# MarinerQ/npf_GWwaveform

Measured on AMD Instinct MI355X. Metric: waveform target-points/sec (train step), higher is better.
Workload: dtype f32 (every contraction of the step: fp32 operands as three exact bf16 terms, six v_mfma_f32_16x16x32_bf16 per product group, f32 accumulation -- f32 results, DESIGN.md 3.1 / 3.2; the 1-4-wide first / last layers: f32 FMAs); 1 GPU; BASELINE config 2: AttnCNP scaledot, r=256, 4-layer xy-encoder/decoder, 256 context / 1024 target points, 256 tasks per GPU (256 global), fp32 train step (fwd+loss+bwd+allreduce+Adam); tasks_per_gpu=256, global_tasks=256, context_points=256, target_points=1024, r_dim=256, n_params=799588, parallelism=dp1, hip_graph=True

## Files before the change

include/npf_hip.h:

```cpp
#ifndef NPF_HIP_H
#define NPF_HIP_H

#include <stdint.h>

#ifdef __cplusplus
extern "C" {
#endif

#define NPF_OK 0
#define NPF_EINVAL (-1)
#define NPF_ELAUNCH (-2)

#define NPF_MAX_OPS 40
#define NPF_MAX_FEATURES 512

enum npf_opcode {
  NPF_OP_END = 0,
  NPF_OP_LOAD_PT = 1,
  NPF_OP_STORE_PT = 2,
  NPF_OP_LOAD_ROWS = 3,
  NPF_OP_STORE_ROWS = 4,
  NPF_OP_LINEAR = 5,
  NPF_OP_SOFTMAX = 6,
  NPF_OP_ADD_PT = 7,
  NPF_OP_MASK_POS = 8,
  NPF_OP_ADD_TASKVEC = 9,
  NPF_OP_ROWDOT_PT = 10,
  NPF_OP_SOFTMAX_BWD = 11,
  NPF_OP_RELU = 12,
  NPF_OP_SCALE = 13,
  NPF_OP_STORE_TR = 14,
  NPF_OP_LAYERNORM = 15,
  NPF_OP_STORE_WB = 18,
  NPF_OP_STORE_TRB = 19,
  NPF_OP_LOAD_RM = 17,
  NPF_OP_STORE_MASK = 20,
  NPF_OP_MASK_BITS = 21,
  NPF_OP_LAYERNORM_BWD = 16
};

enum npf_wmode {
  NPF_W_ROWMAJOR = 0,
  NPF_W_PT_ROWS = 1,
  NPF_W_PT_COLS = 2
};

#define NPF_F_RELU 1u
#define NPF_F_ADD_PT 2u
#define NPF_F_MASK_PT 4u
#define NPF_F_P16 16u
#define NPF_F_MASK_BITS 32u
#define NPF_F_ADD_RM 8u
#define NPF_F_STORE_IN 64u
#define NPF_F_STORE_BITS 256u
#define NPF_F_STORE_P16 128u

typedef struct npf_op {
  int32_t op;
  int32_t i0;
  int32_t i1;
  int32_t i2;
  int32_t i3;
  uint32_t flags;
  float f0;
  int32_t i4;
  const void *p0;
  const void *p1;
  const void *p2;
  int64_t s0;
  int64_t s1;
  void *p3;
} npf_op_t;

typedef struct npf_program {
  int32_t n_ops;
  int32_t n_tasks;
  int32_t pts_per_task;
  int32_t tiles_per_task;
  int32_t wg_per_task;
  int32_t reserved[3];
  npf_op_t ops[NPF_MAX_OPS];
} npf_program_t;

int npf_chain_run(const npf_program_t *prog, void *stream);

typedef struct npf_wgrad_job {
  const float *dZ;
  const float *A;
  float *dW;
  float *db;
  int64_t ldw;
  int32_t N, K;
  int32_t per_task;
  int32_t accumulate;
  int32_t ldz, lda, ldo;
  int32_t reserved;
} npf_wgrad_job_t;
#define NPF_WGRAD_ACCUMULATE 1
#define NPF_WGRAD_BF16 2
#define NPF_WGRAD_DZ16 4
#define NPF_WGRAD_A16 8
#define NPF_WGRAD_F32X6 16
#define NPF_WGRAD_NO_H16 32

#define NPF_MAX_WGRAD_JOBS 16
int npf_wgrad_run(const npf_wgrad_job_t *jobs, int32_t n_jobs, int32_t n_tasks, int32_t tiles_per_task,
                  float *partials, int64_t partials_bytes, void *stream);
int64_t npf_wgrad_partials_bytes(const npf_wgrad_job_t *jobs, int32_t n_jobs, int32_t n_tasks,
                                 int32_t tiles_per_task);

int npf_gauss_head_fwd(const float *suff, int32_t n_rows, int32_t pts, int32_t dy, int32_t homoskedastic,
                       const float *Y, int32_t n_y_rows, float *loc, float *scale, float *sum_logp,
                       void *stream);
int npf_gauss_head_bwd(const float *suff, const float *loc, const float *scale, int32_t n_rows, int32_t pts,
                       int32_t dy, int32_t homoskedastic, const float *Y, int32_t n_y_rows,
                       const float *d_loc, const float *d_scale, const float *d_sum_logp, float *d_suff,
                       void *stream);

int npf_masked_gauss_head_fwd(const float *suff, const int32_t *n_valid, int32_t n_tasks, int32_t n_rows, int32_t pts, int32_t dy,
                              int32_t homoskedastic, const float *Y, int32_t n_y_rows, float *loc, float *scale,
                              float *sum_logp, void *stream);
int npf_masked_gauss_head_bwd(const float *suff, const float *loc, const float *scale, const int32_t *n_valid, int32_t n_tasks,
                              int32_t n_rows, int32_t pts, int32_t dy, int32_t homoskedastic, const float *Y, int32_t n_y_rows,
                              const float *d_loc, const float *d_scale, const float *d_sum_logp, float *d_suff, void *stream);

int npf_mixture_summary(const float *suff, const int32_t *n_valid, int32_t n_z, int32_t n_tasks, int32_t pts, int32_t dy,
                        int32_t homoskedastic, const float *z_p, int32_t n_probs, const float *probs, float *mean, float *std,
                        float *quant, void *stream);

int npf_mixture_score(const float *suff, const float *Y, const int32_t *n_valid, int32_t n_z, int32_t n_tasks, int32_t pts,
                      int32_t dy, int32_t homoskedastic, float *log_density, float *pit, float *crps, void *stream);

int npf_mc_objective_fwd(const float *log_w, int32_t n_z, int32_t n_tasks, int32_t mode, const float *inv_weights,
                         int32_t m, float *out, void *stream);
int npf_mc_objective_bwd(const float *log_w, int32_t n_z, int32_t n_tasks, int32_t mode, const float *inv_weights,
                         int32_t m, const float *d_out, float *d_log_w, float *workspace, void *stream);

int npf_mean_agg_fwd(const float *R_pt, int32_t n_tasks, int32_t pts_per_task, int32_t F, float *out,
                     void *stream);
int npf_mean_agg_bwd(const float *d_out, int32_t n_tasks, int32_t pts_per_task, int32_t F, float *dR_pt,
                     int32_t accumulate, void *stream);

int npf_pack_pt(const float *rows, int32_t n_tasks, int32_t pts_per_task, int32_t F_valid, float *pt,
                void *stream);
int npf_unpack_pt(const float *pt, int32_t n_tasks, int32_t pts_per_task, int32_t F_valid, float *rows,
                  void *stream);
int npf_transpose(const float *src, int32_t rows, int32_t cols, float *dst, void *stream);
int npf_split_heads(const float *src, int32_t n_tasks, int32_t pts_per_task, int32_t F, int32_t n_heads, float *dst,
                    void *stream);
int npf_merge_heads(const float *src, int32_t n_tasks, int32_t pts_per_task, int32_t F, int32_t n_heads, float *dst,
                    void *stream);

int npf_mha_fwd(const float *q, const float *k, const float *v, int32_t n_tasks, int32_t n_heads, int32_t n_keys,
                int32_t n_queries, int32_t F, float *out, float *lse, void *stream);
int npf_mha_bwd(const float *q, const float *k, const float *v, const float *out, const float *d_out, const float *lse,
                int32_t n_tasks, int32_t n_heads, int32_t n_keys, int32_t n_queries, int32_t F, float *d_q, float *d_k, float *d_v,
                void *stream);

int npf_add_layernorm_fwd(const float *a, const float *b, const float *gamma, const float *beta, float eps, int32_t n_tasks,
                          int32_t pts_per_task, int32_t F, float *y, float *stats, void *stream);
int npf_add_layernorm_bwd(const float *a, const float *b, const float *gamma, const float *stats, const float *dy, int32_t n_tasks,
                          int32_t pts_per_task, int32_t F, float *dx, float *partials, void *stream);

int npf_gather_points(const float *x, const float *y, const int64_t *idx, int32_t n_tasks, int32_t n_points,
                      int32_t n_sel, int32_t x_dim, int32_t y_dim, float *out_x, float *out_y, void *stream);

int npf_cast_bf16_weights(const float *src, int32_t n_rows, int32_t n_cols, int32_t ld, int32_t transposed, void *dst,
                          void *stream);

typedef struct npf_wprep_job {
  const float *src;
  void *dst;
  int32_t n_rows, n_cols, ld, kind;
} npf_wprep_job_t;
#define NPF_MAX_WPREP_JOBS 32
int npf_prepare_weights(const npf_wprep_job_t *jobs, int32_t n_jobs, void *stream);

#define NPF_X6_MAX_LAYERS 8
typedef struct {
  const void *w_img;
  const float *bias;
  const float *mask;
  float *store_in;
  float *store_out;
  const float *addend;
  unsigned long long *store_bits;
  const unsigned long long *mask_bits;
  int32_t relu;
  int32_t reserved;
} npf_x6_layer_t;
int npf_mlp_x6_run(const npf_x6_layer_t *layers, int32_t n_layers, const float *x, float *y, int32_t n_tasks,
                   int32_t tiles_per_task, void *stream);
int npf_mlp_x6_run_rows(const npf_x6_layer_t *layers, int32_t n_layers, const float *x, const float *in_rows, const float *in_w,
                        float *y, const float *out_w, const float *out_b, float *out_rows, int32_t n_tasks,
                        int32_t tiles_per_task, void *stream);

#define NPF_X6_MAX_OPS 12
typedef struct npf_x6_op {
  const float *in_pt;
  const float *in_rows;
  const float *in_w;
  const float *in_b;
  const float *pre_add;
  const float *mask;
  const unsigned long long *mask_bits;
  const float *sbwd_p;
  float *store_in;
  unsigned long long *store_in_bits;
  const void *w_img;
  int64_t w_task_stride;
  const float *bias;
  int64_t bias_task_stride;
  const float *addend;
  float *store_out;
  unsigned long long *store_bits;
  int32_t in_n;
  int32_t in_relu;
  int32_t relu;
  int32_t softmax_n;
  float softmax_scale;
  float sbwd_scale;
  int32_t reserved[2];
} npf_x6_op_t;
#define NPF_X6_IN_RM 1
#define NPF_X6_ADD_RM 2
#define NPF_X6_STORE_IN_F32 4
#define NPF_X6_STORE_OUT_F32 8
#define NPF_X6_DEFAULT_VARIANT 3
int npf_x6_run_ex(const npf_x6_op_t *ops, int32_t n_ops, const float *out_w, const float *out_b, float *out_rows,
                  int32_t n_tasks, int32_t tiles_per_task, int32_t pts_per_task, int32_t per_task, int32_t width,
                  int32_t variant, void *stream);
int npf_x6_run(const npf_x6_op_t *ops, int32_t n_ops, const float *out_w, const float *out_b, float *out_rows,
               int32_t n_tasks, int32_t tiles_per_task, int32_t per_task, int32_t width, void *stream);
int npf_x6_task_images(const float *src, int32_t n_tasks, int32_t pts, int32_t width, void *row_img, void *tr_img, void *stream);

int npf_b16_run(const npf_x6_op_t *ops, int32_t n_ops, const float *out_w, const float *out_b, float *out_rows, int32_t n_tasks,
                int32_t tiles_per_task, int32_t per_task, int32_t width, int32_t variant, void *stream);
int npf_b16_task_images(const float *src, int32_t n_tasks, int32_t pts, int32_t width, void *row_img, void *tr_img, void *stream);

int npf_masked_attn_fwd(const float *q, const float *k, const float *v, const int32_t *n_valid, int32_t n_tasks, int32_t n_keys,
                        int32_t n_queries, int32_t d, float scale, float *out, float *lse, void *stream);
int npf_masked_attn_bwd(const float *q, const float *k, const float *v, const int32_t *n_valid, const float *out, const float *d_out,
                        const float *lse, int32_t n_tasks, int32_t n_keys, int32_t n_queries, int32_t d, float scale, float *d_q,
                        float *d_k, float *d_v, void *stream);
int npf_masked_attn_fwd_nq(const float *q, const float *k, const float *v, const int32_t *n_valid, const int32_t *n_q_valid,
                           int32_t n_tasks, int32_t n_keys, int32_t n_queries, int32_t d, float scale, float *out, float *lse,
                           void *stream);
int npf_masked_attn_bwd_nq(const float *q, const float *k, const float *v, const int32_t *n_valid, const int32_t *n_q_valid,
                           const float *out, const float *d_out, const float *lse, int32_t n_tasks, int32_t n_keys, int32_t n_queries,
                           int32_t d, float scale, float *d_q, float *d_k, float *d_v, void *stream);
int npf_masked_attn_fwd_prefix(const float *q, const float *k_pre, const float *v_pre, const int32_t *n_prefix, const float *k_tail,
                               const float *v_tail, const int32_t *n_tail, const int32_t *n_q_valid, int32_t n_tasks,
                               int32_t n_prefix_tasks, int32_t c_pad, int32_t m_tail, int32_t n_queries, int32_t d, float scale,
                               float *out, void *stream);
int npf_masked_attn_fwd_loo(const float *q, const float *k, const float *v, const int32_t *n_valid, const int32_t *n_q_valid,
                            int32_t n_tasks, int32_t n_keys, int32_t n_queries, int32_t d, float scale, float *out, void *stream);
int npf_masked_mean_fwd(const float *R_pt, const int32_t *n_valid, int32_t n_tasks, int32_t pts_per_task, int32_t F, float *out,
                        void *stream);
int npf_masked_mean_bwd(const float *d_out, const int32_t *n_valid, int32_t n_tasks, int32_t pts_per_task, int32_t F, float *dR_pt,
                        int32_t accumulate, void *stream);
int npf_loo_mean(const float *R_pt, const int32_t *n_valid, int32_t n_tasks, int32_t pts_per_task, int32_t F, float *out,
                 void *stream);
int npf_masked_attn_fwd_weighted(const float *q, const float *k, const float *v, const float *w, const int32_t *n_valid,
                                 const int32_t *n_q_valid, int32_t n_tasks, int32_t n_ctx_tasks, int32_t n_keys, int32_t n_queries,
                                 int32_t d, float scale, float *out, void *stream);
int npf_weighted_mean(const float *R_pt, const float *w, const int32_t *n_valid, int32_t n_tasks, int32_t n_ctx_tasks,
                      int32_t pts_per_task, int32_t F, float *out, void *stream);

int npf_masked_attn_fwd_weighted_ex(const float *q, const float *k, const float *v, const float *w, const int32_t *n_valid,
                                    const int32_t *n_q_valid, int32_t n_tasks, int32_t n_ctx_tasks, int32_t n_keys,
                                    int32_t n_queries, int32_t d, float scale, float *out, float *lse, void *stream);
int npf_masked_attn_bwd_weighted(const float *q, const float *k, const float *v, const float *w, const int32_t *n_valid,
                                 const int32_t *n_q_valid, const float *out, const float *d_out, const float *lse, int32_t n_tasks,
                                 int32_t n_keys, int32_t n_queries, int32_t d, float scale, float *d_q, float *d_k, float *d_v,
                                 float *d_w, void *stream);
int npf_weighted_mean_bwd(const float *R_pt, const float *w, const int32_t *n_valid, const float *out, const float *d_out,
                          int32_t n_tasks, int32_t pts_per_task, int32_t F, float *dR_pt, float *dw, void *stream);

#define NPF_APPEND_MAX_PAIRS 3
typedef struct npf_append_pair {
  const float *src;
  float *dst;
  int32_t F;
  int32_t reserved;
} npf_append_pair_t;
int npf_append_points(const npf_append_pair_t *pairs, int32_t n_pairs, int32_t *n_valid, const int32_t *n_new, int32_t n_tasks,
                      int32_t n_rows, int32_t capacity, void *stream);

#define NPF_WAVEFORM_JC 16
int64_t npf_waveform_match_workspace_bytes(int32_t n_rows, int32_t n_tau);
int npf_waveform_match(const float *h, int32_t h_ld, const float *g, const float *wgt, int32_t wgt_rows, const float *freq,
                       int32_t freq_rows, const int32_t *n_valid, int32_t n_rows, int32_t n_tasks, int32_t pts, double tau0,
                       double dtau, int32_t n_tau, float *hh, float *gg, float *overlap, float *match, float *mismatch,
                       int32_t *tau_index, float *phase, float *corr, void *workspace, void *stream);
int npf_waveform_match_ex(const float *h, int32_t h_ld, const float *g, const float *wgt, int32_t wgt_rows, const float *freq,
                          int32_t freq_rows, const int32_t *n_valid, int32_t n_rows, int32_t n_tasks, int32_t pts, double tau0,
                          double dtau, int32_t n_tau, float *hh, float *gg, float *overlap, float *match, float *mismatch,
                          int32_t *tau_index, float *phase, float *corr, void *workspace, double *saved, void *stream);
int npf_waveform_match_bwd(const float *h, int32_t h_ld, const float *g, const float *wgt, int32_t wgt_rows, const float *freq,
                           int32_t freq_rows, const int32_t *n_valid, int32_t n_rows, int32_t n_tasks, int32_t pts, double tau0,
                           double dtau, int32_t n_tau, const int32_t *tau_index, const double *saved, const float *d_match,
                           int32_t n_bcast, float *d_h, int32_t dh_ld, void *stream);

#define NPF_LOGLIKE_I0_SWITCH 24.0
int64_t npf_waveform_loglike_workspace_bytes(int32_t n_rows, int32_t n_tau);
int npf_waveform_loglike(const float *h, int32_t h_ld, const float *d, const float *wgt, int32_t wgt_rows, const float *freq,
                         int32_t freq_rows, const int32_t *n_valid, int32_t n_rows, int32_t n_tasks, int32_t pts, double tau0,
                         double dtau, int32_t n_tau, double *hh, double *dd, double *snr, double *lnl_max, double *lnl_marg,
                         int32_t *tau_index, double *phase, double *series, double *lnl_mix, double *lnl_max_mix, void *workspace,
                         void *stream);

#define NPF_NET_MAX_DET 8
int64_t npf_waveform_loglike_net_workspace_bytes(int32_t n_rows, int32_t n_det, int32_t n_tau);
int npf_waveform_loglike_net(const float *h, int32_t h_ld, const float *d, const float *wgt, int32_t wgt_rows, const float *freq,
                             int32_t freq_rows, const int32_t *n_valid, const double *delay, const double *resp, int32_t n_rows,
                             int32_t n_tasks, int32_t n_det, int32_t pts, double tau0, double dtau, int32_t n_tau, double *hh,
                             double *dd, double *snr, double *lnl_max, double *lnl_marg, int32_t *tau_index, double *phase,
                             double *series, double *lnl_mix, double *lnl_max_mix, double *hh_det, double *snr_det, double *dd_det,
                             void *workspace, void *stream);

int npf_version(void);

#ifdef __cplusplus
}
#endif
#endif
```

npf_gwwaveform_amd/_lib.py:

```python
from __future__ import annotations

import ctypes as C
import os
from typing import Optional

import torch

from . import _build

NPF_MAX_OPS = 40
NPF_MAX_FEATURES = 512
NPF_WGRAD_BLOCK = 256
NPF_MAX_FUSED_ROW = 256

OP_END, OP_LOAD_PT, OP_STORE_PT, OP_LOAD_ROWS, OP_STORE_ROWS, OP_LINEAR, OP_SOFTMAX, OP_ADD_PT, OP_MASK_POS, \
    OP_ADD_TASKVEC, OP_ROWDOT_PT, OP_SOFTMAX_BWD, OP_RELU, OP_SCALE, OP_STORE_TR, OP_LAYERNORM, OP_LAYERNORM_BWD, OP_LOAD_RM, OP_STORE_WB, OP_STORE_TRB, \
    OP_STORE_MASK, OP_MASK_BITS = range(22)
W_ROWMAJOR, W_PT_ROWS, W_PT_COLS = range(3)
F_RELU, F_ADD_PT, F_MASK_PT, F_ADD_RM, F_P16, F_MASK_BITS, F_STORE_IN, F_STORE_P16, F_STORE_BITS = 1, 2, 4, 8, 16, 32, 64, 128, 256


class NpfOp(C.Structure):
    _fields_ = [
        ("op", C.c_int32), ("i0", C.c_int32), ("i1", C.c_int32), ("i2", C.c_int32), ("i3", C.c_int32),
        ("flags", C.c_uint32), ("f0", C.c_float), ("i4", C.c_int32),
        ("p0", C.c_void_p), ("p1", C.c_void_p), ("p2", C.c_void_p),
        ("s0", C.c_int64), ("s1", C.c_int64), ("p3", C.c_void_p),
    ]


class NpfProgram(C.Structure):
    _fields_ = [
        ("n_ops", C.c_int32), ("n_tasks", C.c_int32), ("pts_per_task", C.c_int32), ("tiles_per_task", C.c_int32),
        ("wg_per_task", C.c_int32), ("reserved", C.c_int32 * 3),
        ("ops", NpfOp * NPF_MAX_OPS),
    ]


class NpfWgradJob(C.Structure):
    _fields_ = [
        ("dZ", C.c_void_p), ("A", C.c_void_p), ("dW", C.c_void_p), ("db", C.c_void_p), ("ldw", C.c_int64),
        ("N", C.c_int32), ("K", C.c_int32), ("per_task", C.c_int32), ("accumulate", C.c_int32),
        ("ldz", C.c_int32), ("lda", C.c_int32), ("ldo", C.c_int32), ("reserved", C.c_int32),
    ]


NPF_MAX_WGRAD_JOBS = 16
WGRAD_F32X6 = 16
WGRAD_NO_H16 = 32


class NpfWprepJob(C.Structure):
    _fields_ = [("src", C.c_void_p), ("dst", C.c_void_p), ("n_rows", C.c_int32), ("n_cols", C.c_int32), ("ld", C.c_int32),
                ("kind", C.c_int32)]


NPF_MAX_WPREP_JOBS = 32
NPF_X6_MAX_LAYERS = 8


class NpfX6Layer(C.Structure):
    _fields_ = [("w_img", C.c_void_p), ("bias", C.c_void_p), ("mask", C.c_void_p), ("store_in", C.c_void_p),
                ("store_out", C.c_void_p), ("addend", C.c_void_p), ("store_bits", C.c_void_p), ("mask_bits", C.c_void_p),
                ("relu", C.c_int32), ("reserved", C.c_int32)]


NPF_X6_MAX_OPS = 12
X6_IN_RM, X6_ADD_RM = 1, 2
X6_STORE_IN_F32, X6_STORE_OUT_F32 = 4, 8


class NpfX6Op(C.Structure):
    _fields_ = [("in_pt", C.c_void_p), ("in_rows", C.c_void_p), ("in_w", C.c_void_p), ("in_b", C.c_void_p),
                ("pre_add", C.c_void_p), ("mask", C.c_void_p), ("mask_bits", C.c_void_p), ("sbwd_p", C.c_void_p),
                ("store_in", C.c_void_p), ("store_in_bits", C.c_void_p), ("w_img", C.c_void_p), ("w_task_stride", C.c_int64),
                ("bias", C.c_void_p), ("bias_task_stride", C.c_int64), ("addend", C.c_void_p), ("store_out", C.c_void_p),
                ("store_bits", C.c_void_p), ("in_n", C.c_int32), ("in_relu", C.c_int32), ("relu", C.c_int32),
                ("softmax_n", C.c_int32), ("softmax_scale", C.c_float), ("sbwd_scale", C.c_float), ("reserved", C.c_int32 * 2)]


NPF_APPEND_MAX_PAIRS = 3


class NpfAppendPair(C.Structure):
    _fields_ = [("src", C.c_void_p), ("dst", C.c_void_p), ("F", C.c_int32), ("reserved", C.c_int32)]


assert C.sizeof(NpfAppendPair) == 24
assert C.sizeof(NpfX6Op) == 17 * 8 + 8 * 4
assert C.sizeof(NpfOp) == 80 and C.sizeof(NpfProgram) == 32 + 80 * NPF_MAX_OPS and C.sizeof(NpfWgradJob) == 72 and C.sizeof(NpfWprepJob) == 32

_i32, _i64, _p = C.c_int32, C.c_int64, C.c_void_p
SIGNATURES = {
    "npf_chain_run": (C.c_int, [C.POINTER(NpfProgram), _p]),
    "npf_wgrad_run": (C.c_int, [C.POINTER(NpfWgradJob), _i32, _i32, _i32, _p, _i64, _p]),
    "npf_wgrad_partials_bytes": (_i64, [C.POINTER(NpfWgradJob), _i32, _i32, _i32]),
    "npf_gauss_head_fwd": (C.c_int, [_p, _i32, _i32, _i32, _i32, _p, _i32, _p, _p, _p, _p]),
    "npf_gauss_head_bwd": (C.c_int, [_p, _p, _p, _i32, _i32, _i32, _i32, _p, _i32, _p, _p, _p, _p, _p]),
    "npf_mc_objective_fwd": (C.c_int, [_p, _i32, _i32, _i32, _p, _i32, _p, _p]),
    "npf_mc_objective_bwd": (C.c_int, [_p, _i32, _i32, _i32, _p, _i32, _p, _p, _p, _p]),
    "npf_mean_agg_fwd": (C.c_int, [_p, _i32, _i32, _i32, _p, _p]),
    "npf_mean_agg_bwd": (C.c_int, [_p, _i32, _i32, _i32, _p, _i32, _p]),
    "npf_pack_pt": (C.c_int, [_p, _i32, _i32, _i32, _p, _p]),
    "npf_unpack_pt": (C.c_int, [_p, _i32, _i32, _i32, _p, _p]),
    "npf_transpose": (C.c_int, [_p, _i32, _i32, _p, _p]),
    "npf_cast_bf16_weights": (C.c_int, [_p, _i32, _i32, _i32, _i32, _p, _p]),
    "npf_prepare_weights": (C.c_int, [C.POINTER(NpfWprepJob), _i32, _p]),
    "npf_gather_points": (C.c_int, [_p, _p, _p, _i32, _i32, _i32, _i32, _i32, _p, _p, _p]),
    "npf_split_heads": (C.c_int, [_p, _i32, _i32, _i32, _i32, _p, _p]),
    "npf_merge_heads": (C.c_int, [_p, _i32, _i32, _i32, _i32, _p, _p]),
    "npf_mlp_x6_run": (C.c_int, [C.POINTER(NpfX6Layer), _i32, _p, _p, _i32, _i32, _p]),
    "npf_mlp_x6_run_rows": (C.c_int, [C.POINTER(NpfX6Layer), _i32, _p, _p, _p, _p, _p, _p, _p, _i32, _i32, _p]),
    "npf_x6_run": (C.c_int, [C.POINTER(NpfX6Op), _i32, _p, _p, _p, _i32, _i32, _i32, _i32, _p]),
    "npf_x6_run_ex": (C.c_int, [C.POINTER(NpfX6Op), _i32, _p, _p, _p, _i32, _i32, _i32, _i32, _i32, _i32, _p]),
    "npf_x6_task_images": (C.c_int, [_p, _i32, _i32, _i32, _p, _p, _p]),
    "npf_b16_run": (C.c_int, [C.POINTER(NpfX6Op), _i32, _p, _p, _p, _i32, _i32, _i32, _i32, _i32, _p]),
    "npf_b16_task_images": (C.c_int, [_p, _i32, _i32, _i32, _p, _p, _p]),
    "npf_mha_fwd": (C.c_int, [_p, _p, _p, _i32, _i32, _i32, _i32, _i32, _p, _p, _p]),
    "npf_mha_bwd": (C.c_int, [_p, _p, _p, _p, _p, _p, _i32, _i32, _i32, _i32, _i32, _p, _p, _p, _p]),
    "npf_add_layernorm_fwd": (C.c_int, [_p, _p, _p, _p, C.c_float, _i32, _i32, _i32, _p, _p, _p]),
    "npf_add_layernorm_bwd": (C.c_int, [_p, _p, _p, _p, _p, _i32, _i32, _i32, _p, _p, _p]),
    "npf_masked_attn_fwd": (C.c_int, [_p, _p, _p, _p, _i32, _i32, _i32, _i32, C.c_float, _p, _p, _p]),
    "npf_masked_attn_bwd": (C.c_int, [_p, _p, _p, _p, _p, _p, _p, _i32, _i32, _i32, _i32, C.c_float, _p, _p, _p, _p]),
    "npf_masked_attn_fwd_nq": (C.c_int, [_p, _p, _p, _p, _p, _i32, _i32, _i32, _i32, C.c_float, _p, _p, _p]),
    "npf_masked_attn_bwd_nq": (C.c_int, [_p, _p, _p, _p, _p, _p, _p, _p, _i32, _i32, _i32, _i32, C.c_float, _p, _p, _p, _p]),
    "npf_masked_attn_fwd_prefix": (C.c_int, [_p, _p, _p, _p, _p, _p, _p, _p, _i32, _i32, _i32, _i32, _i32, _i32, C.c_float, _p, _p]),
    "npf_masked_attn_fwd_loo": (C.c_int, [_p, _p, _p, _p, _p, _i32, _i32, _i32, _i32, C.c_float, _p, _p]),
    "npf_loo_mean": (C.c_int, [_p, _p, _i32, _i32, _i32, _p, _p]),
    "npf_masked_attn_fwd_weighted": (C.c_int, [_p, _p, _p, _p, _p, _p, _i32, _i32, _i32, _i32, _i32, C.c_float, _p, _p]),
    "npf_weighted_mean": (C.c_int, [_p, _p, _p, _i32, _i32, _i32, _i32, _p, _p]),
    "npf_masked_attn_fwd_weighted_ex": (C.c_int, [_p, _p, _p, _p, _p, _p, _i32, _i32, _i32, _i32, _i32, C.c_float, _p, _p, _p]),
    "npf_masked_attn_bwd_weighted": (C.c_int, [_p, _p, _p, _p, _p, _p, _p, _p, _p, _i32, _i32, _i32, _i32, C.c_float,
                                               _p, _p, _p, _p, _p]),
    "npf_weighted_mean_bwd": (C.c_int, [_p, _p, _p, _p, _p, _i32, _i32, _i32, _p, _p, _p]),
    "npf_masked_gauss_head_fwd": (C.c_int, [_p, _p, _i32, _i32, _i32, _i32, _i32, _p, _i32, _p, _p, _p, _p]),
    "npf_masked_gauss_head_bwd": (C.c_int, [_p, _p, _p, _p, _i32, _i32, _i32, _i32, _i32, _p, _i32, _p, _p, _p, _p, _p]),
    "npf_mixture_summary": (C.c_int, [_p, _p, _i32, _i32, _i32, _i32, _i32, _p, _i32, _p, _p, _p, _p, _p]),
    "npf_mixture_score": (C.c_int, [_p, _p, _p, _i32, _i32, _i32, _i32, _i32, _p, _p, _p, _p]),
    "npf_masked_mean_fwd": (C.c_int, [_p, _p, _i32, _i32, _i32, _p, _p]),
    "npf_masked_mean_bwd": (C.c_int, [_p, _p, _i32, _i32, _i32, _p, _i32, _p]),
    "npf_append_points": (C.c_int, [C.POINTER(NpfAppendPair), _i32, _p, _p, _i32, _i32, _i32, _p]),
    "npf_waveform_match_workspace_bytes": (_i64, [_i32, _i32]),
    "npf_waveform_match": (C.c_int, [_p, _i32, _p, _p, _i32, _p, _i32, _p, _i32, _i32, _i32, C.c_double, C.c_double, _i32,
                                     _p, _p, _p, _p, _p, _p, _p, _p, _p, _p]),
    "npf_waveform_match_ex": (C.c_int, [_p, _i32, _p, _p, _i32, _p, _i32, _p, _i32, _i32, _i32, C.c_double, C.c_double, _i32,
                                        _p, _p, _p, _p, _p, _p, _p, _p, _p, _p, _p]),
    "npf_waveform_match_bwd": (C.c_int, [_p, _i32, _p, _p, _i32, _p, _i32, _p, _i32, _i32, _i32, C.c_double, C.c_double, _i32,
                                         _p, _p, _p, _i32, _p, _i32, _p]),
    "npf_waveform_loglike_workspace_bytes": (_i64, [_i32, _i32]),
    "npf_waveform_loglike": (C.c_int, [_p, _i32, _p, _p, _i32, _p, _i32, _p, _i32, _i32, _i32, C.c_double, C.c_double, _i32,
                                       _p, _p, _p, _p, _p, _p, _p, _p, _p, _p, _p, _p]),
    "npf_waveform_loglike_net_workspace_bytes": (_i64, [_i32, _i32, _i32]),
    "npf_waveform_loglike_net": (C.c_int, [_p, _i32, _p, _p, _i32, _p, _i32, _p, _p, _p, _i32, _i32, _i32, _i32, C.c_double, C.c_double,
                                           _i32, _p, _p, _p, _p, _p, _p, _p, _p, _p, _p, _p, _p, _p, _p, _p]),
    "npf_version": (C.c_int, []),
}

_lib: Optional[C.CDLL] = None


def lib_path() -> str:
    return os.environ.get("NPF_HIP_LIB") or _build.LIB_PATH


def load() -> C.CDLL:
    global _lib
    if _lib is not None:
        return _lib
    path = lib_path()
    if not os.path.exists(path):
        raise RuntimeError(
            f"HIP extension {path} is missing. Build it with `python -m npf_gwwaveform_amd._build` "
            "(needs hipcc); there is no CPU fallback for the neural-process path."
        )
    try:
        lib = C.CDLL(path)
    except OSError as e:
        raise RuntimeError(f"HIP extension {path} failed to load: {e}") from e
    for name, (res, args) in SIGNATURES.items():
        fn = getattr(lib, name)
        fn.restype = res
        fn.argtypes = args
    _lib = lib
    return lib


def check(rc: int, what: str) -> None:
    if rc != 0:
        raise RuntimeError(f"{what} failed with status {rc} "
                           f"({'invalid argument/unsupported size' if rc == -1 else 'kernel launch error'})")


def stream_ptr(device: Optional[torch.device] = None) -> int:
    return torch.cuda.current_stream(device).cuda_stream


def ptr(t: Optional[torch.Tensor], strided: bool = False) -> Optional[int]:
    if t is None:
        return None
    if not t.is_cuda:
        raise RuntimeError("the HIP path takes device tensors only (got a CPU tensor); there is no CPU fallback")
    if t.dtype != torch.float32:
        raise RuntimeError(f"the HIP path computes in fp32 (got {t.dtype})")
    if not strided and not t.is_contiguous():
        raise RuntimeError("tensor handed to the HIP path must be contiguous")
    return t.data_ptr()
```

npf_gwwaveform_amd/csrc/layout_kernels.hip:

```cpp
#include "npf_common.hpp"

namespace npf {

__global__ void pack_pt_kernel(const float* __restrict__ rows, int n_tasks, int pts, int Fv, int Fp, float* __restrict__ pt) {
  const int tiles = (pts + 31) / 32;
  const size_t total = (size_t)n_tasks * tiles * (Fp / 4) * 32;
  for (size_t idx = blockIdx.x * (size_t)blockDim.x + threadIdx.x; idx < total; idx += (size_t)gridDim.x * blockDim.x) {
    const int p = idx & 31;
    const size_t r = idx >> 5;
    const int f4 = r % (Fp / 4);
    const size_t tt = r / (Fp / 4);
    const int tile = tt % tiles;
    const size_t task = tt / tiles;
    const int point = tile * 32 + p;
    f32x4 v = {0.f, 0.f, 0.f, 0.f};
    if (point < pts) {
      const float* src = rows + (task * pts + point) * (size_t)Fv + 4 * f4;
#pragma unroll
      for (int j = 0; j < 4; ++j)
        if (4 * f4 + j < Fv) v[j] = src[j];
    }
    *(f32x4*)(pt + idx * 4) = v;
  }
}

__global__ void unpack_pt_kernel(const float* __restrict__ pt, int n_tasks, int pts, int Fv, int Fp, float* __restrict__ rows) {
  const int tiles = (pts + 31) / 32;
  const size_t total = (size_t)n_tasks * tiles * (Fp / 4) * 32;
  for (size_t idx = blockIdx.x * (size_t)blockDim.x + threadIdx.x; idx < total; idx += (size_t)gridDim.x * blockDim.x) {
    const int p = idx & 31;
    const size_t r = idx >> 5;
    const int f4 = r % (Fp / 4);
    const size_t tt = r / (Fp / 4);
    const int tile = tt % tiles;
    const size_t task = tt / tiles;
    const int point = tile * 32 + p;
    if (point < pts) {
      const f32x4 v = *(const f32x4*)(pt + idx * 4);
      float* dst = rows + (task * pts + point) * (size_t)Fv + 4 * f4;
#pragma unroll
      for (int j = 0; j < 4; ++j)
        if (4 * f4 + j < Fv) dst[j] = v[j];
    }
  }
}

template <bool SPLIT>
__global__ void heads_kernel(const float* __restrict__ src, int n_tasks, int pts, int Fp, int hsz, int n_heads,
                             float* __restrict__ dst) {
  const int tiles = (pts + 31) / 32;
  const int hq = ((hsz + 31) / 32) * 8;
  const int fq = Fp / 4;
  if (SPLIT) {
    const size_t total = (size_t)n_heads * n_tasks * tiles * hq * 32;
    for (size_t idx = blockIdx.x * (size_t)blockDim.x + threadIdx.x; idx < total; idx += (size_t)gridDim.x * blockDim.x) {
      const int p = idx & 31;
      const size_t r = idx >> 5;
      const int q = r % hq;
      const size_t tt = r / hq;
      const int tile = tt % tiles;
      const size_t ht = tt / tiles;
      const int h = ht / n_tasks, b = ht - (size_t)h * n_tasks;
      f32x4 v = {0.f, 0.f, 0.f, 0.f};
      if (4 * q < hsz) v = *(const f32x4*)(src + ((((size_t)b * tiles + tile) * fq + (h * hsz) / 4 + q) * 32 + p) * 4);
      *(f32x4*)(dst + idx * 4) = v;
    }
  } else {
    const size_t total = (size_t)n_tasks * tiles * fq * 32;
    for (size_t idx = blockIdx.x * (size_t)blockDim.x + threadIdx.x; idx < total; idx += (size_t)gridDim.x * blockDim.x) {
      const int p = idx & 31;
      const size_t r = idx >> 5;
      const int q = r % fq;
      const size_t tt = r / fq;
      const int tile = tt % tiles;
      const size_t b = tt / tiles;
      const int h = (4 * q) / hsz, qh = q - (h * hsz) / 4;
      f32x4 v = {0.f, 0.f, 0.f, 0.f};
      if (h < n_heads) v = *(const f32x4*)(src + (((((size_t)h * n_tasks + b) * tiles + tile) * hq + qh) * 32 + p) * 4);
      *(f32x4*)(dst + idx * 4) = v;
    }
  }
}

__global__ void gather_points_kernel(const float* __restrict__ x, const float* __restrict__ y,
                                     const long long* __restrict__ idx, int n_tasks, int n_points, int n_sel, int x_dim,
                                     int y_dim, float* __restrict__ out_x, float* __restrict__ out_y) {
  const size_t total = (size_t)n_tasks * n_sel;
  for (size_t t = blockIdx.x * (size_t)blockDim.x + threadIdx.x; t < total; t += (size_t)gridDim.x * blockDim.x) {
    const size_t b = t / n_sel;
    long long j = idx[t];
    j = j < 0 ? 0 : (j >= n_points ? n_points - 1 : j);
    const float* xs = x + (b * n_points + (size_t)j) * x_dim;
    for (int d = 0; d < x_dim; ++d) out_x[t * x_dim + d] = xs[d];
    if (y) {
      const float* ys = y + (b * n_points + (size_t)j) * y_dim;
      for (int d = 0; d < y_dim; ++d) out_y[t * y_dim + d] = ys[d];
    }
  }
}

__global__ void cast_bf16_weights_kernel(const float* __restrict__ src, int n_rows, int n_cols, int ld, int transposed,
                                         unsigned short* __restrict__ dst) {
  const int rows = transposed ? n_cols : n_rows, cols = transposed ? n_rows : n_cols;
  const int Kp = ((cols + 31) >> 5) * 32;
  const size_t total = (size_t)rows * Kp;
  for (size_t idx = blockIdx.x * (size_t)blockDim.x + threadIdx.x; idx < total; idx += (size_t)gridDim.x * blockDim.x) {
    const int r = idx / Kp, q = idx - (size_t)r * Kp;
    const int sgrp = q >> 5, g = (q & 31) >> 3, i = q & 7;
    const int c = 32 * sgrp + (i < 4 ? 4 * g + i : 16 + 4 * g + (i - 4));
    float v = 0.f;
    if (c < cols) v = transposed ? src[(size_t)c * ld + r] : src[(size_t)r * ld + c];
    const __bf16 b = (__bf16)v;
    dst[idx] = __builtin_bit_cast(unsigned short, b);
  }
}

__global__ void transpose_kernel(const float* __restrict__ src, int rows, int cols, float* __restrict__ dst) {
  __shared__ float tile[32][33];
  const int c0 = blockIdx.x * 32, r0 = blockIdx.y * 32;
  const int tx = threadIdx.x & 31, ty = threadIdx.x >> 5;
  for (int i = ty; i < 32; i += 8)
    if (r0 + i < rows && c0 + tx < cols) tile[i][tx] = src[(size_t)(r0 + i) * cols + c0 + tx];
  __syncthreads();
  for (int i = ty; i < 32; i += 8)
    if (c0 + i < cols && r0 + tx < rows) dst[(size_t)(c0 + i) * rows + r0 + tx] = tile[tx][i];
}

struct WprepJobs {
  npf_wprep_job_t job[NPF_MAX_WPREP_JOBS];
};
__global__ void prepare_weights_kernel(const WprepJobs J) {
  __shared__ float tile[32][33];
  const npf_wprep_job_t& jb = J.job[blockIdx.y];
  const float* __restrict__ src = jb.src;
  if (jb.kind == 0) {
    float* __restrict__ dst = (float*)jb.dst;
    const int rows = jb.n_rows, cols = jb.n_cols, ld = jb.ld;
    const int tc = (cols + 31) / 32, tr = (rows + 31) / 32;
    const int tx = threadIdx.x & 31, ty = threadIdx.x >> 5;
    for (int tl = blockIdx.x; tl < tc * tr; tl += gridDim.x) {
      const int c0 = (tl % tc) * 32, r0 = (tl / tc) * 32;
      for (int i = ty; i < 32; i += 8)
        if (r0 + i < rows && c0 + tx < cols) tile[i][tx] = src[(size_t)(r0 + i) * ld + c0 + tx];
      __syncthreads();
      for (int i = ty; i < 32; i += 8)
        if (c0 + i < cols && r0 + tx < rows) dst[(size_t)(c0 + i) * rows + r0 + tx] = tile[tx][i];
      __syncthreads();
    }
  } else {
    unsigned short* __restrict__ dst = (unsigned short*)jb.dst;
    const bool transposed = (jb.kind & 3) == 2;
    const int term = (jb.kind >> 4) & 3;
    const int rows = transposed ? jb.n_cols : jb.n_rows, cols = transposed ? jb.n_rows : jb.n_cols, ld = jb.ld;
    const int Kp = (jb.kind & 4) ? 256 : ((cols + 31) >> 5) * 32;
    const size_t total = (size_t)rows * Kp;
    for (size_t idx = blockIdx.x * (size_t)blockDim.x + threadIdx.x; idx < total; idx += (size_t)gridDim.x * blockDim.x) {
      const int r = idx / Kp, q = idx - (size_t)r * Kp;
      const int sgrp = q >> 5, g = (q & 31) >> 3, i = q & 7;
      const int c = 32 * sgrp + (i < 4 ? 4 * g + i : 16 + 4 * g + (i - 4));
      float v = 0.f;
      if (c < cols) v = transposed ? src[(size_t)c * ld + r] : src[(size_t)r * ld + c];
      for (int t = 1; t < term; ++t) v -= (float)(__bf16)v;
      const __bf16 b = (__bf16)v;
      dst[idx] = __builtin_bit_cast(unsigned short, b);
    }
  }
}

template <bool MASKED>
__global__ void mean_fwd_kernel(const float* __restrict__ R, const int32_t* __restrict__ n_valid, int pts, int F,
                                float* __restrict__ out) {
  const int tiles = (pts + 31) / 32;
  const int p = threadIdx.x & 31, f4 = blockIdx.x * 8 + (threadIdx.x >> 5);
  const size_t task = blockIdx.y;
  const int n = MASKED ? clamp_count(n_valid, task, pts) : pts;
  const bool in_F = MASKED || f4 < F / 4;
  f32x4 s = {0.f, 0.f, 0.f, 0.f};
  if (in_F) {
    const float* base = R + task * tiles * (size_t)(F * 32) + pt_off(f4, p);
    for (int t = 0; t * 32 < n; ++t)
      if (t * 32 + p < n) s += *(const f32x4*)(base + (size_t)t * F * 32);
  }
#pragma unroll
  for (int off = 16; off >= 1; off >>= 1)
#pragma unroll
    for (int j = 0; j < 4; ++j) s[j] += __shfl_xor(s[j], off);
  if (p == 0 && in_F) *(f32x4*)(out + task * F + 4 * f4) = (!MASKED || n > 0) ? s * (1.f / (float)n) : f32x4{0.f, 0.f, 0.f, 0.f};
}

__global__ void loo_mean_kernel(const float* __restrict__ R, const int32_t* __restrict__ n_valid, int pts, int F,
                                float* __restrict__ out) {
  const int tiles = (pts + 31) / 32;
  const int p = threadIdx.x & 31, f4 = blockIdx.x * 8 + (threadIdx.x >> 5);
  const size_t task = blockIdx.y;
  const int n = clamp_count(n_valid, task, pts);
  const size_t at = task * tiles * (size_t)(F * 32) + pt_off(f4, p);
  double s[4] = {0.0, 0.0, 0.0, 0.0};
  for (int t = 0; t * 32 < n; ++t)
    if (t * 32 + p < n) {
      const f32x4 r = *(const f32x4*)(R + at + (size_t)t * F * 32);
#pragma unroll
      for (int j = 0; j < 4; ++j) s[j] += (double)r[j];
    }
#pragma unroll
  for (int off = 16; off >= 1; off >>= 1)
#pragma unroll
    for (int j = 0; j < 4; ++j) s[j] += __shfl_xor(s[j], off);
  const double others = (double)(n - 1);
  for (int t = 0; t < tiles; ++t) {
    f32x4 v = {0.f, 0.f, 0.f, 0.f};
    if (n > 1 && t * 32 + p < n) {
      const f32x4 r = *(const f32x4*)(R + at + (size_t)t * F * 32);
#pragma unroll
      for (int j = 0; j < 4; ++j) v[j] = (float)((s[j] - (double)r[j]) / others);
    }
    *(f32x4*)(out + at + (size_t)t * F * 32) = v;
  }
}

__global__ void weighted_mean_kernel(const float* __restrict__ R, const float* __restrict__ W, const int32_t* __restrict__ n_valid,
                                     int n_ctx_tasks, int pts, int F, float* __restrict__ out) {
  const int tiles = (pts + 31) / 32, fblocks = F / 32;
  const int p = threadIdx.x & 31, f4 = (blockIdx.x % fblocks) * 8 + (threadIdx.x >> 5);
  const size_t task = blockIdx.x / fblocks, bc = task % n_ctx_tasks;
  const int n = clamp_count(n_valid, bc, pts);
  const float* base = R + bc * tiles * (size_t)(F * 32) + pt_off(f4, p);
  const float* wrow = W + task * pts;
  double s[4] = {0.0, 0.0, 0.0, 0.0}, ws = 0.0;
  for (int t = 0; t * 32 < n; ++t)
    if (t * 32 + p < n) {
      const float w = wrow[t * 32 + p];
      if (w > 0.f && w < INFINITY) {
        const f32x4 r = *(const f32x4*)(base + (size_t)t * F * 32);
#pragma unroll
        for (int j = 0; j < 4; ++j) s[j] += (double)w * (double)r[j];
        ws += (double)w;
      }
    }
#pragma unroll
  for (int off = 16; off >= 1; off >>= 1) {
#pragma unroll
    for (int j = 0; j < 4; ++j) s[j] += __shfl_xor(s[j], off);
    ws += __shfl_xor(ws, off);
  }
  if (p == 0) {
    f32x4 v = {0.f, 0.f, 0.f, 0.f};
    if (ws > 0.0) {
#pragma unroll
      for (int j = 0; j < 4; ++j) v[j] = (float)(s[j] / ws);
    }
    *(f32x4*)(out + task * F + 4 * f4) = v;
  }
}

__global__ void weighted_mean_bwd_kernel(const float* __restrict__ R, const float* __restrict__ W, const int32_t* __restrict__ n_valid,
                                         const float* __restrict__ , const float* __restrict__ d_out, int pts, int F,
                                         float* __restrict__ dR, float* __restrict__ dW) {
  __shared__ double part[8 * 32];
  const int tiles = (pts + 31) / 32;
  const int p = threadIdx.x & 31, fg = threadIdx.x >> 5;
  const size_t task = blockIdx.x / tiles;
  const int t = blockIdx.x % tiles;
  const int n = clamp_count(n_valid, task, pts);
  const float* wrow = W + task * pts;
  double ws = 0.0;
  for (int tt = 0; tt * 32 < n; ++tt)
    if (tt * 32 + p < n) {
      const float w = wrow[tt * 32 + p];
      if (w > 0.f && w < INFINITY) ws += (double)w;
    }
#pragma unroll
  for (int off = 16; off >= 1; off >>= 1) ws += __shfl_xor(ws, off);
  const int pt = t * 32 + p;
  const float w = pt < n ? wrow[pt] : 0.f;
  const bool ok = ws > 0.0 && w > 0.f && w < INFINITY;
  const double cw = ok ? (double)w / ws : 0.0;
  const size_t base = (task * tiles + t) * (size_t)(F * 32);
  const bool any = ws > 0.0 && t * 32 < n;
  double dot = 0.0;
  for (int f4 = fg; f4 < F / 4; f4 += 8) {
    double o[4] = {0.0, 0.0, 0.0, 0.0};
    if (any) {
      for (int tt = 0; tt * 32 < n; ++tt)
        if (tt * 32 + p < n) {
          const float wk = wrow[tt * 32 + p];
          if (wk > 0.f && wk < INFINITY) {
            const f32x4 r = *(const f32x4*)(R + (task * tiles + tt) * (size_t)(F * 32) + pt_off(f4, p));
#pragma unroll
            for (int j = 0; j < 4; ++j) o[j] += (double)wk * (double)r[j];
          }
        }
#pragma unroll
      for (int off = 16; off >= 1; off >>= 1) {
#pragma unroll
        for (int j = 0; j < 4; ++j) o[j] += __shfl_xor(o[j], off);
      }
#pragma unroll
      for (int j = 0; j < 4; ++j) o[j] /= ws;
    }
    f32x4 v = {0.f, 0.f, 0.f, 0.f};
    if (ok) {
      const f32x4 r = *(const f32x4*)(R + base + pt_off(f4, p));
      const f32x4 gq = *(const f32x4*)(d_out + task * F + 4 * f4);
#pragma unroll
      for (int j = 0; j < 4; ++j) {
        v[j] = (float)(cw * (double)gq[j]);
        dot += (double)gq[j] * ((double)r[j] - o[j]);
      }
    }
    *(f32x4*)(dR + base + pt_off(f4, p)) = v;
  }
  part[fg * 32 + p] = dot;
  __syncthreads();
  if (fg == 0 && pt < pts) {
    double s = 0.0;
#pragma unroll
    for (int k = 0; k < 8; ++k) s += part[k * 32 + p];
    dW[task * pts + pt] = ok ? (float)(s / ws) : 0.f;
  }
}

template <bool MASKED>
__global__ void mean_bwd_kernel(const float* __restrict__ d_out, const int32_t* __restrict__ n_valid, int n_tasks, int pts, int F,
                                float* __restrict__ dR, int accumulate) {
  const int tiles = (pts + 31) / 32;
  const size_t total = (size_t)n_tasks * tiles * (F / 4) * 32;
  for (size_t idx = blockIdx.x * (size_t)blockDim.x + threadIdx.x; idx < total; idx += (size_t)gridDim.x * blockDim.x) {
    const int p = idx & 31;
    const size_t r = idx >> 5;
    const int f4 = r % (F / 4);
    const size_t tt = r / (F / 4);
    const int tile = tt % tiles;
    const size_t task = tt / tiles;
    const int n = MASKED ? clamp_count(n_valid, task, pts) : pts;
    f32x4 v = {0.f, 0.f, 0.f, 0.f};
    if (tile * 32 + p < n) v = *(const f32x4*)(d_out + task * F + 4 * f4) * (1.f / (float)n);
    if (accumulate) v += *(const f32x4*)(dR + idx * 4);
    *(f32x4*)(dR + idx * 4) = v;
  }
}

static unsigned grid_for(size_t total, int block) {
  size_t g = (total + block - 1) / block;
  if (g > 256u * 8u) g = 256u * 8u;
  if (g == 0) g = 1;
  return (unsigned)g;
}

}

extern "C" int npf_pack_pt(const float* rows, int32_t n_tasks, int32_t pts, int32_t Fv, float* pt, void* stream) {
  if (!rows || !pt || n_tasks <= 0 || pts <= 0 || Fv <= 0) return NPF_EINVAL;
  const int Fp = npf::round_up(Fv, 32);
  const size_t total = (size_t)n_tasks * ((pts + 31) / 32) * (Fp / 4) * 32;
  hipLaunchKernelGGL(npf::pack_pt_kernel, dim3(npf::grid_for(total, 256)), dim3(256), 0, (hipStream_t)stream, rows, n_tasks,
                     pts, Fv, Fp, pt);
  NPF_CHECK_LAUNCH();
  return NPF_OK;
}

extern "C" int npf_unpack_pt(const float* pt, int32_t n_tasks, int32_t pts, int32_t Fv, float* rows, void* stream) {
  if (!rows || !pt || n_tasks <= 0 || pts <= 0 || Fv <= 0) return NPF_EINVAL;
  const int Fp = npf::round_up(Fv, 32);
  const size_t total = (size_t)n_tasks * ((pts + 31) / 32) * (Fp / 4) * 32;
  hipLaunchKernelGGL(npf::unpack_pt_kernel, dim3(npf::grid_for(total, 256)), dim3(256), 0, (hipStream_t)stream, pt,
                     n_tasks, pts, Fv, Fp, rows);
  NPF_CHECK_LAUNCH();
  return NPF_OK;
}

extern "C" int npf_transpose(const float* src, int32_t rows, int32_t cols, float* dst, void* stream) {
  if (!src || !dst || rows <= 0 || cols <= 0) return NPF_EINVAL;
  hipLaunchKernelGGL(npf::transpose_kernel, dim3((cols + 31) / 32, (rows + 31) / 32), dim3(256), 0, (hipStream_t)stream,
                     src, rows, cols, dst);
  NPF_CHECK_LAUNCH();
  return NPF_OK;
}

static int heads_launch(bool split, const float* src, int32_t n_tasks, int32_t pts, int32_t F, int32_t n_heads, float* dst,
                        void* stream) {
  if (!src || !dst || n_tasks <= 0 || pts <= 0 || F <= 0 || n_heads <= 0 || F % n_heads) return NPF_EINVAL;
  const int hsz = F / n_heads;
  if (hsz & 3) return NPF_EINVAL;
  const int Fp = npf::round_up(F, 32), tiles = (pts + 31) / 32;
  if (split) {
    const size_t total = (size_t)n_heads * n_tasks * tiles * (npf::round_up(hsz, 32) / 4) * 32;
    hipLaunchKernelGGL(npf::heads_kernel<true>, dim3(npf::grid_for(total, 256)), dim3(256), 0, (hipStream_t)stream, src,
                       n_tasks, pts, Fp, hsz, n_heads, dst);
  } else {
    const size_t total = (size_t)n_tasks * tiles * (Fp / 4) * 32;
    hipLaunchKernelGGL(npf::heads_kernel<false>, dim3(npf::grid_for(total, 256)), dim3(256), 0, (hipStream_t)stream, src,
                       n_tasks, pts, Fp, hsz, n_heads, dst);
  }
  NPF_CHECK_LAUNCH();
  return NPF_OK;
}

extern "C" int npf_gather_points(const float* x, const float* y, const int64_t* idx, int32_t n_tasks, int32_t n_points,
                                 int32_t n_sel, int32_t x_dim, int32_t y_dim, float* out_x, float* out_y, void* stream) {
  if (!x || !idx || !out_x || n_tasks <= 0 || n_points <= 0 || n_sel < 0 || x_dim <= 0) return NPF_EINVAL;
  if (y && (!out_y || y_dim <= 0)) return NPF_EINVAL;
  if (n_sel == 0) return NPF_OK;
  const size_t total = (size_t)n_tasks * n_sel;
  hipLaunchKernelGGL(npf::gather_points_kernel, dim3(npf::grid_for(total, 256)), dim3(256), 0, (hipStream_t)stream, x, y,
                     (const long long*)idx, n_tasks, n_points, n_sel, x_dim, y_dim, out_x, out_y);
  NPF_CHECK_LAUNCH();
  return NPF_OK;
}

extern "C" int npf_cast_bf16_weights(const float* src, int32_t n_rows, int32_t n_cols, int32_t ld, int32_t transposed,
                                     void* dst, void* stream) {
  if (!src || !dst || n_rows <= 0 || n_cols <= 0 || ld < n_cols || (((uintptr_t)dst) & 15)) return NPF_EINVAL;
  const int rows = transposed ? n_cols : n_rows, cols = transposed ? n_rows : n_cols;
  const size_t total = (size_t)rows * npf::round_up(cols, 32);
  hipLaunchKernelGGL(npf::cast_bf16_weights_kernel, dim3(npf::grid_for(total, 256)), dim3(256), 0, (hipStream_t)stream, src,
                     n_rows, n_cols, ld, transposed, (unsigned short*)dst);
  NPF_CHECK_LAUNCH();
  return NPF_OK;
}

extern "C" int npf_prepare_weights(const npf_wprep_job_t* jobs, int32_t n_jobs, void* stream) {
  if (!jobs || n_jobs <= 0 || n_jobs > NPF_MAX_WPREP_JOBS) return NPF_EINVAL;
  npf::WprepJobs J;
  size_t most = 0;
  for (int j = 0; j < n_jobs; ++j) {
    const npf_wprep_job_t& b = jobs[j];
    const int base = b.kind & 15, term = b.kind >> 4;
    const bool kind_ok = b.kind >= 0 && ((term == 0 && (base <= 2 || base == 5 || base == 6)) || (term >= 1 && term <= 3 && (base == 1 || base == 2)));
    if (!b.src || !b.dst || b.n_rows <= 0 || b.n_cols <= 0 || b.ld < b.n_cols || !kind_ok) return NPF_EINVAL;
    if (b.kind != 0 && (((uintptr_t)b.dst) & 15)) return NPF_EINVAL;
    if ((b.kind == 5 && b.n_cols > 256) || (b.kind == 6 && b.n_rows > 256)) return NPF_EINVAL;
    J.job[j] = b;
    const size_t img_rows = (b.kind & 3) == 2 ? b.n_cols : b.n_rows;
    const size_t blocks = b.kind == 0   ? (size_t)((b.n_rows + 31) / 32) * ((b.n_cols + 31) / 32)
                          : (b.kind & 4) ? (img_rows * 256 + 255) / 256
                                         : ((size_t)b.n_rows * b.n_cols + 255) / 256;
    most = blocks > most ? blocks : most;
  }
  for (int j = n_jobs; j < NPF_MAX_WPREP_JOBS; ++j) J.job[j] = jobs[0];
  const unsigned gx = (unsigned)(most < 64 ? most : 64);
  hipLaunchKernelGGL(npf::prepare_weights_kernel, dim3(gx ? gx : 1, n_jobs), dim3(256), 0, (hipStream_t)stream, J);
  NPF_CHECK_LAUNCH();
  return NPF_OK;
}

extern "C" int npf_split_heads(const float* src, int32_t n_tasks, int32_t pts, int32_t F, int32_t n_heads, float* dst,
                               void* stream) {
  return heads_launch(true, src, n_tasks, pts, F, n_heads, dst, stream);
}

extern "C" int npf_merge_heads(const float* src, int32_t n_tasks, int32_t pts, int32_t F, int32_t n_heads, float* dst,
                               void* stream) {
  return heads_launch(false, src, n_tasks, pts, F, n_heads, dst, stream);
}

extern "C" int npf_mean_agg_fwd(const float* R_pt, int32_t n_tasks, int32_t pts, int32_t F, float* out, void* stream) {
  if (!R_pt || !out || n_tasks <= 0 || pts <= 0 || F <= 0 || (F & 31)) return NPF_EINVAL;
  hipLaunchKernelGGL(npf::mean_fwd_kernel<false>, dim3(F / 32, n_tasks), dim3(256), 0, (hipStream_t)stream, R_pt, nullptr, pts, F,
                     out);
  NPF_CHECK_LAUNCH();
  return NPF_OK;
}

extern "C" int npf_mean_agg_bwd(const float* d_out, int32_t n_tasks, int32_t pts, int32_t F, float* dR_pt,
                                int32_t accumulate, void* stream) {
  if (!d_out || !dR_pt || n_tasks <= 0 || pts <= 0 || F <= 0 || (F & 31)) return NPF_EINVAL;
  const size_t total = (size_t)n_tasks * ((pts + 31) / 32) * (F / 4) * 32;
  hipLaunchKernelGGL(npf::mean_bwd_kernel<false>, dim3(npf::grid_for(total, 256)), dim3(256), 0, (hipStream_t)stream, d_out,
                     nullptr, n_tasks, pts, F, dR_pt, accumulate);
  NPF_CHECK_LAUNCH();
  return NPF_OK;
}

extern "C" int npf_masked_mean_fwd(const float* R_pt, const int32_t* n_valid, int32_t n_tasks, int32_t pts, int32_t F, float* out,
                                   void* stream) {
  if (!R_pt || !n_valid || !out || n_tasks < 0 || pts <= 0 || F <= 0 || (F & 31)) return NPF_EINVAL;
  if ((((uintptr_t)R_pt) | ((uintptr_t)out)) & 15) return NPF_EINVAL;
  if (n_tasks == 0) return NPF_OK;
  hipLaunchKernelGGL(npf::mean_fwd_kernel<true>, dim3(F / 32, n_tasks), dim3(256), 0, (hipStream_t)stream, R_pt, n_valid, pts, F, out);
  NPF_CHECK_LAUNCH();
  return NPF_OK;
}

extern "C" int npf_masked_mean_bwd(const float* d_out, const int32_t* n_valid, int32_t n_tasks, int32_t pts, int32_t F, float* dR_pt,
                                   int32_t accumulate, void* stream) {
  if (!d_out || !n_valid || !dR_pt || n_tasks < 0 || pts <= 0 || F <= 0 || (F & 31)) return NPF_EINVAL;
  if ((((uintptr_t)d_out) | ((uintptr_t)dR_pt)) & 15) return NPF_EINVAL;
  if (n_tasks == 0) return NPF_OK;
  const size_t total = (size_t)n_tasks * ((pts + 31) / 32) * (F / 4) * 32;
  hipLaunchKernelGGL(npf::mean_bwd_kernel<true>, dim3(npf::grid_for(total, 256)), dim3(256), 0, (hipStream_t)stream, d_out, n_valid,
                     n_tasks, pts, F, dR_pt, accumulate);
  NPF_CHECK_LAUNCH();
  return NPF_OK;
}

extern "C" int npf_loo_mean(const float* R_pt, const int32_t* n_valid, int32_t n_tasks, int32_t pts, int32_t F, float* out,
                            void* stream) {
  if (!R_pt || !n_valid || !out || n_tasks < 0 || pts <= 0 || F <= 0 || (F & 31)) return NPF_EINVAL;
  if ((((uintptr_t)R_pt) | ((uintptr_t)out)) & 15) return NPF_EINVAL;
  if (n_tasks == 0) return NPF_OK;
  if (n_tasks > 65535) return NPF_EINVAL;
  hipLaunchKernelGGL(npf::loo_mean_kernel, dim3(F / 32, n_tasks), dim3(256), 0, (hipStream_t)stream, R_pt, n_valid, pts, F, out);
  NPF_CHECK_LAUNCH();
  return NPF_OK;
}

extern "C" int npf_weighted_mean(const float* R_pt, const float* w, const int32_t* n_valid, int32_t n_tasks, int32_t n_ctx_tasks,
                                 int32_t pts, int32_t F, float* out, void* stream) {
  if (!R_pt || !w || !n_valid || !out || n_tasks < 0 || n_ctx_tasks <= 0 || n_tasks % n_ctx_tasks != 0) return NPF_EINVAL;
  if (pts <= 0 || F <= 0 || (F & 31)) return NPF_EINVAL;
  if (((((uintptr_t)R_pt) | ((uintptr_t)out)) & 15) || (((uintptr_t)w) & 3)) return NPF_EINVAL;
  if (n_tasks == 0) return NPF_OK;
  if ((size_t)n_tasks * (F / 32) > 0x7fffffffu) return NPF_EINVAL;
  hipLaunchKernelGGL(npf::weighted_mean_kernel, dim3((unsigned)n_tasks * (F / 32)), dim3(256), 0, (hipStream_t)stream, R_pt, w, n_valid,
                     n_ctx_tasks, pts, F, out);
  NPF_CHECK_LAUNCH();
  return NPF_OK;
}

extern "C" int npf_weighted_mean_bwd(const float* R_pt, const float* w, const int32_t* n_valid, const float* out, const float* d_out,
                                     int32_t n_tasks, int32_t pts, int32_t F, float* dR_pt, float* dw, void* stream) {
  if (!R_pt || !w || !n_valid || !out || !d_out || !dR_pt || !dw || n_tasks < 0) return NPF_EINVAL;
  if (pts <= 0 || F <= 0 || (F & 31)) return NPF_EINVAL;
  if ((((uintptr_t)R_pt) | ((uintptr_t)out) | ((uintptr_t)d_out) | ((uintptr_t)dR_pt)) & 15) return NPF_EINVAL;
  if ((((uintptr_t)w) | ((uintptr_t)dw)) & 3) return NPF_EINVAL;
  if (n_tasks == 0) return NPF_OK;
  const size_t blocks = (size_t)n_tasks * ((pts + 31) / 32);
  if (blocks > 0x7fffffffu) return NPF_EINVAL;
  hipLaunchKernelGGL(npf::weighted_mean_bwd_kernel, dim3((unsigned)blocks), dim3(256), 0, (hipStream_t)stream, R_pt, w, n_valid, out,
                     d_out, pts, F, dR_pt, dw);
  NPF_CHECK_LAUNCH();
  return NPF_OK;
}

extern "C" int npf_version(void) { return 2; }
```

npf_gwwaveform_amd/csrc/npf_common.hpp:

```cpp
#pragma once
#include <hip/hip_runtime.h>
#include <stdint.h>

#include "npf_hip.h"

typedef float f32x16 __attribute__((ext_vector_type(16)));
typedef float f32x4 __attribute__((ext_vector_type(4)));

namespace npf {

constexpr int kTilePts = 32;

__host__ __device__ inline int pt_off(int f4, int p) { return (f4 * 32 + p) * 4; }

inline int round_up(int v, int m) { return (v + m - 1) / m * m; }

__device__ __forceinline__ int clamp_count(const int32_t* __restrict__ n, size_t i, int hi) {
  const int v = n[i];
  return v < 0 ? 0 : (v > hi ? hi : v);
}

#define NPF_CHECK_LAUNCH()                     \
  do {                                         \
    hipError_t e__ = hipGetLastError();        \
    if (e__ != hipSuccess) return NPF_ELAUNCH; \
  } while (0)

__device__ __forceinline__ float block_sum(float v, float* red) {
#pragma unroll
  for (int off = 32; off >= 1; off >>= 1) v += __shfl_xor(v, off);
  const int wave = threadIdx.x >> 6;
  __syncthreads();
  if ((threadIdx.x & 63) == 0) red[wave] = v;
  __syncthreads();
  float s = 0.f;
  for (int i = 0; i < (int)(blockDim.x >> 6); ++i) s += red[i];
  return s;
}

__device__ __forceinline__ float softplus_t(float x) { return x > 20.f ? x : log1pf(expf(x)); }

}
```

npf_gwwaveform_amd/functional.py:

```python
from __future__ import annotations

import math
import os
from typing import NamedTuple, Optional

import torch

from . import _lib as L
from . import chain as CH
from .chain import pad32, pt_empty, pt_shape, tiles_of


def _pack(rows: torch.Tensor) -> torch.Tensor:
    n_tasks, pts, F = rows.shape
    out = pt_empty(n_tasks, pts, F, rows.device)
    L.check(L.load().npf_pack_pt(L.ptr(rows.contiguous()), n_tasks, pts, F, L.ptr(out), L.stream_ptr()), "npf_pack_pt")
    return out


def _unpack(pt: torch.Tensor, pts: int, F: int) -> torch.Tensor:
    n_tasks = pt.shape[0]
    out = torch.empty((n_tasks, pts, F), dtype=torch.float32, device=pt.device)
    L.check(L.load().npf_unpack_pt(L.ptr(pt.contiguous()), n_tasks, pts, F, L.ptr(out), L.stream_ptr()), "npf_unpack_pt")
    return out


class _PackFn(torch.autograd.Function):
    @staticmethod
    def forward(ctx, rows):
        ctx.pts, ctx.F = rows.shape[1], rows.shape[2]
        return _pack(rows)

    @staticmethod
    def backward(ctx, g):
        return _unpack(g.contiguous(), ctx.pts, ctx.F)


class _UnpackFn(torch.autograd.Function):
    @staticmethod
    def forward(ctx, pt, pts, F):
        return _unpack(pt, pts, F)

    @staticmethod
    def backward(ctx, g):
        return _pack(g.contiguous()), None, None


def pack_pt(rows: torch.Tensor) -> torch.Tensor:
    return _PackFn.apply(rows)


def unpack_pt(pt: torch.Tensor, pts: int, F: int) -> torch.Tensor:
    return _UnpackFn.apply(pt, pts, F)


def sum_points_pt(pt: torch.Tensor, pts: int, F: int) -> torch.Tensor:
    n_tasks = pt.shape[0]
    Fp = pad32(F)
    out = torch.empty((n_tasks, Fp), dtype=torch.float32, device=pt.device)
    L.check(L.load().npf_mean_agg_fwd(L.ptr(pt), n_tasks, pts, Fp, L.ptr(out), L.stream_ptr()), "npf_mean_agg_fwd")
    return out * float(pts)


class _MeanFn(torch.autograd.Function):

    @staticmethod
    def forward(ctx, pt, n_valid, n_tasks, pts, F):
        Fp = pad32(F)
        ctx.geo = (n_tasks, pts, Fp)
        if n_valid is not None:
            ctx.save_for_backward(n_valid)
        out = torch.empty((n_tasks, Fp), dtype=torch.float32, device=pt.device)
        name, counts = ("npf_mean_agg_fwd", ()) if n_valid is None else ("npf_masked_mean_fwd", (_iptr(n_valid),))
        L.check(getattr(L.load(), name)(L.ptr(pt.contiguous()), *counts, n_tasks, pts, Fp, L.ptr(out), L.stream_ptr()), name)
        return out

    @staticmethod
    def backward(ctx, g):
        n_tasks, pts, Fp = ctx.geo
        d = pt_empty(n_tasks, pts, Fp, g.device)
        name, counts = ("npf_masked_mean_bwd", (_iptr(ctx.saved_tensors[0]),)) if ctx.saved_tensors else ("npf_mean_agg_bwd", ())
        L.check(getattr(L.load(), name)(L.ptr(g.contiguous()), *counts, n_tasks, pts, Fp, L.ptr(d), 0, L.stream_ptr()), name)
        return d, None, None, None, None


def mean_agg(pt: torch.Tensor, pts: int, F: int) -> torch.Tensor:
    return _MeanFn.apply(pt, None, pt.shape[0], pts, F)


class _GaussHeadFn(torch.autograd.Function):

    @staticmethod
    def forward(ctx, suff, Y, n_valid, dy, homosk, want_dist):
        n_rows, pts, two_dy = suff.shape
        n_tasks = 1 if n_valid is None else n_valid.shape[0]
        assert two_dy == 2 * dy and n_rows % n_tasks == 0
        suff = suff.contiguous()
        loc = scale = None
        if want_dist:
            loc = torch.empty((n_rows, pts, dy), dtype=torch.float32, device=suff.device)
            scale = torch.empty_like(loc)
        slp = None
        n_y = 0
        if Y is not None:
            Y = Y.contiguous()
            n_y = Y.shape[0]
            assert Y.shape[1:] == (pts, dy) and n_rows % n_y == 0 and n_y % n_tasks == 0
            slp = torch.empty((n_rows,), dtype=torch.float32, device=suff.device)
        elif not want_dist:
            raise ValueError("a loss-only head launch needs the targets")
        name, counts = ("npf_gauss_head_fwd", ()) if n_valid is None else ("npf_masked_gauss_head_fwd", (_iptr(n_valid), n_tasks))
        L.check(getattr(L.load(), name)(L.ptr(suff), *counts, n_rows, pts, dy, int(homosk), L.ptr(Y), n_y, L.ptr(loc), L.ptr(scale),
                                        L.ptr(slp), L.stream_ptr()), name)
        ctx.save_for_backward(suff, loc, scale, Y, *(() if n_valid is None else (n_valid,)))
        ctx.cfg = (dy, homosk)
        empty = suff.new_zeros((0,))
        outs = [loc if want_dist else empty, scale if want_dist else empty, slp if slp is not None else suff.new_zeros((n_rows,))]
        nd = ([] if want_dist else [outs[0], outs[1]]) + ([] if slp is not None else [outs[2]])
        if nd:
            ctx.mark_non_differentiable(*nd)
        return tuple(outs)

    @staticmethod
    def backward(ctx, d_loc, d_scale, d_slp):
        suff, loc, scale, Y, *n_valid = ctx.saved_tensors
        dy, homosk = ctx.cfg
        n_rows, pts, _ = suff.shape
        d_suff = torch.empty_like(suff)
        c = lambda t: t.contiguous() if t is not None else None
        if loc is None:
            d_loc = d_scale = None
        name, counts = ("npf_masked_gauss_head_bwd", (_iptr(n_valid[0]), n_valid[0].shape[0])) if n_valid else ("npf_gauss_head_bwd", ())
        L.check(getattr(L.load(), name)(L.ptr(suff), L.ptr(loc), L.ptr(scale), *counts, n_rows, pts, dy, int(homosk), L.ptr(Y),
                                        Y.shape[0] if Y is not None else 0, L.ptr(c(d_loc)), L.ptr(c(d_scale)),
                                        L.ptr(c(d_slp)) if Y is not None else None, L.ptr(d_suff), L.stream_ptr()), name)
        return d_suff, None, None, None, None, None


def gauss_head(suff: torch.Tensor, Y: Optional[torch.Tensor], dy: int, homoskedastic: bool, want_dist: bool = True,
               n_valid: Optional[torch.Tensor] = None):
    if n_valid is not None:
        n_tasks = n_valid.shape[0] if isinstance(n_valid, torch.Tensor) and n_valid.dim() == 1 else suff.shape[0]
        if suff.shape[0] % max(n_tasks, 1) != 0 or n_tasks == 0:
            raise ValueError(f"n_valid has {n_tasks} counts, the head {suff.shape[0]} rows (not a multiple)")
        n_valid = counts_i32(n_valid, n_tasks)
    return _GaussHeadFn.apply(suff, Y, n_valid, dy, homoskedastic, want_dist)


MIXTURE_MAX_NZ = 128
_Z_P_CACHE = {}


def check_probs(probs) -> tuple:
    if isinstance(probs, torch.Tensor) or not isinstance(probs, (tuple, list)):
        raise ValueError(f"probs must be a host sequence (tuple / list) of probabilities, got {type(probs).__name__}")
    out = []
    for p in probs:
        if isinstance(p, torch.Tensor) or isinstance(p, bool) or not isinstance(p, (int, float)):
            raise ValueError(f"probs must hold host floats, got {type(p).__name__}")
        if not (0.0 < float(p) < 1.0):
            raise ValueError(f"probs must lie strictly inside (0, 1), got {p}")
        out.append(float(p))
    return tuple(out)


def normal_quantiles(probs) -> tuple:
    probs = check_probs(probs)
    if not probs:
        return ()
    return tuple(torch.special.ndtri(torch.tensor(probs, dtype=torch.float64)).tolist())


def _z_p_device(probs: tuple, device: torch.device):
    key = (probs, device.type, device.index if device.index is not None else torch.cuda.current_device())
    hit = _Z_P_CACHE.get(key)
    if hit is None:
        hit = (torch.tensor(normal_quantiles(probs), dtype=torch.float64).to(torch.float32).to(device),
               torch.tensor(probs, dtype=torch.float64).to(torch.float32).to(device))
        _Z_P_CACHE[key] = hit
    return hit


def mixture_summary(suff: torch.Tensor, n_z: int, dy: int, homoskedastic: bool, probs=(), n_valid: Optional[torch.Tensor] = None):
    probs = check_probs(probs)
    if not suff.is_cuda or suff.dtype != torch.float32:
        raise RuntimeError("the HIP path takes fp32 device tensors only; there is no CPU fallback")
    n_rows, pts, two_dy = suff.shape
    if two_dy != 2 * dy or n_z < 1 or n_rows % n_z != 0:
        raise ValueError(f"suff of shape {tuple(suff.shape)} does not hold n_z={n_z} samples of a {dy}-dimensional head")
    if n_z > MIXTURE_MAX_NZ:
        raise NotImplementedError(f"mixture_summary covers up to {MIXTURE_MAX_NZ} latent samples (got {n_z})")
    B = n_rows // n_z
    suff = suff.detach().contiguous()
    nv = counts_i32(n_valid, B) if n_valid is not None else None
    mean = torch.empty((B, pts, dy), dtype=torch.float32, device=suff.device)
    std = torch.empty_like(mean)
    quant = torch.empty((len(probs), B, pts, dy), dtype=torch.float32, device=suff.device)
    z_p, p_dev = _z_p_device(probs, suff.device) if probs else (None, None)
    L.check(L.load().npf_mixture_summary(L.ptr(suff), _iptr(nv) if nv is not None else None, n_z, B, pts, dy, int(homoskedastic),
                                         L.ptr(z_p), len(probs), L.ptr(p_dev), L.ptr(mean), L.ptr(std),
                                         L.ptr(quant) if probs else None, L.stream_ptr()), "npf_mixture_summary")
    return mean, std, quant


SCORE_NAMES = ("log_density", "pit", "crps")


def check_want(want) -> tuple:
    if isinstance(want, str) or not isinstance(want, (tuple, list)):
        raise ValueError(f"want must be a tuple / list of names out of {SCORE_NAMES}, got {want!r}")
    for w in want:
        if w not in SCORE_NAMES:
            raise ValueError(f"want: unknown score {w!r} (known: {SCORE_NAMES})")
    if not want:
        raise ValueError(f"want must name at least one of {SCORE_NAMES}")
    return tuple(want)


def mixture_score(suff: torch.Tensor, Y: torch.Tensor, n_z: int, dy: int, homoskedastic: bool, n_valid: Optional[torch.Tensor] = None,
                  want=SCORE_NAMES):
    want = check_want(want)
    if not suff.is_cuda or suff.dtype != torch.float32 or not Y.is_cuda or Y.dtype != torch.float32:
        raise RuntimeError("the HIP path takes fp32 device tensors only; there is no CPU fallback")
    n_rows, pts, two_dy = suff.shape
    if two_dy != 2 * dy or n_z < 1 or n_rows % n_z != 0:
        raise ValueError(f"suff of shape {tuple(suff.shape)} does not hold n_z={n_z} samples of a {dy}-dimensional head")
    if n_z > MIXTURE_MAX_NZ:
        raise NotImplementedError(f"mixture_score covers up to {MIXTURE_MAX_NZ} latent samples (got {n_z})")
    B = n_rows // n_z
    if tuple(Y.shape) != (B, pts, dy):
        raise ValueError(f"Y must have shape [B={B}, pts={pts}, dy={dy}], got {tuple(Y.shape)}")
    suff, Y = suff.detach().contiguous(), Y.detach().contiguous()
    nv = counts_i32(n_valid, B) if n_valid is not None else None
    out = [torch.empty((B, pts, dy), dtype=torch.float32, device=suff.device) if name in want else None for name in SCORE_NAMES]
    L.check(L.load().npf_mixture_score(L.ptr(suff), L.ptr(Y), _iptr(nv) if nv is not None else None, n_z, B, pts, dy,
                                       int(homoskedastic), L.ptr(out[0]), L.ptr(out[1]), L.ptr(out[2]), L.stream_ptr()),
            "npf_mixture_score")
    return tuple(out)


MATCH_NAMES = ("hh", "gg", "overlap", "match", "mismatch", "tau_index", "phase")
MATCH_JC = 16
MATCH_MAX_TAU = 65536
_MATCH_WS = {}


class WaveformMatch(NamedTuple):
    hh: Optional[torch.Tensor]
    gg: Optional[torch.Tensor]
    overlap: Optional[torch.Tensor]
    match: Optional[torch.Tensor]
    mismatch: Optional[torch.Tensor]
    tau_index: Optional[torch.Tensor]
    phase: Optional[torch.Tensor]
    corr: Optional[torch.Tensor]


def check_match_want(want) -> tuple:
    if isinstance(want, str) or not isinstance(want, (tuple, list)):
        raise ValueError(f"want must be a tuple / list of names out of {MATCH_NAMES}, got {want!r}")
    for w in want:
        if w not in MATCH_NAMES:
            raise ValueError(f"want: unknown entry {w!r} (known: {MATCH_NAMES})")
    return tuple(want)


def check_taus(taus, have_freqs: bool):
    if taus is None:
        return None
    if isinstance(taus, torch.Tensor) or not isinstance(taus, (tuple, list)) or len(taus) != 3:
        raise ValueError(f"taus must be None or a host triple (tau0, dtau, n_tau), got {taus!r}")
    if not have_freqs:
        raise ValueError("taus (a time-shift grid) needs freqs, the physical frequency of every point")
    t0, dt, n = taus
    if any(isinstance(v, (torch.Tensor, bool)) or not isinstance(v, (int, float)) for v in (t0, dt)) \
            or isinstance(n, bool) or not isinstance(n, int):
        raise ValueError(f"taus = (tau0, dtau, n_tau) takes two host floats and a host int, got {taus!r}")
    if n < 1 or n > MATCH_MAX_TAU:
        raise ValueError(f"taus: n_tau must lie in [1, {MATCH_MAX_TAU}], got {n} (no time maximisation: taus=None)")
    tau0, dtau = float(t0), float(dt)
    if not (math.isfinite(tau0) and math.isfinite(dtau)):
        raise ValueError(f"taus: tau0 and dtau must be finite, got {tau0}, {dtau}")
    return tau0, dtau, n


def check_match_args(h_shape, g, weights=None, freqs=None, taus=None, what="g (the reference waveforms)"):
    h_shape = tuple(h_shape)
    if len(h_shape) != 3 or h_shape[2] < 2 or h_shape[0] < 1 or h_shape[1] < 1:
        raise ValueError(f"h must have shape [R, T, >= 2] (amplitude, phase first), got {list(h_shape)}")
    R, T, ld = h_shape
    if not isinstance(g, torch.Tensor) or g.dim() != 3 or g.shape[0] < 1 or tuple(g.shape[1:]) != (T, 2):
        raise ValueError(f"{what} must have shape [B, T={T}, 2], got "
                         f"{list(g.shape) if isinstance(g, torch.Tensor) else type(g).__name__}")
    B = g.shape[0]
    if R % B != 0:
        raise ValueError(f"h holds {R} rows, g {B} tasks: R % B != 0 (row k * B + b is latent sample k of task b)")

    def rows_of(t, what):
        if t is None:
            return 1
        if not isinstance(t, torch.Tensor) or tuple(t.shape) not in ((T,), (B, T)):
            raise ValueError(f"{what} must be None or a tensor of shape [T={T}] or [B={B}, T={T}], got "
                             f"{list(t.shape) if isinstance(t, torch.Tensor) else type(t).__name__}")
        return 1 if t.dim() == 1 else B

    wgt_rows, freq_rows = rows_of(weights, "weights"), rows_of(freqs, "freqs")
    taus = check_taus(taus, freqs is not None)
    tau0, dtau, n_tau = taus if taus is not None else (0.0, 0.0, 0)
    return R, T, ld, B, wgt_rows, freq_rows, tau0, dtau, n_tau


def _match_workspace(device: torch.device, n_bytes: int) -> torch.Tensor:
    idx = device.index if device.index is not None else torch.cuda.current_device()
    held = _MATCH_WS.setdefault(idx, [])
    need = (n_bytes + 7) // 8
    if not held or held[-1].numel() < need:
        if torch.cuda.is_current_stream_capturing():
            raise RuntimeError("waveform_match: the workspace has to grow, which cannot happen during graph capture; call once at "
                               "these sizes before capturing")
        held.append(torch.empty((max(need, 2 * held[-1].numel() if held else 0),), dtype=torch.float64, device=device))
    return held[-1]


def waveform_match(h: torch.Tensor, g: torch.Tensor, weights: Optional[torch.Tensor] = None, freqs: Optional[torch.Tensor] = None,
                   taus=None, n_valid: Optional[torch.Tensor] = None, want=MATCH_NAMES, corr: bool = False) -> WaveformMatch:
    want = check_match_want(want)
    R, T, ld, B, wgt_rows, freq_rows, tau0, dtau, n_tau = check_match_args(getattr(h, "shape", ()), g, weights, freqs, taus)
    if not want and not corr:
        raise ValueError(f"want must name at least one of {MATCH_NAMES} (or corr=True)")
    for t in (h, g, weights, freqs):
        if t is not None and (not t.is_cuda or t.dtype != torch.float32):
            raise RuntimeError("the HIP path takes fp32 device tensors only; there is no CPU fallback")
    h, g = h.detach().contiguous(), g.detach().contiguous()
    weights = weights.detach().contiguous() if weights is not None else None
    freqs = freqs.detach().contiguous() if freqs is not None and n_tau > 0 else None
    nv = counts_i32(n_valid, B) if n_valid is not None else None
    return _match_launch(h, g, weights, freqs, nv, (R, T, ld, B, wgt_rows, freq_rows, tau0, dtau, n_tau), want, corr, None)


def _match_launch(h, g, weights, freqs, nv, geo, want, corr, saved) -> WaveformMatch:
    R, T, ld, B, wgt_rows, freq_rows, tau0, dtau, n_tau = geo
    lib = L.load()
    ws = _match_workspace(h.device, int(lib.npf_waveform_match_workspace_bytes(R, n_tau)))
    new = lambda n, dtype=torch.float32: torch.empty((n,), dtype=dtype, device=h.device)
    out = {name: (new(B if name == "gg" else R, torch.int32 if name == "tau_index" else torch.float32) if name in want else None)
           for name in MATCH_NAMES}
    c = torch.empty((R, max(n_tau, 1), 2), dtype=torch.float32, device=h.device) if corr else None
    args = (L.ptr(h), ld, L.ptr(g), L.ptr(weights), wgt_rows, L.ptr(freqs), freq_rows, _iptr(nv) if nv is not None else None, R, B, T,
            tau0, dtau, n_tau, *(out[name].data_ptr() if out[name] is not None else None for name in MATCH_NAMES), L.ptr(c),
            ws.data_ptr())
    if saved is None:
        L.check(lib.npf_waveform_match(*args, L.stream_ptr()), "npf_waveform_match")
    else:
        L.check(lib.npf_waveform_match_ex(*args, saved.data_ptr(), L.stream_ptr()), "npf_waveform_match_ex")
    return WaveformMatch(*(out[name] for name in MATCH_NAMES), c)

# ... 646 lines not shown
```

npf_gwwaveform_amd/neuralproc.py:

```python
from __future__ import annotations

import abc
import math
from functools import partial
from typing import NamedTuple, Optional, Tuple

import torch
import torch.nn as nn
from torch.distributions import Independent, Normal

from . import functional as FN
from .architectures import (MLP, DotAttender, KeyWeights, LeaveOneOut, MergeFlatInputs, MultiheadAttender, PrefixTail, SelfAttention,
                            TrainKeyWeights, as_key_rule, get_attender, merge_flat_input)
from .chain import Chain, PTensor, pad32, pt_shape

__all__ = ["NeuralProcessFamily", "LatentNeuralProcessFamily", "CNP", "LNP", "AttnCNP", "AttnLNP",
           "MultivariateNormalDiag", "HeadDistribution", "Conditioned", "Prediction", "Score", "Match", "LogLike", "NetworkLogLike", "Reweighted", "bootstrap_weights",
           "kfold_weights"]


def MultivariateNormalDiag(loc, scale_diag):
    if loc.dim() < 1:
        raise ValueError("loc must be at least one-dimensional.")
    return Independent(Normal(loc, scale_diag, validate_args=False), 1)
# ... 339 lines not shown
    def kfold(self, folds, k) -> HeadDistribution:
        m = self._model
        m._refuse_kfold()
        rows = self._rows()
        k = _check_folds(folds, k, self.B, rows)
        Xc_pt, R_pts, n = self._row_tensors("kfold")
        if folds.device != R_pts.t.device:
            raise ValueError(f"folds lives on {folds.device}, the conditioned state on {R_pts.t.device}")
        with torch.no_grad():
            if n is None:
                n = torch.full((self.B,), rows, dtype=torch.int32, device=folds.device)
            return m._kfold_from(Xc_pt, R_pts, n, folds, k, self.B, rows)

    def _function_sampler(self, X_trgt, n_samples, eps, chunk):
        m = self._model
        m._refuse_unimplemented("sample_functions")
        if self.z_samples is not None and self.z_samples.shape[0] != 1:
            raise ValueError(f"sample_functions draws one trajectory per sample: condition with n_z_samples=1 (got {self.z_samples.shape[0]})")
        if X_trgt.dim() != 3 or X_trgt.shape[0] != self.B or X_trgt.shape[2] != m.x_dim:
            raise ValueError(f"X_trgt must be [B={self.B}, T, x_dim={m.x_dim}], got {list(X_trgt.shape)}")
        T = X_trgt.shape[1]
        if T == 0:
            raise ValueError("X_trgt holds no target points")
        S = int(n_samples)
        if S < 1:
            raise ValueError(f"n_samples must be at least 1, got {n_samples}")
        if eps is not None and tuple(eps.shape) != (S, self.B, T, m.y_dim):
            raise ValueError(f"eps must be [S={S}, B={self.B}, T={T}, y_dim={m.y_dim}], got {list(eps.shape)}")
        chunk = int(chunk)
        if chunk < 1:
            raise ValueError(f"chunk must be at least 1, got {chunk}")
        padded_kind = self.capacity is not None or (self.n_cntxt is not None and self.C > 0)
        if self._fused_t and not padded_kind:
            raise ValueError("sample_functions: this context was stored for the fused target side (images of keys / values only); "
                             "condition with counts (n_cntxt=...) or a capacity (condition_with_capacity)")
        m._check_tensors(X_trgt, eps)
        if eps is None:
            eps = torch.randn(S, self.B, T, m.y_dim, device=X_trgt.device)
        with torch.no_grad():
            return _FunctionSampler(self, S, T, X_trgt.device), eps, chunk

    def sample_functions(self, X_trgt, n_samples, eps=None, chunk=1) -> torch.Tensor:
        sampler, eps, chunk = self._function_sampler(X_trgt, n_samples, eps, chunk)
        S, B, T = sampler.S, self.B, X_trgt.shape[1]
        m = self._model
        Y = torch.empty(S, B, T, m.y_dim, device=X_trgt.device)
        with torch.no_grad():
            for t0 in range(0, T, chunk):
                x = X_trgt[:, t0:t0 + chunk]
                n = x.shape[1]
                x = x.unsqueeze(0).expand(S, B, n, m.x_dim).reshape(S * B, n, m.x_dim)
                y = sampler.step(x, eps[:, :, t0:t0 + chunk].reshape(S * B, n, m.y_dim))
                Y[:, :, t0:t0 + chunk] = y.view(S, B, n, m.y_dim)
        return Y


def tail_capacity(T: int) -> int:
    return pad32(T)


def pooled_mean_of_two(mean_p, n_p, mean_t, n_t):
    n_p, n_t = n_p.to(mean_p.dtype).unsqueeze(-1), n_t.to(mean_t.dtype).unsqueeze(-1)
    return (n_p * mean_p + n_t * mean_t) / (n_p + n_t).clamp(min=1)


class _FunctionSampler:

    def __init__(self, post: "Conditioned", S: int, T: int, device):
        m = post._model
        self.post, self.m, self.S, self.B, self.SB = post, m, S, post.B, S * post.B
        B, r = post.B, m.r_dim
        self.c_pad = post.C if post.capacity is None else post.capacity
        self.m_tail = tail_capacity(T)
        if post.n_cntxt is not None:
            self.n_pre = post.n_cntxt
        else:
            self.n_pre = torch.full((B,), self.c_pad, dtype=torch.int32, device=device)
        self.n_tail = torch.zeros(self.SB, dtype=torch.int32, device=device)
        zeros = lambda n, pts, F: torch.zeros(pt_shape(n, pts, F), device=device)
        att = getattr(m, "attender", None)
        latent = post.z_samples is not None
        self.keep_R = not m._attentive or isinstance(att, DotAttender) or latent
        self.R_tail = zeros(self.SB, self.m_tail, r) if self.keep_R else None
        self.tails = [(self.R_tail, r)] if self.keep_R else []
        if m._attentive:
            Xc = post._Xc_pt.t if post._Xc_pt is not None else zeros(B, 0, m.x_transf_dim)
            R = post._R.t if post._R is not None else zeros(B, 0, r)
            if isinstance(att, DotAttender):
                self.K_tail = zeros(self.SB, self.m_tail, m.x_transf_dim)
                self.tails.append((self.K_tail, m.x_transf_dim))
                self.walk = PrefixTail(Xc, R, self.n_pre, self.K_tail, self.R_tail, self.n_tail, B, self.c_pad, self.m_tail)
            else:
                H, d = att.n_heads, att.kq_size
                if self.c_pad > 0:
                    Kh = FN.split_heads(att._project(Xc, B, self.c_pad, att.key_transform), B, self.c_pad, d, H)
                    Vh = FN.split_heads(att._project(R, B, self.c_pad, att.value_transform), B, self.c_pad, att.value_size, H)
                else:
                    Kh, Vh = zeros(H * B, 0, d // H), zeros(H * B, 0, att.value_size // H)
                self.K_tail, self.V_tail = zeros(self.SB, self.m_tail, d), zeros(self.SB, self.m_tail, att.value_size)
                self.tails += [(self.K_tail, d), (self.V_tail, att.value_size)]
                self.walk = PrefixTail(Kh, Vh, self.n_pre, self.K_tail, self.V_tail, self.n_tail, H * B, self.c_pad, self.m_tail,
                                       heads_of_prefix=H)
            self.mean_pre = FN.masked_mean(R, self.n_pre, B, self.c_pad, r)[:, :r] if (latent and self.c_pad > 0) \
                else torch.zeros(B, r, device=device)
        else:
            self.walk = None
            self.mean_pre = post._R.reshape(B, r)
        self.eps_z = None
        if latent:
            if post.eps is not None:
                eps = post.eps
            else:
                q = post.q_zCc.base_dist
                eps = (post.z_samples - q.loc) / q.scale
            self.eps_z = eps[0].repeat(S, 1, 1)

    def _pooled(self):
        m, r = self.m, self.m.r_dim
        mean_t = FN.masked_mean(self.R_tail, self.n_tail, self.SB, self.m_tail, r)[:, :r]
        n_p = self.n_pre.clamp(0, self.c_pad).repeat(self.S)
        return pooled_mean_of_two(self.mean_pre.repeat(self.S, 1), n_p, mean_t, self.n_tail).reshape(self.SB, 1, r)

    def step(self, x, eps):
        m, SB = self.m, self.SB
        n = x.shape[1]
        Xt_pt = m._xenc_pt(x)
        z = None
        R = None
        if self.eps_z is not None or not m._attentive:
            R = self._pooled()
        if self.eps_z is not None:
            q = m._latent_dist_from(R).base_dist
            z = (q.loc + q.scale * self.eps_z).unsqueeze(0)
        C = self.c_pad + self.m_tail
        if m._attentive:
            suff = m._target_suffstat(None, z, None, Xt_pt, SB, C, n, n_valid=self.walk)
        else:
            suff = m._target_suffstat(None, z, R, Xt_pt, SB, C, n)
        p = m._head(suff, None, SB, n).base_dist
        y = p.loc[0] + p.scale[0] * eps
        Xn_pt, Rn_pts = m._encode_points(x, y)
        src = [Rn_pts.t] if self.keep_R else []
        if m._attentive:
            att = m.attender
            if isinstance(att, DotAttender):
                src.append(Xn_pt.t)
            else:
                src += [att._project(Xn_pt.t, SB, n, att.key_transform), att._project(Rn_pts.t, SB, n, att.value_transform)]
        FN.append_points([(s, dst, F) for s, (dst, F) in zip(src, self.tails)], self.n_tail, None, SB, n, self.m_tail)
        return y


class Reweighted:

    def __init__(self, post: "Conditioned", W, Xc_pt, R_pts, n, rows):
        self.post, self.W, self.S, self.B, self.rows = post, W, W.shape[0], post.B, rows
        self._Xc_pt, self._R_pts, self.n_cntxt = Xc_pt, R_pts, n

    def _eps(self):
        post = self.post
        if post.eps is not None:
            eps = post.eps
        else:
            q = post.q_zCc.base_dist
            eps = (post.z_samples - q.loc) / q.scale
        return eps.repeat(1, self.S, 1, 1)

    def query(self, X_trgt, n_trgt=None) -> HeadDistribution:
        post, m, S, B, rows = self.post, self.post._model, self.S, self.B, self.rows
        SB, r = S * B, m.r_dim
        with torch.no_grad():
            if n_trgt is not None:
                n_trgt = m._check_counts(n_trgt, X_trgt, "n_trgt").repeat(S)
            m._check_tensors(X_trgt)
            if X_trgt.dim() != 3 or X_trgt.shape[0] != B:
                raise ValueError(f"X_trgt must be [B={B}, T, x_dim] (the batch the model was conditioned on), got {list(X_trgt.shape)}")
            T = X_trgt.shape[1]
            if T == 0:
                raise ValueError("no target points")
            Xt_pt = m._xenc_pt(X_trgt)
            z = Rw = None
            if post.z_samples is not None or not m._attentive:
                Rw = FN.weighted_mean(self._R_pts.t, self.W, self.n_cntxt, SB, B, rows, r)[:, :r].reshape(SB, 1, r)
            if post.z_samples is not None:
                q = m._latent_dist_from(Rw).base_dist
                z = q.loc.unsqueeze(0) + q.scale.unsqueeze(0) * self._eps()
            if m._attentive:
                Xt_rep = PTensor(Xt_pt.t.repeat(S, 1, 1, 1, 1), T, m.x_transf_dim) if S > 1 else Xt_pt
                suff = m._target_suffstat(self._Xc_pt, z, self._R_pts, Xt_rep, SB, rows, T,
                                          n_valid=KeyWeights(self.W, self.n_cntxt, S), n_q_valid=n_trgt)
            else:
                vec = Rw.reshape(SB, r) if z is None else m._rep_rows(z, Rw, SB)
                suff = m._decode_taskvec(Xt_pt, vec.contiguous(), B, T, vec.shape[0])
            return m._head(suff, None, SB, T, n_trgt=n_trgt)


def bootstrap_weights(n_cntxt_or_C, S, rows, generator=None, device=None, n_tasks=1) -> torch.Tensor:
    S, rows = int(S), int(rows)
    if S < 1 or rows < 1:
        raise ValueError(f"bootstrap_weights needs S >= 1 and rows >= 1, got {S} and {rows}")
    if isinstance(n_cntxt_or_C, torch.Tensor):
        n = n_cntxt_or_C
        if n.dim() != 1 or n.is_floating_point() or n.dtype == torch.bool:
            raise ValueError(f"the counts must be an integer tensor [B], got {n.dtype} {list(n.shape)}")
        device = n.device if device is None else torch.device(device)
        n = n.to(device)
    else:
        n = torch.full((int(n_tasks),), int(n_cntxt_or_C), dtype=torch.int32, device=device)
        device = n.device
    B = n.shape[0]
    n = n.clamp(0, rows).view(1, B, 1)
    u = torch.rand(S, B, rows, generator=generator, device=device)
    idx = (u * n).long().minimum((n - 1).clamp(min=0).long())
    drawn = (torch.arange(rows, device=device).view(1, 1, rows) < n).to(torch.float32).expand(S, B, rows)
    return torch.zeros(S, B, rows, dtype=torch.float32, device=device).scatter_add_(2, idx, drawn.contiguous())


def _check_folds(folds, k, B, rows) -> int:
    k = int(k)
    if k < 2:
        raise ValueError(f"k must be at least 2 folds, got {k}")
    if not isinstance(folds, torch.Tensor) or folds.is_floating_point() or folds.dtype == torch.bool:
        raise ValueError(f"folds must be an integer tensor [B={B}, rows={rows}] of fold ids in [0, k), got "
                         f"{folds.dtype if isinstance(folds, torch.Tensor) else type(folds).__name__}")
    if tuple(folds.shape) != (B, rows):
        raise ValueError(f"folds must be [B={B}, rows={rows}] (one fold id per stored context row), got {list(folds.shape)}")
    return k


def kfold_weights(folds, k) -> torch.Tensor:
    return (folds.unsqueeze(0) != torch.arange(int(k), device=folds.device, dtype=folds.dtype).view(-1, 1, 1)).to(torch.float32)


def _mean_rows(R_pt, pts, B, r, n_valid=None):
    if isinstance(n_valid, TrainKeyWeights):
        m = FN.key_weighted_mean(R_pt, n_valid.w, n_valid.n_valid, B, pts, r)
    else:
        m = FN.mean_agg(R_pt, pts, r) if n_valid is None else FN.masked_mean(R_pt, n_valid, B, pts, r)
    return m[:, :r].reshape(B, 1, r)


def _q_z_scale(z_scale):
    return 0.1 + 0.9 * torch.sigmoid(z_scale)


class NeuralProcessFamily(nn.Module, abc.ABC):

    _valid_paths = ["deterministic", "latent", "both"]

    def __init__(self, x_dim, y_dim, encoded_path, r_dim=128, x_transf_dim=-1, is_heteroskedastic=True, XEncoder=None,
                 Decoder=None, PredictiveDistribution=MultivariateNormalDiag, p_y_loc_transformer=None,
                 p_y_scale_transformer=None):
        super().__init__()
        self.x_dim, self.y_dim, self.r_dim = x_dim, y_dim, r_dim
        self.is_heteroskedastic = is_heteroskedastic
        if x_transf_dim is None:
            self.x_transf_dim = self.x_dim
        elif x_transf_dim == -1:
            self.x_transf_dim = self.r_dim
        else:
            self.x_transf_dim = x_transf_dim
        self.encoded_path = encoded_path.lower()
        if self.encoded_path not in self._valid_paths:
            raise ValueError(f"Unknown encoded_path={self.encoded_path}.")
        if PredictiveDistribution is not MultivariateNormalDiag or p_y_loc_transformer is not None \
                or p_y_scale_transformer is not None:
            raise NotImplementedError("the HIP Gaussian head implements the reference defaults only: diagonal "
                                      "Gaussian, identity loc, scale = 0.01 + 0.99 softplus (base.py:114-116)")
        if XEncoder is None:
            XEncoder = self.dflt_Modules["XEncoder"]
        if Decoder is None:
            Decoder = self.dflt_Modules["Decoder"]
        self.x_encoder = XEncoder(self.x_dim, self.x_transf_dim)
        self.decoder = Decoder(self.x_transf_dim, self.r_dim, self.y_dim * 2)
        if not isinstance(self.x_encoder, MLP) or not isinstance(self.decoder, MergeFlatInputs):
            raise NotImplementedError("the HIP path needs the stock MLP XEncoder and merge_flat_input(MLP) Decoder")
        if max(self.x_dim, 2 * self.y_dim) > 32:
            raise NotImplementedError("x_dim and 2*y_dim are limited to 32 on the hot path")
        self.PredictiveDistribution = PredictiveDistribution
        self.p_y_loc_transformer = nn.Identity()
        self.validate_inputs = True

    def reset_parameters(self):
        pass

    @property
    def dflt_Modules(self):
        d = dict()
        d["XEncoder"] = partial(MLP, n_hidden_layers=1, hidden_size=self.r_dim)
        d["SubDecoder"] = partial(MLP, n_hidden_layers=4, hidden_size=self.r_dim)
        d["Decoder"] = merge_flat_input(d["SubDecoder"], is_sum_merge=True)
        return d

    def forward(self, X_cntxt, Y_cntxt, X_trgt, Y_trgt=None, n_cntxt=None, n_trgt=None):
        return self._forward_weighted(X_cntxt, Y_cntxt, X_trgt, Y_trgt, n_cntxt=n_cntxt, n_trgt=n_trgt)

    def _forward_weighted(self, X_cntxt, Y_cntxt, X_trgt, Y_trgt=None, n_cntxt=None, n_trgt=None, w_cntxt=None):
        if n_cntxt is not None:
            n_cntxt = self._check_counts(n_cntxt, X_cntxt, "n_cntxt")
        if n_trgt is not None:
            n_trgt = self._check_counts(n_trgt, X_trgt, "n_trgt")
        if w_cntxt is not None:
            w_cntxt = self._check_weights(w_cntxt, X_cntxt)
        self._validate_inputs(X_cntxt, Y_cntxt, X_trgt, Y_trgt)
        B, C, _ = X_cntxt.shape
        T = X_trgt.shape[1]
        if T == 0:
            raise ValueError("no target points")
        if w_cntxt is not None and C > 0:
            full = n_cntxt if n_cntxt is not None else torch.full((B,), C, dtype=torch.int32, device=X_cntxt.device)
            n_cntxt = TrainKeyWeights(w_cntxt, full)
        fused_t = self._fused_target_side(C, T)
        Xc_pt, R = self._context_stage(X_cntxt, Y_cntxt, n_cntxt, fused_t)
        return self._target_stage(Xc_pt, R, X_trgt, Y_trgt, B, C, n_cntxt, n_trgt, fused_t)

    def influence(self, X_cntxt, Y_cntxt, X_trgt, Y_trgt, n_cntxt=None, n_trgt=None) -> torch.Tensor:
        self._refuse_weights()
        B, C, _ = X_cntxt.shape
        w = torch.ones((B, C), dtype=torch.float32, device=X_cntxt.device, requires_grad=True)
        if C == 0:
            return w.detach()
        was = self.training
        self.eval()
        try:
            with torch.enable_grad():
                p_yCc = self(X_cntxt, Y_cntxt, X_trgt, Y_trgt, n_cntxt=n_cntxt, n_trgt=n_trgt, w_cntxt=w)[0]
                ll = p_yCc.sum_log_prob(Y_trgt)
                (g,) = torch.autograd.grad(ll.sum(), w)
        finally:
            self.train(was)
        return g

    def _context_stage(self, X_cntxt, Y_cntxt, n_cntxt, fused_t):
        from . import chain as _chain

        B, C, _ = X_cntxt.shape
        if n_cntxt is not None and C > 0:
            if self._fused_context_side(C):
                from . import x6

                Xc_pt, R_pts = x6.context_side(self, X_cntxt, Y_cntxt)
                return Xc_pt, self._pool_pt(R_pts, B, n_valid=n_cntxt)
            Xc_pt = self._xenc_pt(X_cntxt)
            return Xc_pt, self._encode_globally_pt(Xc_pt, Y_cntxt, B, C, n_valid=n_cntxt)
        fused_c = self._fused_context_side(C)
        if fused_c and self._attentive and not fused_t and _chain.COMPUTE_DTYPE == "bf16":
            fused_c = False
        if fused_c:
            from . import x6

            Xc_pt, R_pts = x6.context_side(self, X_cntxt, Y_cntxt)
            return Xc_pt, self._pool_pt(R_pts, B)
        Xc_pt = self._xenc_pt(X_cntxt, with_tr=self._attentive and not fused_t) if C > 0 else None
        return Xc_pt, self._encode_globally_pt(Xc_pt, Y_cntxt, B, C)

    def _target_stage(self, Xc_pt, R, X_trgt, Y_trgt, B, C, n_cntxt, n_trgt, fused_t, latent=None):
        T = X_trgt.shape[1]
        padded = n_cntxt is not None and C > 0
        n_valid = n_cntxt if padded else None
        X_raw = None
        if padded:
            Xt_pt = self._xenc_pt(X_trgt)
        elif fused_t:
            Xt_pt, X_raw = None, X_trgt
        elif self._xenc_with_query_projection(C, T):
            from . import x6

            Xt_pt, q_proj = x6.xenc_proj(self, X_trgt, self.attender.query_transform)
            Xt_pt.proj = q_proj
        else:
            Xt_pt = self._xenc_pt(X_trgt)
        self._X_trgt_raw = X_raw
        try:
            if latent is not None:
                z_samples, q_zCc, q_zCct = latent[0], latent[1], None
            elif self.encoded_path in ["latent", "both"]:
                z_samples, q_zCc, q_zCct = self._latent_path_pt(R, C, Xt_pt, Y_trgt, B, T, n_valid=n_valid, n_trgt=n_trgt)
            else:
                z_samples, q_zCc, q_zCct = None, None, None
            if self.encoded_path == "latent":
                R = None
            suff = self._target_suffstat(Xc_pt, z_samples, R, Xt_pt, B, C, T, n_valid=n_valid,
                                         n_q_valid=n_trgt if padded else None)
        finally:
            self._X_trgt_raw = None
        return self._head(suff, Y_trgt, B, T, n_trgt=n_trgt), z_samples, q_zCc, q_zCct

    def _n_z_for(self, n_z_samples=None) -> Optional[int]:
        return None

    def condition(self, X_cntxt, Y_cntxt, n_cntxt=None, n_z_samples=None) -> "Conditioned":
        with torch.no_grad():
            n_z = self._n_z_for(n_z_samples)
            if n_cntxt is not None:
                n_cntxt = self._check_counts(n_cntxt, X_cntxt, "n_cntxt")
            self._check_tensors(X_cntxt, Y_cntxt)
            B, C, _ = X_cntxt.shape
            if n_z is not None:
                self.n_z_samples = n_z
            fused_t = self._fused_target_side(C, 1)
            R_pts = None
            if not self._attentive and C > 0 and not getattr(self, "is_self_attn", False):
                Xc_pt, R_pts = self._encode_points(X_cntxt, Y_cntxt)
                R = self._pool_pt(R_pts, B, n_valid=n_cntxt)
            else:
                Xc_pt, R = self._context_stage(X_cntxt, Y_cntxt, n_cntxt, fused_t)
            z_samples = q_zCc = None
            if n_z is not None:
                q_zCc = self._infer_q_zCc(R, B, n_cntxt if C > 0 else None)
                z_samples = q_zCc.rsample([n_z])
        return Conditioned(self, Xc_pt, R, z_samples, q_zCc, n_cntxt, B, C, fused_t, R_pts=R_pts)

    def condition_with_capacity(self, X_cntxt, Y_cntxt, capacity, n_cntxt=None, n_z_samples=None) -> "Conditioned":
        self._refuse_unimplemented("capacity")
        with torch.no_grad():
            n_z = self._n_z_for(n_z_samples)
            if X_cntxt.dim() != 3 or Y_cntxt.dim() != 3 or X_cntxt.shape[:2] != Y_cntxt.shape[:2]:
                raise ValueError(f"X_cntxt / Y_cntxt must be [B, C, x_dim] / [B, C, y_dim], got {list(X_cntxt.shape)} / {list(Y_cntxt.shape)}")
            B, C, _ = X_cntxt.shape
            capacity = int(capacity)
            if capacity < max(C, 1):
                raise ValueError(f"capacity={capacity} must be at least the context size C={C} (and at least 1)")
            self._check_tensors(X_cntxt, Y_cntxt)
            if n_cntxt is not None:
                n_cntxt = self._check_counts(n_cntxt, X_cntxt, "n_cntxt")
            if n_z is not None:
                self.n_z_samples = n_z
            dev = X_cntxt.device
            R_pts = PTensor(torch.zeros(pt_shape(B, capacity, self.r_dim), device=dev), capacity, self.r_dim)
            Xc_pt = PTensor(torch.zeros(pt_shape(B, capacity, self.x_transf_dim), device=dev), capacity, self.x_transf_dim)
            counts = torch.zeros(B, dtype=torch.int32, device=dev)
            post = Conditioned(self, Xc_pt, R_pts if self._attentive else torch.zeros(B, 1, self.r_dim, device=dev), None, None, counts,
                               B, C, False, capacity=capacity, R_pts=R_pts)
            if C > 0:
                Xn_pt, Rn_pts = self._encode_points(X_cntxt, Y_cntxt)
                pairs = [(Rn_pts.t, R_pts.t, self.r_dim), (Xn_pt.t, Xc_pt.t, self.x_transf_dim)]
                FN.append_points(pairs, counts, n_cntxt, B, C, capacity)
            post._refresh()
            if n_z is not None:
                post.q_zCc = q = self._infer_q_zCc(post._R, B, counts)
                post.eps = torch.randn(n_z, B, 1, self.z_dim, device=dev)
                post.z_samples = q.base_dist.loc + q.base_dist.scale * post.eps
        return post

    def loo(self, X_cntxt, Y_cntxt, n_cntxt=None) -> HeadDistribution:
        self._refuse_loo()
        if X_cntxt.dim() != 3 or Y_cntxt.dim() != 3 or X_cntxt.shape[:2] != Y_cntxt.shape[:2]:
            raise ValueError(f"X_cntxt / Y_cntxt must be [B, C, x_dim] / [B, C, y_dim], got {list(X_cntxt.shape)} / {list(Y_cntxt.shape)}")
        B, C, _ = X_cntxt.shape
        if C == 0:
            raise ValueError("loo: no context points")
        with torch.no_grad():
            if n_cntxt is not None:
                n_cntxt = self._check_counts(n_cntxt, X_cntxt, "n_cntxt")
            self._check_tensors(X_cntxt, Y_cntxt)
            if n_cntxt is None:
                n_cntxt = torch.full((B,), C, dtype=torch.int32, device=X_cntxt.device)
            Xc_pt, R_pts = self._encode_points(X_cntxt, Y_cntxt)
            return self._loo_from(Xc_pt, R_pts, n_cntxt, B, C)

    def _refuse_loo(self):
        if self.encoded_path != "deterministic":
            raise NotImplementedError("loo is not implemented for latent models (LNP / AttnLNP): q(z | C without i) differs per "
                                      "left-out point and the decoder takes one z per task")
        self._refuse_unimplemented("loo")

    def _loo_from(self, Xc_pt, R_pts, n, B, rows) -> HeadDistribution:
        return self._head(self._loo_suffstat(Xc_pt, R_pts, n, B, rows), None, B, rows, n_trgt=n)

    def kfold(self, X_cntxt, Y_cntxt, folds, k, n_cntxt=None) -> HeadDistribution:
        self._refuse_kfold()
        if X_cntxt.dim() != 3 or Y_cntxt.dim() != 3 or X_cntxt.shape[:2] != Y_cntxt.shape[:2]:
            raise ValueError(f"X_cntxt / Y_cntxt must be [B, C, x_dim] / [B, C, y_dim], got {list(X_cntxt.shape)} / {list(Y_cntxt.shape)}")
        B, C, _ = X_cntxt.shape
        if C == 0:
            raise ValueError("kfold: no context points")
        k = _check_folds(folds, k, B, C)
        with torch.no_grad():
            if n_cntxt is not None:
                n_cntxt = self._check_counts(n_cntxt, X_cntxt, "n_cntxt")
            self._check_tensors(X_cntxt, Y_cntxt)
            if folds.device != X_cntxt.device:
                raise ValueError(f"folds lives on {folds.device}, the batch on {X_cntxt.device}")
            if n_cntxt is None:
                n_cntxt = torch.full((B,), C, dtype=torch.int32, device=X_cntxt.device)
            Xc_pt, R_pts = self._encode_points(X_cntxt, Y_cntxt)
            return self._kfold_from(Xc_pt, R_pts, n_cntxt, folds, k, B, C)

    def _refuse_kfold(self):
        if self.encoded_path != "deterministic":
            raise NotImplementedError("kfold is not implemented for latent models (LNP / AttnLNP): q(z | C without the fold) differs "
                                      "per fold and the decoder takes one z per task; use Conditioned.reweighted with the fold masks")
        self._refuse_unimplemented("kfold")

    def _kfold_from(self, Xc_pt, R_pts, n, folds, k, B, rows) -> HeadDistribution:
        own = folds.long().clamp(0, k - 1)
        R_g = self._kfold_rep(Xc_pt, R_pts, n, kfold_weights(own, k), own, k, B, rows)
        return self._head(self._decode_pointwise(R_g, Xc_pt.t, B, rows), None, B, rows, n_trgt=n)

    def _decode_pointwise(self, R_t, X1_pt, B, T):
        from . import x6

        if x6.decoder_side_usable(self, T):
            return x6.decoder_side(self, R_t, X1_pt, T)
        ch = Chain(B, T, X1_pt.device, wg_per_task=True)
        ch.input_pt(R_t, self.r_dim)
        return self.decoder.finish_rows(ch, x1_pt=X1_pt)

    def _encode_points(self, X, Y):
        if self._fused_context_side(X.shape[1]):
            from . import x6

            return x6.context_side(self, X, Y)
        X_pt = self._xenc_pt(X)
        return X_pt, self._xyenc_pt(X_pt, Y, with_tr=False)

    def predict(self, X_cntxt, Y_cntxt, X_trgt, n_cntxt=None, n_trgt=None, n_z_samples=None, probs=(0.025, 0.5, 0.975)) -> Prediction:
        probs = FN.check_probs(probs)
        return self.condition(X_cntxt, Y_cntxt, n_cntxt=n_cntxt, n_z_samples=n_z_samples).query(X_trgt, n_trgt=n_trgt).summary(probs)

    def _refuse_unimplemented(self, what):
        from . import chain as _chain

        if getattr(self, "is_self_attn", False):
            raise NotImplementedError(f"{what} is not implemented for self-attention context encoders (is_self_attn=True)")
        if _chain.COMPUTE_DTYPE != "fp32":
            raise NotImplementedError(f"{what} is not implemented in the bf16 compute mode (set_compute_dtype('bf16'))")

    def _refuse_weights(self):
        self._refuse_unimplemented("w_cntxt")
        if isinstance(self, LatentNeuralProcessFamily):
            raise NotImplementedError("w_cntxt is not implemented for the latent models (LNP / AttnLNP): q(z | C, T) would need a rule "
                                      "for the weights of the targets")

    def _check_weights(self, w, X):
        self._refuse_weights()
        B, C = X.shape[0], X.shape[1]
        if not isinstance(w, torch.Tensor) or not w.is_floating_point():
            raise ValueError(f"w_cntxt must be a float device tensor of shape [{B}, {C}], got "
                             f"{w.dtype if isinstance(w, torch.Tensor) else type(w).__name__}")
        if tuple(w.shape) != (B, C):
            raise ValueError(f"w_cntxt must have shape [{B}, {C}] (one weight per context point), got {list(w.shape)}")
        if w.device != X.device:
            raise ValueError(f"w_cntxt lives on {w.device}, the batch on {X.device}")
        return w.to(torch.float32).contiguous()

    def _check_counts(self, n, X, what):
        self._refuse_unimplemented(what)
        n = FN.counts_i32(n, X.shape[0], what)
        if n.device != X.device:
            raise ValueError(f"{what} lives on {n.device}, the batch on {X.device}")
        return n

    def _validate_inputs(self, X_cntxt, Y_cntxt, X_trgt, Y_trgt):
        self._check_tensors(X_cntxt, Y_cntxt, X_trgt, Y_trgt)
        if self.training and self.validate_inputs:
            m = X_trgt.abs().amax() if X_trgt.numel() else X_trgt.new_zeros(())
            if X_cntxt.numel():
                m = torch.maximum(m, X_cntxt.abs().amax())
            if self.validate_inputs == "deferred":
                if getattr(self, "_range_seen", None) is None or self._range_seen.device != m.device:
                    self._range_seen = torch.zeros((), device=m.device)
                self._range_seen.copy_(torch.maximum(self._range_seen, m))
                return
            if not (m.item() <= 1.0):
                lo = min(X_cntxt.min().item() if X_cntxt.numel() else 0.0, X_trgt.min().item())
                hi = max(X_cntxt.max().item() if X_cntxt.numel() else 0.0, X_trgt.max().item())
                raise ValueError(f"Features during training should be in [-1,1]. Got [{lo}, {hi}].")

    @staticmethod
    def _check_tensors(*tensors):
        for t in tensors:
            if t is not None and (not t.is_cuda or t.dtype != torch.float32):
                raise RuntimeError("the HIP path takes fp32 device tensors only; there is no CPU fallback")

    def check_deferred_inputs(self):
        seen = getattr(self, "_range_seen", None)
        if seen is None:
            return
        worst = seen.item()
        seen.zero_()
        if not (worst <= 1.0):
            raise ValueError(f"Features during training should be in [-1,1]. Got max |x| = {worst}.")

    _attentive = False

    def _fused_target_side(self, C, T) -> bool:
        return False

    def _xenc_with_query_projection(self, C, T) -> bool:
        from . import x6

        att = getattr(self, "attender", None)
        if not (self._attentive and isinstance(att, MultiheadAttender) and C > 0):
            return False
        return FN.mha_usable(att.kq_head_size, att.value_head_size, C) and x6.xenc_proj_usable(self, att.query_transform, T)

    def _fused_context_side(self, C) -> bool:
        from . import x6

        return hasattr(self, "xy_encoder") and hasattr(self, "_pool_pt") and x6.context_side_usable(self, C)

    def _xenc_pt(self, X, with_tr=False) -> PTensor:
        B, P, dx = X.shape
        ch = Chain(B, P, X.device)
        ch.input_rows(X.contiguous(), dx)
        return self.x_encoder.append_to(ch).run_pt(as_weights=with_tr)

    def _xyenc_pt(self, X_enc: PTensor, Y, with_tr: Optional[bool] = None) -> PTensor:
        ch = Chain(X_enc.n_tasks, X_enc.pts, Y.device)
        ch.input_rows(Y.contiguous(), self.y_dim)
        return self.xy_encoder.run_pt(ch, X_enc.t, X_enc.n_tasks, X_enc.pts,
                                      with_tr=self._attentive if with_tr is None else with_tr)

    def _head(self, suff, Y_trgt, B, T, n_trgt=None):
        return HeadDistribution(suff, self.y_dim, not self.is_heteroskedastic, suff.shape[0] // B, B, T, n_trgt=n_trgt)

    def _decode_taskvec(self, Xt_pt, vec, B, T, n_rows):
        ch = Chain(n_rows, T, Xt_pt.t.device)
        ch.input_pt(Xt_pt.t, self.x_transf_dim, modulus=(B if n_rows != B else 0))
        return self.decoder.finish_rows(ch, taskvec=vec)

    @abc.abstractmethod
    def encode_globally(self, X_cntxt, Y_cntxt):
        pass

    @abc.abstractmethod
    def trgt_dependent_representation(self, X_cntxt, z_samples, R, X_trgt):
        pass

    def latent_path(self, X_cntxt, R, X_trgt, Y_trgt):
        raise NotImplementedError(
            f"`latent_path` not implemented. Cannot use encoded_path={self.encoded_path} in such case.")

    def decode(self, X_trgt, R_trgt):
        n_z, B, T, _ = R_trgt.shape
        suff = self.decoder(X_trgt, R_trgt).reshape(n_z * B, T, 2 * self.y_dim)
        return self._head(suff, None, B, T)

    def set_extrapolation(self, min_max):
        pass


class LatentNeuralProcessFamily(NeuralProcessFamily):

    _valid_paths = ["latent", "both"]

    def __init__(self, *args, is_q_zCct=False, n_z_samples_train=32, n_z_samples_test=32, LatentEncoder=None,
                 LatentDistribution=MultivariateNormalDiag, q_z_loc_transformer=None, q_z_scale_transformer=None,
                 z_dim=None, **kwargs):
        super().__init__(*args, **kwargs)
        self.is_q_zCct = is_q_zCct
        self.n_z_samples_train, self.n_z_samples_test = n_z_samples_train, n_z_samples_test
        self.z_dim = self.r_dim if z_dim is None else z_dim
        if LatentEncoder is None:
            LatentEncoder = self.dflt_Modules["LatentEncoder"]
        self.latent_encoder = LatentEncoder(self.r_dim, self.z_dim * 2)
        if self.encoded_path == "both":
            self.r_z_merger = nn.Linear(self.r_dim + self.z_dim, self.r_dim)
        self.LatentDistribution = LatentDistribution
        self.q_z_loc_transformer = nn.Identity() if q_z_loc_transformer is None else q_z_loc_transformer
        self.q_z_scale_transformer = _q_z_scale if q_z_scale_transformer is None else q_z_scale_transformer
        if self.z_dim != self.r_dim and self.encoded_path == "latent":
            self.reshaper_z = nn.Linear(self.z_dim, self.r_dim)

    @property
    def dflt_Modules(self):
        d = NeuralProcessFamily.dflt_Modules.__get__(self)
        d["LatentEncoder"] = partial(MLP, n_hidden_layers=1, hidden_size=self.r_dim)
        return d

    def forward(self, *args, **kwargs):
        self.n_z_samples = self._n_z_for()
        return super().forward(*args, **kwargs)

    def _n_z_for(self, n_z_samples=None) -> int:
        if n_z_samples is not None:
            if int(n_z_samples) < 1:
                raise ValueError(f"n_z_samples must be at least 1, got {n_z_samples}")
            return int(n_z_samples)
        try:
            return self.n_z_samples_train.rvs() if self.training else self.n_z_samples_test.rvs()
        except AttributeError:
            return self.n_z_samples_train if self.training else self.n_z_samples_test

    def infer_latent_dist(self, X, R):
        R_lat_inp = self.rep_to_lat_input(R)
        return self._latent_dist_from(R_lat_inp)

    def _latent_dist_from(self, R_lat_inp):
        suff = self.latent_encoder(R_lat_inp)
        q_z_loc, q_z_scale = suff.split(self.z_dim, dim=-1)
        return self.LatentDistribution(self.q_z_loc_transformer(q_z_loc), self.q_z_scale_transformer(q_z_scale))

    def rep_to_lat_input(self, R):
        return R

    def latent_path(self, X_cntxt, R, X_trgt, Y_trgt):
        q_zCc = self.infer_latent_dist(X_cntxt, R)
        if self.is_q_zCct and Y_trgt is not None:
            R_from_trgt = self.encode_globally(X_trgt, Y_trgt)
            q_zCct = self.infer_latent_dist(X_trgt, R_from_trgt)
            sampling_dist = q_zCct
        else:
            q_zCct, sampling_dist = None, q_zCc
        return sampling_dist.rsample([self.n_z_samples]), q_zCc, q_zCct

    def _infer_q_zCc(self, R, B, n_valid=None):
        return self._latent_dist_from(self._lat_input(R, B, n_valid=n_valid))

    def _latent_path_pt(self, R, C, Xt_pt, Y_trgt, B, T, n_valid=None, n_trgt=None):
        q_zCc = self._infer_q_zCc(R, B, n_valid)
        if self.is_q_zCct and Y_trgt is not None:
            if Xt_pt is None:
                if self._fused_context_side(T):
                    from . import x6

                    R_t = self._pool_pt(x6.context_side(self, self._X_trgt_raw, Y_trgt)[1], B, n_valid=n_trgt)
                else:
                    R_t = self._encode_globally_pt(self._xenc_pt(self._X_trgt_raw), Y_trgt, B, T, n_valid=n_trgt)
            else:
                R_t = self._encode_globally_pt(Xt_pt, Y_trgt, B, T, n_valid=n_trgt)
            q_zCct = self._latent_dist_from(self._lat_input(R_t, B, n_valid=n_trgt))
            sampling_dist = q_zCct
        else:
            q_zCct, sampling_dist = None, q_zCc
        return sampling_dist.rsample([self.n_z_samples]), q_zCc, q_zCct

    def merge_r_z(self, R, z_samples):
        if R.shape != z_samples.shape:
            R = R.unsqueeze(0).expand(*z_samples.shape[:-1], self.r_dim)
        lead = z_samples.shape[:-1]
        rows = int(math.prod(lead))
        out = self._merge_rows(R.reshape(rows, self.r_dim), z_samples.reshape(rows, self.z_dim))
        return out.reshape(*lead, self.r_dim)

    def _merge_rows(self, R_rows, z_rows):
        rows = R_rows.shape[0]
        W, b, r = self.r_z_merger.weight, self.r_z_merger.bias, self.r_dim
        ch = Chain(1, rows, R_rows.device)
        ch.input_pt(FN.pack_pt(z_rows.reshape(1, rows, self.z_dim)), self.z_dim).linear(W[:, r:], b).output_pt()
        (zb,) = ch.run()
        ch = Chain(1, rows, R_rows.device)
        ch.input_pt(FN.pack_pt(R_rows.reshape(1, rows, r)), r).linear(W[:, :r], None, relu=True, addend=zb).output_pt()
        return FN.unpack_pt(ch.run()[0], rows, r).reshape(rows, r)


class CNP(NeuralProcessFamily):

    _valid_paths = ["deterministic"]

    def __init__(self, x_dim, y_dim, XYEncoder=None, **kwargs):
        kwargs["encoded_path"] = kwargs.get("encoded_path", "deterministic")
        super().__init__(x_dim, y_dim, **kwargs)
        if XYEncoder is None:
            XYEncoder = self.dflt_Modules["XYEncoder"]
        self.xy_encoder = XYEncoder(self.x_transf_dim, self.y_dim, self.r_dim)
        if not isinstance(self.xy_encoder, MergeFlatInputs):
            raise NotImplementedError("the HIP path needs the stock merge_flat_input(MLP) XYEncoder")

    @property
    def dflt_Modules(self):
        d = NeuralProcessFamily.dflt_Modules.__get__(self)
        sub = partial(MLP, n_hidden_layers=2, is_force_hid_smaller=True, hidden_size=self.r_dim)
        d["XYEncoder"] = merge_flat_input(sub, is_sum_merge=True)
        return d

    forward = NeuralProcessFamily._forward_weighted

    def encode_globally(self, X_cntxt, Y_cntxt):
        B, C, _ = X_cntxt.shape
        if C == 0:
            return torch.zeros(B, 1, self.r_dim, device=X_cntxt.device)
        return self._encode_globally_pt(PTensor(FN.pack_pt(X_cntxt), C, self.x_transf_dim), Y_cntxt, B, C)

    def trgt_dependent_representation(self, _, __, R, X_trgt):
        B, T, _ = X_trgt.shape
        return R.expand(B, T, self.r_dim).unsqueeze(0)

    def _encode_globally_pt(self, X_enc, Y, B, P, n_valid=None):
        if P == 0:
            return torch.zeros(B, 1, self.r_dim, device=Y.device)
        return self._pool_pt(self._xyenc_pt(X_enc, Y), B, n_valid=n_valid)

    def _pool_pt(self, R_pts: PTensor, B, n_valid=None):
        return _mean_rows(R_pts.t, R_pts.pts, B, self.r_dim, n_valid)

    def _target_suffstat(self, Xc_pt, z_samples, R, Xt_pt, B, C, T, n_valid=None, n_q_valid=None):
        return self._decode_taskvec(Xt_pt, R.reshape(B, self.r_dim), B, T, B)

    def _loo_suffstat(self, Xc_pt, R_pts, n, B, rows):
        return self._decode_pointwise(FN.loo_mean(R_pts.t, n, B, rows, self.r_dim), Xc_pt.t, B, rows)

    def _kfold_rep(self, Xc_pt, R_pts, n, W, own, k, B, rows):
        r = self.r_dim
        means = FN.weighted_mean(R_pts.t, W, n, k * B, B, rows, r)[:, :r].view(k, B, r)
        return FN.pack_pt(means[own, torch.arange(B, device=own.device).view(B, 1)])


class LNP(LatentNeuralProcessFamily, CNP):

    _valid_paths = ["latent", "both"]

    def __init__(self, x_dim, y_dim, encoded_path="latent", **kwargs):
        super().__init__(x_dim, y_dim, encoded_path=encoded_path, **kwargs)

    def _lat_input(self, R, B, n_valid=None):
        return R

    def _rep_rows(self, z_samples, R, B):
        n_z = z_samples.size(0)
        if self.encoded_path == "both":
            R_trgt = self.merge_r_z(R, z_samples)
        else:
            R_trgt = z_samples
            if self.z_dim != self.r_dim:
                R_trgt = _rows_mlp_linear(self.reshaper_z, R_trgt)
        return R_trgt.reshape(n_z * B, self.r_dim)

    def trgt_dependent_representation(self, _, z_samples, R, X_trgt):
        B, T, _ = X_trgt.shape
        n_z = z_samples.size(0)
        return self._rep_rows(z_samples, R, B).reshape(n_z, B, 1, self.r_dim).expand(n_z, B, T, self.r_dim)

    def _target_suffstat(self, Xc_pt, z_samples, R, Xt_pt, B, C, T, n_valid=None, n_q_valid=None):
        n_z = z_samples.size(0)
        return self._decode_taskvec(Xt_pt, self._rep_rows(z_samples, R, B), B, T, n_z * B)


def _rows_mlp_linear(lin: nn.Linear, x: torch.Tensor) -> torch.Tensor:
    lead = x.shape[:-1]
    rows = int(math.prod(lead))
    ch = Chain(1, rows, x.device)
    ch.input_pt(FN.pack_pt(x.reshape(1, rows, x.shape[-1])), x.shape[-1]).linear(lin.weight, lin.bias).output_pt()
    return FN.unpack_pt(ch.run()[0], rows, lin.out_features).reshape(*lead, lin.out_features)


class AttnCNP(NeuralProcessFamily):

    _valid_paths = ["deterministic"]
    _attentive = True

    def __init__(self, x_dim, y_dim, XYEncoder=None, attention="scaledot", attention_kwargs={},
                 self_attention_kwargs={}, is_self_attn=False, **kwargs):
        kwargs["encoded_path"] = kwargs.get("encoded_path", "deterministic")
        super().__init__(x_dim, y_dim, **kwargs)
        self.is_self_attn = is_self_attn
        if is_self_attn:
            XYEncoder = merge_flat_input(SelfAttention, is_sum_merge=True, **self_attention_kwargs)
        elif XYEncoder is None:
            XYEncoder = self.dflt_Modules["XYEncoder"]
        self.xy_encoder = XYEncoder(self.x_transf_dim, self.y_dim, self.r_dim)
        if not isinstance(self.xy_encoder, MergeFlatInputs):
            raise NotImplementedError("the HIP path needs the stock merge_flat_input(MLP) XYEncoder")
        self.attender = get_attender(attention, self.x_transf_dim, self.r_dim, self.r_dim, **attention_kwargs)
        if not isinstance(self.attender, (DotAttender, MultiheadAttender)):
            raise NotImplementedError("the HIP path implements attention = 'scaledot', 'multihead', 'transformer'")

    dflt_Modules = CNP.dflt_Modules
    forward = NeuralProcessFamily._forward_weighted

    def _fused_target_side(self, C, T) -> bool:
        from . import x6

        return type(self) is AttnCNP and self.encoded_path == "deterministic" and x6.target_side_usable(self, C, T)

    def encode_globally(self, X_cntxt, Y_cntxt):
        B, C, _ = X_cntxt.shape
        if C == 0:
            return torch.zeros(B, 0, self.r_dim, device=X_cntxt.device)
        return self.xy_encoder(X_cntxt, Y_cntxt)
# ... 166 lines not shown
```

npf_gwwaveform_amd/x6.py:

```python
from __future__ import annotations

import ctypes as C
import math
import os
from typing import List, Optional, Sequence

import torch

from . import _lib as L
from . import chain as CH
from . import functional as FN

ENABLED = os.environ.get("NPF_NO_X6_FUSED", "0") != "1"
WIDTH = 256
VARIANT = int(os.environ.get("NPF_X6_VARIANT", "0"))
B16_ENABLED = os.environ.get("NPF_NO_B16_FUSED", "0") != "1"
B16_VARIANT = int(os.environ.get("NPF_B16_VARIANT", "0"))


class Program:

    def __init__(self, n_tasks: int, tiles: int, per_task: bool, width: int = WIDTH, pts: Optional[int] = None,
                 bf16: bool = False):
        self.n_tasks, self.tiles, self.per_task, self.width = n_tasks, tiles, per_task, width
        self.bf16 = bf16
        self.pts = tiles * 32 if pts is None else pts
        self.ops: List[dict] = []
        self.tail = None
        self.tag = ""

    def op(self, **kw) -> "Program":
        self.ops.append(kw)
        return self

    @staticmethod
    def _ptr(t, what):
        if t is None:
            return None
        if not t.is_cuda or not t.is_contiguous():
            raise RuntimeError(f"x6 program operand {what} must be a contiguous device tensor")
        return t.data_ptr()

    def _pt_ok(self, t, what, p16=False):
        want = (self.n_tasks, self.tiles, self.width // 8, 32, 8) if p16 else (self.n_tasks, self.tiles, self.width // 4, 32, 4)
        dt = torch.bfloat16 if p16 else torch.float32
        if t is not None and (tuple(t.shape) != want or t.dtype != dt):
            raise ValueError(f"x6 program operand {what}: {'PT16' if p16 else 'PT32'} tensor {tuple(t.shape)} {t.dtype}, "
                             f"expected {want} {dt}")

    def launch(self) -> None:
        if len(self.ops) > L.NPF_X6_MAX_OPS:
            raise RuntimeError(f"x6 program longer than NPF_X6_MAX_OPS={L.NPF_X6_MAX_OPS}")
        arr = (L.NpfX6Op * len(self.ops))()
        F, pts = self.width, self.n_tasks * self.tiles * 32
        flops = 0
        nbytes = 0
        for j, o in enumerate(self.ops):
            flags = 0
            for k in ("in_pt", "pre_add", "mask", "sbwd_p", "store_in", "addend", "store_out"):
                t = o.get(k)
                if t is not None and o.get(k + "_rm"):
                    if k not in ("in_pt", "addend") or tuple(t.shape) != (self.n_tasks, self.pts, F) or t.dtype != torch.float32:
                        raise ValueError(f"x6 program operand {k}: row-major tensor {tuple(t.shape)} {t.dtype}")
                    if self.bf16:
                        raise ValueError("b16 programs take no row-major operands")
                    flags |= L.X6_IN_RM if k == "in_pt" else L.X6_ADD_RM
                else:
                    p16 = self.bf16 and (k == "sbwd_p" or (k in ("store_in", "store_out") and not o.get(k + "_f32")))
                    if self.bf16 and k in ("store_in", "store_out") and o.get(k + "_f32") and t is not None:
                        flags |= L.X6_STORE_IN_F32 if k == "store_in" else L.X6_STORE_OUT_F32
                    if self.bf16 and k == "mask" and t is not None:
                        raise ValueError("b16 programs take ReLU masks as bits")
                    self._pt_ok(t, k, p16)
                setattr(arr[j], k, self._ptr(t, k))
                nbytes += pts * F * (t.element_size() if t is not None else 0)
            arr[j].reserved[0] = flags
            for k in ("mask_bits", "store_in_bits", "store_bits"):
                t = o.get(k)
                if t is not None and (tuple(t.shape) != (self.n_tasks, self.tiles, 2, 64) or t.dtype != torch.int64):
                    raise ValueError(f"x6 program operand {k}: bits tensor {tuple(t.shape)} {t.dtype}")
                setattr(arr[j], k, self._ptr(t, k))
                nbytes += pts * F // 8 if t is not None else 0
            if o.get("in_rows") is not None:
                rows, w, b = o["in_rows"], o["in_w"], o.get("in_b")
                n = w.shape[1]
                if tuple(rows.shape) != (self.n_tasks, self.tiles * 32, 4) or w.shape[0] != 4 or n % 16 or n > F:
                    raise ValueError(f"x6 rows prologue: rows {tuple(rows.shape)}, matrix {tuple(w.shape)}")
                if b is not None and tuple(b.shape) != (n,):
                    raise ValueError("x6 rows prologue: bias shape")
                arr[j].in_rows, arr[j].in_w, arr[j].in_b = L.ptr(rows), L.ptr(w), L.ptr(b)
                arr[j].in_n, arr[j].in_relu = n, int(bool(o.get("in_relu", False)))
                flops += 2 * 4 * n * pts
                nbytes += pts * 16
            img = o.get("img")
            if img is not None:
                per_task = bool(o.get("img_per_task", False))
                terms = (1,) if self.bf16 else (3,)
                want = ((self.n_tasks,) if per_task else ()) + (() if self.bf16 else (3,)) + (F, F)
                if tuple(img.shape) != want or img.dtype != torch.bfloat16 or not img.is_contiguous():
                    raise ValueError(f"x6 program weight image {tuple(img.shape)} {img.dtype}, expected {want} bfloat16")
                arr[j].w_img = img.data_ptr()
                arr[j].w_task_stride = terms[0] * F * F * 2 if per_task else 0
                bias = o.get("bias")
                if bias is not None:
                    bpt = bool(o.get("bias_per_task", False))
                    if tuple(bias.shape) != ((self.n_tasks, F) if bpt else (F,)):
                        raise ValueError(f"x6 program bias {tuple(bias.shape)}")
                    arr[j].bias = L.ptr(bias)
                    arr[j].bias_task_stride = F if bpt else 0
                arr[j].relu = int(bool(o.get("relu", False)))
                arr[j].softmax_n = int(o.get("softmax_n", 0))
                arr[j].softmax_scale = float(o.get("softmax_scale", 1.0))
                flops += 2 * o.get("true_k", F) * o.get("true_n", F) * pts
                nbytes += terms[0] * 2 * F * F * (self.n_tasks if per_task else 1)
            elif any(o.get(k) is not None for k in ("bias", "addend", "store_out", "store_bits")) or o.get("relu") or o.get("softmax_n"):
                raise ValueError("x6 program: an op without a multiply has no output side")
            arr[j].sbwd_scale = float(o.get("sbwd_scale", 1.0))
        tail = self.tail
        if tail is not None:
            flops += 2 * 4 * F * pts
            nbytes += pts * 16
        if CH.PROFILE is not None:
            ev0, ev1 = torch.cuda.Event(enable_timing=True), torch.cuda.Event(enable_timing=True)
            ev0.record()
        tw, tb, tr = (L.ptr(tail[0]) if tail else None, L.ptr(tail[1]) if (tail and tail[1] is not None) else None,
                      L.ptr(tail[2]) if tail else None)
        if self.bf16:
            if self.pts != self.tiles * 32:
                raise ValueError("b16 programs run on whole tiles")
            L.check(L.load().npf_b16_run(arr, len(self.ops), tw, tb, tr, self.n_tasks, self.tiles, int(self.per_task), F,
                                         B16_VARIANT, L.stream_ptr()), "npf_b16_run")
        else:
            L.check(L.load().npf_x6_run_ex(arr, len(self.ops), tw, tb, tr, self.n_tasks, self.tiles, self.pts, int(self.per_task), F,
                                           VARIANT if F in (256, 512) else 0, L.stream_ptr()), "npf_x6_run_ex")
        if CH.PROFILE is not None:
            ev1.record()
            CH.PROFILE.append(("b16_program_kernel" if self.bf16 else "x6_program_kernel", flops, ev0, ev1, nbytes, self.tag))
        if CH.TRACE is not None:
            CH.TRACE.append(("prog", self))


def task_images(pt: torch.Tensor, pts: int, row: bool = True, tr: bool = True, width: int = WIDTH, bf16: bool = False):
    n_tasks = pt.shape[0]
    if tuple(pt.shape) != (n_tasks, CH.tiles_of(pts), width // 4, 32, 4) or pts > width:
        raise ValueError(f"task_images: PT32 tensor {tuple(pt.shape)} for {pts} points x {width} features")
    shape = (n_tasks, width, width) if bf16 else (n_tasks, 3, width, width)
    mk = lambda: torch.empty(shape, dtype=torch.bfloat16, device=pt.device)
    ri, ti = (mk() if row else None), (mk() if tr else None)
    if CH.PROFILE is not None:
        ev0, ev1 = torch.cuda.Event(enable_timing=True), torch.cuda.Event(enable_timing=True)
        ev0.record()
    fn = L.load().npf_b16_task_images if bf16 else L.load().npf_x6_task_images
    L.check(fn(L.ptr(pt.detach().contiguous()), n_tasks, pts, width, ri.data_ptr() if row else None,
               ti.data_ptr() if tr else None, L.stream_ptr()), "npf_x6_task_images")
    if CH.PROFILE is not None:
        ev1.record()
        CH.PROFILE.append(("x6_task_images_kernel", 0, ev0, ev1,
                           pt.numel() * 4 + (int(row) + int(tr)) * n_tasks * (1 if bf16 else 3) * width * width * 2))
    return ri, ti


def _weight_images(Ws: Sequence[torch.Tensor], kinds: Sequence[int], width: int = WIDTH, bf16: bool = False) -> List[List[torch.Tensor]]:
    if bf16:
        n = len(Ws)
        buf = torch.empty((len(kinds), n, width, width), dtype=torch.bfloat16, device=Ws[0].device)
        CH.prepare_weights([(Ws[i].detach(), kind) for kind in kinds for i in range(n)],
                           dsts=[buf[k, i] for k in range(len(kinds)) for i in range(n)])
        return [[buf[k, i] for i in range(n)] for k in range(len(kinds))]
    from .mlp_x6 import _three_term_images

    return _three_term_images(Ws, kinds, width)


def _r16(t: Optional[torch.Tensor]) -> Optional[torch.Tensor]:
    return None if t is None else t.to(torch.bfloat16).to(torch.float32)


def _bits(n_tasks, tiles, dev):
    return torch.empty((n_tasks, tiles, 2, 64), dtype=torch.int64, device=dev)


_ZEROS = {}


def _zeros(shape, device) -> torch.Tensor:
    key = (tuple(shape), str(device))
    z = _ZEROS.get(key)
    if z is None:
        z = torch.zeros(shape, dtype=torch.float32, device=device)
        if not (z.is_cuda and torch.cuda.is_current_stream_capturing()):
            _ZEROS[key] = z
    return z


def _pad_rows4(X: torch.Tensor) -> torch.Tensor:
    d = X.shape[-1]
    if d == 4:
        return X.contiguous()
    return torch.cat((X, _zeros((*X.shape[:-1], 4 - d), X.device)), dim=-1)


def _first_layer_matrix(W: torch.Tensor, n_out: int) -> torch.Tensor:
    n, d = W.shape
    Wt = W.detach().t()
    if n < n_out:
        Wt = torch.cat((Wt, _zeros((d, n_out - n), W.device)), dim=1)
    if d < 4:
        Wt = torch.cat((Wt, _zeros((4 - d, n_out), W.device)), dim=0)
    return Wt.contiguous()


def decode_rows_usable(mod, x1: torch.Tensor, x2: torch.Tensor) -> bool:
    from .architectures import MLP

    if not (ENABLED and CH.COMPUTE_DTYPE == "fp32" and mod.is_sum_merge and isinstance(mod.flat_module, MLP)):
        return False
    F = x1.shape[-1]
    fm, rs = mod.flat_module, mod.resizer
    if F not in (128, 256, 512) or x2.shape[-1] != F or x1.shape[:-1] != x2.shape[:-1] or fm.is_res or rs.is_res:
        return False
    if any(m.dropout_p > 0 and m.training for m in (fm, rs)):
        return False
    if not (_square(rs.layers(), F) and _square([fm.to_hidden, *fm.linears], F) and fm.out.in_features == F
            and fm.out.out_features <= 4):
        return False
    return len(rs.layers()) + len(fm.linears) + 1 <= L.NPF_X6_MAX_OPS and x1.shape[-2] > 0


def decode_rows(mod, x1: torch.Tensor, x2: torch.Tensor) -> torch.Tensor:
    n, T, F = x1.shape
    fm, rs = mod.flat_module, mod.resizer
    lins = [*rs.layers(), fm.to_hidden, *fm.linears]
    imgs = _weight_images([l.weight for l in lins], (1,), F)[0]
    tiles = CH.tiles_of(T)
    prog = Program(n, tiles, per_task=False, width=F, pts=T)
    n_res = len(rs.layers())
    for i, lin in enumerate(lins):
        o = dict(img=imgs[i], bias=lin.bias.detach() if lin.bias is not None else None, relu=True)
        if i == 0:
            o.update(in_pt=x2.detach().contiguous(), in_pt_rm=True)
        if i == n_res - 1:
            o.update(addend=x1.detach().contiguous(), addend_rm=True)
        prog.op(**o)
    rows = torch.empty((n, tiles * 32, 4), dtype=torch.float32, device=x1.device)
    Wo, bo = _pad_out(fm.out.weight, fm.out.bias)
    prog.tail = (Wo, bo, rows)
    prog.tag = f"decode (merge + {F}-wide decoder + output layer) from row-major inputs"
    prog.launch()
    return rows[:, :T, :fm.out.out_features]


def _pad_out(W: torch.Tensor, b: Optional[torch.Tensor]):
    n = W.shape[0]
    if n == 4:
        return W.detach().contiguous(), (b.detach().contiguous() if b is not None else None)
    Wp = torch.zeros((4, W.shape[1]), dtype=torch.float32, device=W.device)
    Wp[:n] = W.detach()
    bp = None
    if b is not None:
        bp = torch.zeros((4,), dtype=torch.float32, device=W.device)
        bp[:n] = b.detach()
    return Wp, bp


class _TargetSideFn(torch.autograd.Function):

    @staticmethod
    def forward(ctx, X, K_pt, V_pt, C, scale, spec, zb, *params):
        n_x, n_mrz, n_res, n_flat = spec
        B, T, dx = X.shape
        dev = X.device
        tiles = T // 32
        Ws, bs = list(params[0::2]), list(params[1::2])
        W1, b1 = Ws[0], bs[0]
        W_out, b_out = Ws[-1], bs[-1]
        n_out = W_out.shape[0]
        mid_W, mid_b = Ws[1:-1], bs[1:-1]
        F = mid_W[0].shape[0]
        if n_mrz:
            mid_b[n_x] = zb
        train = any(ctx.needs_input_grad)
        bf16 = CH.COMPUTE_DTYPE == "bf16"
        imgs = _weight_images(mid_W, (1, 2) if train else (1,), F, bf16)
        fw = imgs[0]
        K_row, K_tr = task_images(K_pt, C, row=True, tr=train, width=F, bf16=bf16)
        V_row, V_tr = task_images(V_pt, C, row=train, tr=True, width=F, bf16=bf16)
        X4 = _pad_rows4(X.detach())
        W1p = _first_layer_matrix(W1, F)
        if bf16:
            X4, W1p = _r16(X4), _r16(W1p)
        pt = lambda: CH.pt_empty(B, T, F, dev)
        pb = (lambda: CH.pt16_empty(B, T, F, dev)) if bf16 else pt
        prog = Program(B, tiles, per_task=True, width=F, bf16=bf16)
        saved_acts, saved_bits = [], []
        h1 = pb() if train else None
        bits_h1 = _bits(B, tiles, dev) if train else None
        Xt_enc = pt()
        for i in range(n_x):
            last = i == n_x - 1
            o = dict(img=fw[i], w_ref=("shared", mid_W[i]), bias=mid_b[i].detach() if mid_b[i] is not None else None, relu=not last)
            if i == 0:
                o.update(in_rows=X4, in_w=W1p, in_b=b1.detach() if b1 is not None else None, in_relu=True, store_in=h1,
                         store_in_bits=bits_h1)
            if last:
                o["store_out"], o["store_out_f32"] = Xt_enc, True
            elif train:
                o["store_out"], o["store_bits"] = pb(), _bits(B, tiles, dev)
                saved_acts.append(o["store_out"])
                saved_bits.append(o["store_bits"])
            prog.op(**o)
        P = pb() if train else None
        prog.op(img=K_row, w_ref=("task_row", K_pt, C), img_per_task=True, softmax_n=C, softmax_scale=scale, store_out=P, true_n=C)
        R_trgt = pb() if train else None
        prog.op(img=V_tr, w_ref=("task_tr", V_pt, C), img_per_task=True, store_out=R_trgt, true_k=C)
        for i in range(n_mrz + n_res + n_flat):
            j = n_x + i
            o = dict(img=fw[j], w_ref=("shared", mid_W[j]), bias=mid_b[j].detach().contiguous() if mid_b[j] is not None else None,
                     relu=True, bias_per_task=bool(n_mrz and i == 0))
            if i == n_mrz + n_res - 1:
                o["addend"] = Xt_enc
            if train:
                o["store_out"], o["store_bits"] = pb(), _bits(B, tiles, dev)
                saved_acts.append(o["store_out"])
                saved_bits.append(o["store_bits"])
            prog.op(**o)
        rows = torch.empty((B, T, 4), dtype=torch.float32, device=dev)
        Wo, bo = _pad_out(W_out, b_out)
        if bf16:
            Wo = _r16(Wo)
        prog.tail = (Wo, bo, rows)
        prog.tag = "target side forward (x-encoder, attention, decoder, output layer)"
        prog.launch()
        ctx.geom = (B, T, tiles, dx, C, float(scale), n_out, F)
        ctx.spec, ctx.bf16 = spec, bf16
        ctx.trace_ref = ([W.detach() for W in mid_W], K_pt, V_pt) if CH.TRACE is not None else None
        ctx.has_b = [b is not None for b in bs]
        ctx.set_materialize_grads(False)
        if train:
            ctx.n_acts, ctx.n_bits = len(saved_acts), len(saved_bits)
            ctx.save_for_backward(X4, h1, bits_h1, Xt_enc, P, R_trgt, *saved_acts, *saved_bits, *imgs[1], V_row, K_tr, Wo)
        return rows[..., :n_out] if n_out != 4 else rows

    @staticmethod
    def backward(ctx, g):
        n_x, n_mrz, n_res, n_flat = ctx.spec
        n_dec = n_mrz + n_res + n_flat
        n_mid = n_x + n_dec
        n_par = 2 * (n_mid + 2)
        if g is None:
            return (None,) * (7 + n_par)
        B, T, tiles, dx, C, scale, n_out, F = ctx.geom
        sv = list(ctx.saved_tensors)
        X4, h1, bits_h1, Xt_enc, P, R_trgt = sv[:6]
        acts = sv[6:6 + ctx.n_acts]
        bits = sv[6 + ctx.n_acts:6 + ctx.n_acts + ctx.n_bits]
        rest = sv[6 + ctx.n_acts + ctx.n_bits:]
        bw, (V_row, K_tr, Wo) = rest[:n_mid], rest[n_mid:]
        dev = g.device
        bf16 = ctx.bf16
        g4 = g.contiguous() if n_out == 4 else torch.nn.functional.pad(g, (0, 4 - n_out)).contiguous()
        if bf16:
            g4 = _r16(g4)
        pt = lambda: CH.pt_empty(B, T, F, dev)
        pb = (lambda: CH.pt16_empty(B, T, F, dev)) if bf16 else pt
        x_acts, x_bits = acts[:n_x - 1], bits[:n_x - 1]
        d_acts, d_bits = acts[n_x - 1:], bits[n_x - 1:]
        prog = Program(B, tiles, per_task=True, width=F, bf16=bf16)
        tr = ctx.trace_ref
        wref = lambda j: ("shared", tr[0][j].t()) if tr is not None else None
        dz = [None] * n_mid
        for i in range(n_dec - 1, -1, -1):
            j = n_x + i
            is_merge = i == n_mrz + n_res - 1 or (n_mrz and i == 0)
            dz[j] = pt() if is_merge else pb()
            o = dict(mask_bits=d_bits[i], store_in=dz[j], store_in_f32=is_merge, img=bw[j], w_ref=wref(j))
            if i == n_dec - 1:
                o.update(in_rows=g4, in_w=Wo)
            prog.op(**o)
        dO, dS = pb(), pb()
        prog.op(store_in=dO, img=V_row, w_ref=("task_row", tr[2], C) if tr is not None else None, img_per_task=True, true_n=C)
        prog.op(sbwd_p=P, sbwd_scale=scale, store_in=dS, img=K_tr, w_ref=("task_tr", tr[1], C) if tr is not None else None,
                img_per_task=True, addend=dz[n_x + n_mrz + n_res - 1], true_k=C)
        for i in range(n_x - 1, -1, -1):
            dz[i] = pb()
            o = dict(store_in=dz[i], img=bw[i], w_ref=wref(i))
            if i < n_x - 1:
                o["mask_bits"] = x_bits[i]
            prog.op(**o)
        dz1 = pb()
        prog.op(mask_bits=bits_h1, store_in=dz1)
        prog.tag = "target side dgrad (decoder, attention backward, x-encoder)"
        prog.launch()
        jobs, grads = [], []
        dW1p = torch.empty((F, 4), dtype=torch.float32, device=dev)
        db1 = torch.empty((F,), dtype=torch.float32, device=dev) if ctx.has_b[0] else None
        jobs.append(dict(dZ=dz1, A=FN._pack(X4), N=F, K=4, dW=dW1p, db=db1))
        grads += [None, db1]
        ins = [h1, *x_acts, R_trgt, *d_acts[:-1]]
        for j in range(n_mid):
            dW = torch.empty((F, F), dtype=torch.float32, device=dev)
            db = torch.empty((F,), dtype=torch.float32, device=dev) if (ctx.has_b[1 + j] and not (n_mrz and j == n_x)) else None
            jobs.append(dict(dZ=dz[j], A=ins[j], N=F, K=F, dW=dW, db=db))
            grads += [dW, db]
        dz_out = torch.zeros(CH.pt_shape(B, T, 4), dtype=torch.float32, device=dev)
        dz_out[:, :, 0] = g4.view(B, tiles, 32, 4)
        dWo = torch.empty((n_out, F), dtype=torch.float32, device=dev)
        dbo = torch.empty((n_out,), dtype=torch.float32, device=dev) if ctx.has_b[-1] else None
        jobs.append(dict(dZ=dz_out, A=d_acts[-1], N=n_out, K=F, dW=dWo, db=dbo))
        grads += [dWo, dbo]
        mk = torch.zeros if C % 32 else torch.empty
        dK = mk(CH.pt_shape(B, C, F), dtype=torch.float32, device=dev) if ctx.needs_input_grad[1] else None
        dV = mk(CH.pt_shape(B, C, F), dtype=torch.float32, device=dev) if ctx.needs_input_grad[2] else None
        if dV is not None:
            jobs.append(dict(dZ=P, A=dO, N=C, K=F, dW=dV, per_task=True, ldz=F))
        if dK is not None:
            jobs.append(dict(dZ=dS, A=Xt_enc, N=C, K=F, dW=dK, per_task=True, ldz=F))
        CH.run_wgrad(jobs, B, T, dev, tag="target side weight / key / value gradients")
        if CH.TRACE is not None:
            CH.TRACE.append(("wgrad", jobs, B, T, bf16))
        grads[0] = dW1p[:, :dx].contiguous() if dx != 4 else dW1p
        d_zb = FN.sum_points_pt(dz[n_x], T, F)[:, :F].contiguous() if (n_mrz and ctx.needs_input_grad[6]) else None
        return (None, dK, dV, None, None, None, d_zb, *grads)


class _DecoderSideFn(torch.autograd.Function):

    @staticmethod
    def forward(ctx, R_pt, X1_pt, T, spec, zb, *params):
        n_mrz, n_res, n_flat = spec
        B, tiles = R_pt.shape[0], R_pt.shape[1]
        dev = R_pt.device
        Ws, bs = list(params[0::2]), list(params[1::2])
        W_out, b_out = Ws[-1], bs[-1]
        n_out = W_out.shape[0]
        mid_W, mid_b = Ws[:-1], bs[:-1]
        F = mid_W[0].shape[0]
        n_mid = n_mrz + n_res + n_flat
        if n_mrz:
            mid_b[0] = zb
        train = any(ctx.needs_input_grad)
        imgs = _weight_images(mid_W, (1, 2) if train else (1,), F)
        fw = imgs[0]
        R_pt, X1_pt = R_pt.contiguous(), X1_pt.contiguous()
        pt = lambda: CH.pt_empty(B, tiles * 32, F, dev)
        prog = Program(B, tiles, per_task=bool(n_mrz), width=F)
        acts, bits = [], []
        for i in range(n_mid):
            o = dict(img=fw[i], w_ref=("shared", mid_W[i]), bias=mid_b[i].detach().contiguous() if mid_b[i] is not None else None,
                     relu=True, bias_per_task=bool(n_mrz and i == 0))
            if i == 0:
                o["in_pt"] = R_pt.detach()
            if i == n_mrz + n_res - 1:
                o["addend"] = X1_pt.detach()
            if train:
                o["store_out"], o["store_bits"] = pt(), _bits(B, tiles, dev)
                acts.append(o["store_out"])
                bits.append(o["store_bits"])
            prog.op(**o)
        rows = torch.empty((B, tiles * 32, 4), dtype=torch.float32, device=dev)
        Wo, bo = _pad_out(W_out, b_out)
        prog.tail = (Wo, bo, rows)
        prog.tag = "decoder forward (resizer, merge, flat MLP, output layer)"
        prog.launch()
        ctx.geom = (B, T, tiles, n_out, F)
        ctx.spec = spec
        ctx.has_b = [b is not None for b in bs]
        ctx.set_materialize_grads(False)
        ctx.trace_ref = [W.detach() for W in mid_W] if CH.TRACE is not None else None
        if train:
            ctx.save_for_backward(R_pt.detach(), *acts, *bits, *imgs[1], Wo)
        return rows[:, :T, :n_out]

    @staticmethod
    def backward(ctx, g):
        n_mrz, n_res, n_flat = ctx.spec
        n_mid = n_mrz + n_res + n_flat
        if g is None:
            return (None,) * (5 + 2 * (n_mid + 1))
        B, T, tiles, n_out, F = ctx.geom
        sv = list(ctx.saved_tensors)
        R_pt, acts, bits, bw, Wo = sv[0], sv[1:1 + n_mid], sv[1 + n_mid:1 + 2 * n_mid], sv[1 + 2 * n_mid:1 + 3 * n_mid], sv[-1]
        dev = g.device
        if T == tiles * 32 and n_out == 4:
            g4 = g.contiguous()
        else:
            g4 = torch.zeros((B, tiles * 32, 4), dtype=torch.float32, device=dev)
            g4[:, :T, :n_out] = g
        pt = lambda: CH.pt_empty(B, tiles * 32, F, dev)
        tr = ctx.trace_ref
        prog = Program(B, tiles, per_task=bool(n_mrz), width=F)
        dz = [None] * n_mid
        dR = pt() if ctx.needs_input_grad[0] else None
        for i in range(n_mid - 1, -1, -1):
            dz[i] = pt()
            o = dict(mask_bits=bits[i], store_in=dz[i], img=bw[i], w_ref=("shared", tr[i].t()) if tr is not None else None)
            if i == n_mid - 1:
                o.update(in_rows=g4, in_w=Wo)
            if i == 0 and dR is not None:
                o["store_out"] = dR
            prog.op(**o)
        prog.tag = "decoder dgrad"
        prog.launch()
        jobs, grads = [], []
        ins = [R_pt, *acts[:-1]]
        for j in range(n_mid):
            dW = torch.empty((F, F), dtype=torch.float32, device=dev)
            db = torch.empty((F,), dtype=torch.float32, device=dev) if (ctx.has_b[j] and not (n_mrz and j == 0)) else None
            jobs.append(dict(dZ=dz[j], A=ins[j], N=F, K=F, dW=dW, db=db))
            grads += [dW, db]
        dz_out = torch.zeros(CH.pt_shape(B, tiles * 32, 4), dtype=torch.float32, device=dev)
        dz_out[:, :, 0] = g4.view(B, tiles, 32, 4)
        dWo = torch.empty((n_out, F), dtype=torch.float32, device=dev)
        dbo = torch.empty((n_out,), dtype=torch.float32, device=dev) if ctx.has_b[-1] else None
        jobs.append(dict(dZ=dz_out, A=acts[-1], N=n_out, K=F, dW=dWo, db=dbo))
        grads += [dWo, dbo]
        CH.run_wgrad(jobs, B, tiles * 32, dev, tag="decoder weight gradients")
        if CH.TRACE is not None:
            CH.TRACE.append(("wgrad", jobs, B, tiles * 32, False))
        dX1 = dz[n_mrz + n_res - 1] if ctx.needs_input_grad[1] else None
        d_zb = FN.sum_points_pt(dz[0], tiles * 32, F)[:, :F].contiguous() if (n_mrz and ctx.needs_input_grad[4]) else None
        return (dR, dX1, None, None, d_zb, *grads)


def decoder_side_usable(model, T: int) -> bool:
    from .architectures import MLP, MergeFlatInputs

    if not (ENABLED and CH.COMPUTE_DTYPE == "fp32") or T <= 0:
        return False
    dec = getattr(model, "decoder", None)
    F = getattr(model, "r_dim", 0)
    if F != 128 or getattr(model, "x_transf_dim", F) != F or not isinstance(dec, MergeFlatInputs):
        return False
    if not (dec.is_sum_merge and isinstance(dec.flat_module, MLP)):
        return False
    fm, rs = dec.flat_module, dec.resizer
    for m in (fm, rs):
        if m.is_res or (m.dropout_p > 0 and m.training):
            return False
    if not (_square(rs.layers(), F) and _square([fm.to_hidden, *fm.linears], F) and fm.out.in_features == F
            and fm.out.out_features <= 4):
        return False
    return len(rs.layers()) + len(fm.linears) + 2 <= L.NPF_X6_MAX_OPS


def decoder_side(model, R_pt: torch.Tensor, X1_pt: torch.Tensor, T: int, zb: Optional[torch.Tensor] = None) -> torch.Tensor:
    dec = model.decoder
    fm, rs = dec.flat_module, dec.resizer
    lins = [*rs.layers(), fm.to_hidden, *fm.linears, fm.out]
    params = []
    for lin in lins:
        params += [lin.weight, lin.bias]
    if zb is not None:
        params[0:0] = [model.r_z_merger.weight[:, :model.r_dim], None]
    return _DecoderSideFn.apply(R_pt, X1_pt, T, (int(zb is not None), len(rs.layers()), len(fm.linears) + 1), zb, *params)


class _PairLinearFn(torch.autograd.Function):

    @staticmethod
    def forward(ctx, a_pt, b_pt, pts, Wa, Wb):
        B, tiles = a_pt.shape[0], a_pt.shape[1]
        F = Wa.shape[0]
        dev = a_pt.device
        train = any(ctx.needs_input_grad)
        imgs = _weight_images([Wa, Wb], (1, 2) if train else (1,), F)
        a_pt, b_pt = a_pt.contiguous(), b_pt.contiguous()
        oa, ob = CH.pt_empty(B, tiles * 32, F, dev), CH.pt_empty(B, tiles * 32, F, dev)
        prog = Program(B, tiles, per_task=False, width=F)
        prog.op(in_pt=a_pt.detach(), img=imgs[0][0], w_ref=("shared", Wa), store_out=oa)
        prog.op(in_pt=b_pt.detach(), img=imgs[0][1], w_ref=("shared", Wb), store_out=ob)
        prog.tag = "key / value projections"
        prog.launch()
        ctx.geom = (B, tiles, F, pts)
        ctx.set_materialize_grads(False)
        if train:
            ctx.save_for_backward(a_pt.detach(), b_pt.detach(), *imgs[1])
        return oa, ob

    @staticmethod
    def backward(ctx, ga, gb):
        if ga is None and gb is None:
            return (None,) * 5
        B, tiles, F, pts = ctx.geom
        a_pt, b_pt, ia, ib = ctx.saved_tensors
        dev = a_pt.device
        zeros = lambda: torch.zeros(CH.pt_shape(B, tiles * 32, F), dtype=torch.float32, device=dev)
        ga = ga.contiguous() if ga is not None else zeros()
        gb = gb.contiguous() if gb is not None else zeros()
        da, db = CH.pt_empty(B, tiles * 32, F, dev), CH.pt_empty(B, tiles * 32, F, dev)
        prog = Program(B, tiles, per_task=False, width=F)
        prog.op(in_pt=ga, img=ia, store_out=da)
        prog.op(in_pt=gb, img=ib, store_out=db)
        prog.tag = "key / value projections dgrad"
        prog.launch()
        dWa, dWb = (torch.empty((F, F), dtype=torch.float32, device=dev) for _ in range(2))
        CH.run_wgrad([dict(dZ=ga, A=a_pt, N=F, K=F, dW=dWa, db=None), dict(dZ=gb, A=b_pt, N=F, K=F, dW=dWb, db=None)], B, pts, dev,
                     tag="key / value projection weight gradients")
        return da, db, None, dWa, dWb


def pair_linear_usable(lin_a, lin_b) -> bool:
    F = lin_a.in_features
    return (ENABLED and CH.COMPUTE_DTYPE == "fp32" and F in (128, 256) and lin_a.bias is None and lin_b.bias is None
            and _square([lin_a, lin_b], F))


def pair_linear(a_pt: torch.Tensor, b_pt: torch.Tensor, pts: int, lin_a, lin_b):
    return _PairLinearFn.apply(a_pt, b_pt, pts, lin_a.weight, lin_b.weight)


class _XEncProjFn(torch.autograd.Function):

    @staticmethod
    def forward(ctx, X, n_x, *params):
        B, P, dx = X.shape
        dev = X.device
        tiles = P // 32
        Ws, bs = list(params[0::2]), list(params[1::2])
        W1, b1 = Ws[0], bs[0]
        x_W, x_b = Ws[1:1 + n_x], bs[1:1 + n_x]
        Wq, bq = Ws[-1], bs[-1]
        F = Wq.shape[0]
        train = any(ctx.needs_input_grad)
        imgs = _weight_images([*x_W, Wq], (1, 2) if train else (1,), F)
        fw = imgs[0]
        X4 = _pad_rows4(X.detach())
        pt = lambda: CH.pt_empty(B, P, F, dev)
        prog = Program(B, tiles, per_task=False, width=F)
        acts, bits = [], []
        h1 = pt() if train else None
        bits_h1 = _bits(B, tiles, dev) if train else None
        X_enc, Q = pt(), pt()
        for i in range(n_x):
            last = i == n_x - 1
            o = dict(img=fw[i], w_ref=("shared", x_W[i]), bias=x_b[i].detach() if x_b[i] is not None else None, relu=not last)
            if i == 0:
                o.update(in_rows=X4, in_w=_first_layer_matrix(W1, F), in_b=b1.detach() if b1 is not None else None, in_relu=True,
                         store_in=h1, store_in_bits=bits_h1)
            if last:
                o["store_out"] = X_enc
            elif train:
                o["store_out"], o["store_bits"] = pt(), _bits(B, tiles, dev)
                acts.append(o["store_out"])
                bits.append(o["store_bits"])
            prog.op(**o)
        prog.op(img=fw[n_x], w_ref=("shared", Wq), bias=bq.detach() if bq is not None else None, store_out=Q)
        prog.tag = "x-encoder + query projection"
        prog.launch()
        ctx.geom = (B, P, tiles, dx, F)
        ctx.n_x = n_x
        ctx.has_b = [b is not None for b in bs]
        ctx.set_materialize_grads(False)
        if train:
            ctx.save_for_backward(X4, h1, bits_h1, X_enc, *acts, *bits, *imgs[1])
        return X_enc, Q

    @staticmethod
    def backward(ctx, gX, gQ):
        n_x = ctx.n_x
        n_par = 2 * (n_x + 2)
        if gX is None and gQ is None:
            return (None,) * (2 + n_par)
        B, P, tiles, dx, F = ctx.geom
        sv = list(ctx.saved_tensors)
        X4, h1, bits_h1, X_enc = sv[:4]
        acts, bits, bw = sv[4:4 + n_x - 1], sv[4 + n_x - 1:4 + 2 * (n_x - 1)], sv[4 + 2 * (n_x - 1):]
        dev = X4.device
        pt = lambda: CH.pt_empty(B, P, F, dev)
        prog = Program(B, tiles, per_task=False, width=F)
        jobs, grads = [], [None] * n_par

        def wjob(pos, dZ, A, N, K):
            dW = torch.empty((N, K), dtype=torch.float32, device=dev)
            db = torch.empty((N,), dtype=torch.float32, device=dev) if ctx.has_b[pos] else None
            jobs.append(dict(dZ=dZ, A=A, N=N, K=K, dW=dW, db=db))
            grads[2 * pos], grads[2 * pos + 1] = dW, db
            return dW

        if gQ is not None:
            gQ = gQ.contiguous()
            prog.op(in_pt=gQ, img=bw[n_x])
            wjob(n_x + 1, gQ, X_enc, F, F)
            first = dict(pre_add=gX.contiguous()) if gX is not None else {}
        else:
            first = dict(in_pt=gX.contiguous())
        x_in = [h1, *acts]
        for i in range(n_x - 1, -1, -1):
            dz = pt()
            o = dict(store_in=dz, img=bw[i])
            if i == n_x - 1:
                o.update(first)
            else:
                o["mask_bits"] = bits[i]
            prog.op(**o)
            wjob(1 + i, dz, x_in[i], F, F)
        dz1 = pt()
        prog.op(mask_bits=bits_h1, store_in=dz1)
        dW1p = wjob(0, dz1, FN._pack(X4), F, 4)
        prog.tag = "x-encoder + query projection dgrad"
        prog.launch()
        CH.run_wgrad(jobs, B, P, dev, tag="x-encoder + query projection weight gradients")
        if dx != 4:
            grads[0] = dW1p[:, :dx].contiguous()
        return (None, None, *grads)


def xenc_proj_usable(model, lin_q, T: int) -> bool:
    from .architectures import MLP

    if not (ENABLED and CH.COMPUTE_DTYPE == "fp32") or T <= 0:
        return False
    F = _width_of(model)
    xe = model.x_encoder
    if not F or not (isinstance(xe, MLP) and xe.input_size <= 4 and xe.hidden_size == F and xe.output_size == F
                     and not xe.is_res and not (xe.dropout_p > 0 and xe.training)):
        return False
    return lin_q.in_features == F and lin_q.out_features == F and len(xe.linears) + 3 <= L.NPF_X6_MAX_OPS


def xenc_proj(model, X: torch.Tensor, lin_q):
    xe = model.x_encoder
    lins = [xe.to_hidden, *xe.linears, xe.out, lin_q]
    params = []
    for lin in lins:
        params += [lin.weight, lin.bias]
    T = X.shape[1]
    if T % 32:
        X = torch.nn.functional.pad(X, (0, 0, 0, CH.pad32(T) - T))
    Xe, Q = _XEncProjFn.apply(X, len(xe.linears) + 1, *params)
    return CH.PTensor(Xe, T, model.r_dim), Q


class _MlpPtFn(torch.autograd.Function):

    @staticmethod
    def forward(ctx, x_pt, pts, *params):
        B, tiles = x_pt.shape[0], x_pt.shape[1]
        dev = x_pt.device
        Ws, bs = list(params[0::2]), list(params[1::2])
        n, F = len(Ws), Ws[0].shape[0]
        train = any(ctx.needs_input_grad)
        imgs = _weight_images(Ws, (1, 2) if train else (1,), F)
        x_pt = x_pt.contiguous()
        pt = lambda: CH.pt_empty(B, tiles * 32, F, dev)
        prog = Program(B, tiles, per_task=False, width=F)
        acts, bits = [], []
        y = pt()
        for i in range(n):
            last = i == n - 1
            o = dict(img=imgs[0][i], w_ref=("shared", Ws[i]), bias=bs[i].detach() if bs[i] is not None else None, relu=not last)
            if i == 0:
                o["in_pt"] = x_pt.detach()
            if last:
                o["store_out"] = y
            elif train:
                o["store_out"], o["store_bits"] = pt(), _bits(B, tiles, dev)
                acts.append(o["store_out"])
                bits.append(o["store_bits"])
            prog.op(**o)
        prog.tag = "MLP block forward"
        prog.launch()
        ctx.geom = (B, tiles, F, pts, n)
        ctx.has_b = [b is not None for b in bs]
        ctx.set_materialize_grads(False)
        if train:
            ctx.save_for_backward(x_pt.detach(), *acts, *bits, *imgs[1])
        return y

    @staticmethod
    def backward(ctx, g):
        B, tiles, F, pts, n = ctx.geom
        if g is None:
            return (None,) * (2 + 2 * n)
        sv = list(ctx.saved_tensors)
        x_pt, acts, bits, bw = sv[0], sv[1:n], sv[n:2 * n - 1], sv[2 * n - 1:]
        dev = g.device
        g = g.contiguous()
        pt = lambda: CH.pt_empty(B, tiles * 32, F, dev)
        prog = Program(B, tiles, per_task=False, width=F)
        dz = [None] * n
        dx = pt()
        for i in range(n - 1, -1, -1):
            o = dict(img=bw[i])
            if i == n - 1:
                o["in_pt"], dz[i] = g, g
            else:
                dz[i] = pt()
                o.update(mask_bits=bits[i], store_in=dz[i])
            if i == 0:
                o["store_out"] = dx
            prog.op(**o)
        prog.tag = "MLP block dgrad"
        prog.launch()
        ins = [x_pt, *acts]
        jobs, grads = [], []
        for i in range(n):
            dW = torch.empty((F, F), dtype=torch.float32, device=dev)
            db = torch.empty((F,), dtype=torch.float32, device=dev) if ctx.has_b[i] else None
            jobs.append(dict(dZ=dz[i], A=ins[i], N=F, K=F, dW=dW, db=db))
            grads += [dW, db]
        CH.run_wgrad(jobs, B, pts, dev, tag="MLP block weight gradients")
        return (dx, None, *grads)


def mlp_pt_usable(mlp) -> bool:
    from .architectures import MLP

    if not (ENABLED and CH.COMPUTE_DTYPE == "fp32" and isinstance(mlp, MLP)):
        return False
    F = mlp.input_size
    if F not in (128, 256) or mlp.is_res or (mlp.dropout_p > 0 and mlp.training):
        return False
    return _square(mlp.layers(), F) and len(mlp.layers()) <= L.NPF_X6_MAX_OPS


def mlp_pt(mlp, x_pt: torch.Tensor, pts: int) -> torch.Tensor:
    params = []
    for lin in mlp.layers():
        params += [lin.weight, lin.bias]
    return _MlpPtFn.apply(x_pt, pts, *params)


def _width_of(model) -> int:
    F = getattr(model, "r_dim", 0)
    return F if (F in (128, 256) and getattr(model, "x_transf_dim", F) == F) else 0


def _mode_ok() -> bool:
    return ENABLED and (CH.COMPUTE_DTYPE == "fp32" or (CH.COMPUTE_DTYPE == "bf16" and B16_ENABLED))


def _square(lins, width=WIDTH) -> bool:
    return all(l.in_features == width and l.out_features == width for l in lins)


def target_side_usable(model, C: int, T: int, latent_merge: bool = False) -> bool:
    from .architectures import MLP, DotAttender

    if not _mode_ok():
        return False
    WIDTH = _width_of(model)
    if not WIDTH:
        return False
    xe, dec, att = model.x_encoder, model.decoder, getattr(model, "attender", None)
    if not isinstance(att, DotAttender) or att.kq_size != WIDTH or att.value_size != WIDTH:
        return False
    if not ((WIDTH // 2 < C or (WIDTH == 128 and C >= 1)) and C <= WIDTH and T > 0):
        return False
    if not (isinstance(xe, MLP) and xe.input_size <= 4 and xe.hidden_size == WIDTH and xe.output_size == WIDTH
            and not xe.is_res and not (xe.dropout_p > 0 and xe.training)):
        return False
    if not (dec.is_sum_merge and isinstance(dec.flat_module, MLP)):
        return False
    fm, rs = dec.flat_module, dec.resizer
    for m in (fm, rs):
        if m.is_res or (m.dropout_p > 0 and m.training):
            return False
    if not (_square(rs.layers(), WIDTH) and _square([fm.to_hidden, *fm.linears], WIDTH) and fm.out.in_features == WIDTH
            and fm.out.out_features <= 4):
        return False
    n_mrz = int(latent_merge)
    if n_mrz:
        mz = getattr(model, "r_z_merger", None)
        if mz is None or mz.out_features != WIDTH or mz.in_features <= WIDTH or model.r_dim != WIDTH:
            return False
    n_x, n_res, n_flat = len(xe.linears) + 1, len(rs.layers()), len(fm.linears) + 1
    return n_x + 2 + n_mrz + n_res + n_flat + 1 <= L.NPF_X6_MAX_OPS


def target_side(model, X_trgt: torch.Tensor, K: CH.PTensor, V: CH.PTensor, zb: Optional[torch.Tensor] = None) -> torch.Tensor:
    xe, dec, att = model.x_encoder, model.decoder, model.attender
    fm, rs = dec.flat_module, dec.resizer
    lins = [xe.to_hidden, *xe.linears, xe.out, *rs.layers(), fm.to_hidden, *fm.linears, fm.out]
    params = []
    for lin in lins:
        params += [lin.weight, lin.bias]
    n_x = len(xe.linears) + 1
    if zb is not None:
        params[2 * (n_x + 1):2 * (n_x + 1)] = [model.r_z_merger.weight[:, :model.r_dim], None]
    spec = (n_x, int(zb is not None), len(rs.layers()), len(fm.linears) + 1)
    scale = 1.0 / math.sqrt(att.kq_size) if att.is_scale else 1.0
    T = X_trgt.shape[1]
    Tp = CH.pad32(T)
    if Tp != T:
        X_trgt = torch.nn.functional.pad(X_trgt, (0, 0, 0, Tp - T))
    rows = _TargetSideFn.apply(X_trgt, K.t, V.t, K.pts, scale, spec, zb, *params)
    return rows if Tp == T else rows[:, :T].contiguous()


class _ContextSideFn(torch.autograd.Function):

    @staticmethod
    def forward(ctx, X, Y, spec, *params):
        n_x, n_flat = spec
        B, Cn, dx = X.shape
        dy = Y.shape[-1]
        dev = X.device
        tiles = Cn // 32
        Ws, bs = list(params[0::2]), list(params[1::2])
        W1, b1 = Ws[0], bs[0]
        x_W, x_b = Ws[1:1 + n_x], bs[1:1 + n_x]
        Wr1, br1, Wr2, br2 = Ws[1 + n_x], bs[1 + n_x], Ws[2 + n_x], bs[2 + n_x]
        f_W, f_b = Ws[3 + n_x:], bs[3 + n_x:]
        h = Wr1.shape[0]
        F = Wr2.shape[0]
        train = any(ctx.needs_input_grad)
        bf16 = CH.COMPUTE_DTYPE == "bf16"
        Wr2p = torch.zeros((F, F), dtype=torch.float32, device=dev)
        Wr2p[:, :h] = Wr2.detach()
        imgs = _weight_images([*x_W, Wr2p, *f_W], (1, 2) if train else (1,), F, bf16)
        fw = imgs[0]
        X4, Y4 = _pad_rows4(X.detach()), _pad_rows4(Y.detach())
        W1p, Wr1p = _first_layer_matrix(W1, F), _first_layer_matrix(Wr1, h)
        if bf16:
            X4, Y4, W1p, Wr1p = _r16(X4), _r16(Y4), _r16(W1p), _r16(Wr1p)
        pt = lambda: CH.pt_empty(B, Cn, F, dev)
        pb = (lambda: CH.pt16_empty(B, Cn, F, dev)) if bf16 else pt
        prog = Program(B, tiles, per_task=False, width=F, bf16=bf16)
        acts, bits = [], []
        h1 = pb() if train else None
        bits_h1 = _bits(B, tiles, dev) if train else None
        Xc_enc = pt()
        for i in range(n_x):
            last = i == n_x - 1
            o = dict(img=fw[i], w_ref=("shared", x_W[i]), bias=x_b[i].detach() if x_b[i] is not None else None, relu=not last)
            if i == 0:
                o.update(in_rows=X4, in_w=W1p, in_b=b1.detach() if b1 is not None else None,
                         in_relu=True, store_in=h1, store_in_bits=bits_h1)
            if last:
                o["store_out"], o["store_out_f32"] = Xc_enc, True
            elif train:
                o["store_out"], o["store_bits"] = pb(), _bits(B, tiles, dev)
                acts.append(o["store_out"])
                bits.append(o["store_bits"])
            prog.op(**o)
        hy = pb() if train else None
        bits_hy = _bits(B, tiles, dev) if train else None
        o = dict(in_rows=Y4, in_w=Wr1p, in_b=br1.detach() if br1 is not None else None, in_relu=True,
                 store_in=hy, store_in_bits=bits_hy, img=fw[n_x], w_ref=("shared", Wr2p),
                 bias=br2.detach() if br2 is not None else None, relu=True, addend=Xc_enc, true_k=h)
        if train:
            o["store_out"], o["store_bits"] = pb(), _bits(B, tiles, dev)
            acts.append(o["store_out"])
            bits.append(o["store_bits"])
        prog.op(**o)
        R = pt()
        for i in range(n_flat):
            last = i == n_flat - 1
            o = dict(img=fw[n_x + 1 + i], w_ref=("shared", f_W[i]), bias=f_b[i].detach() if f_b[i] is not None else None,
                     relu=not last)
            if last:
                o["store_out"], o["store_out_f32"] = R, True
            elif train:
                o["store_out"], o["store_bits"] = pb(), _bits(B, tiles, dev)
                acts.append(o["store_out"])
                bits.append(o["store_bits"])
            prog.op(**o)
        prog.tag = "context side forward (x-encoder, XY-encoder)"
        prog.launch()
        ctx.geom = (B, Cn, tiles, dx, dy, h, F)
        ctx.spec, ctx.bf16 = spec, bf16
        ctx.trace_ref = [W.detach() for W in (*x_W, Wr2p, *f_W)] if CH.TRACE is not None else None
        ctx.has_b = [b is not None for b in bs]
        ctx.set_materialize_grads(False)
        if train:
            ctx.n_acts = len(acts)
            ctx.save_for_backward(X4, Y4, h1, bits_h1, hy, bits_hy, *acts, *bits, *imgs[1])
        return Xc_enc, R

    @staticmethod
    def backward(ctx, gK, gR):
        n_x, n_flat = ctx.spec
        n_par = 2 * (1 + n_x + 2 + n_flat)
        if gK is None and gR is None:
            return (None,) * (3 + n_par)
        B, Cn, tiles, dx, dy, h, F = ctx.geom
        sv = list(ctx.saved_tensors)
        X4, Y4, h1, bits_h1, hy, bits_hy = sv[:6]
        acts, bits = sv[6:6 + ctx.n_acts], sv[6 + ctx.n_acts:6 + 2 * ctx.n_acts]
        bw = sv[6 + 2 * ctx.n_acts:]
        dev = X4.device
        bf16 = ctx.bf16
        pt = lambda: CH.pt_empty(B, Cn, F, dev)
        pb = (lambda: CH.pt16_empty(B, Cn, F, dev)) if bf16 else pt
        x_acts, x_bits = acts[:n_x - 1], bits[:n_x - 1]
        m_act, m_bits = acts[n_x - 1], bits[n_x - 1]
        f_acts, f_bits = acts[n_x:], bits[n_x:]
        prog = Program(B, tiles, per_task=False, width=F, bf16=bf16)
        wref = lambda j: ("shared", ctx.trace_ref[j].t()) if ctx.trace_ref is not None else None
        jobs, grads = [], [None] * n_par

        def wjob(pos, dZ, A, N, K, **kw):
            dW = torch.empty((N, K), dtype=torch.float32, device=dev)
            db = torch.empty((N,), dtype=torch.float32, device=dev) if ctx.has_b[pos] else None
            jobs.append(dict(dZ=dZ, A=A, N=N, K=K, dW=dW, db=db, **kw))
            grads[2 * pos], grads[2 * pos + 1] = dW, db
            return dW

        dz_m = None
        if gR is not None:
            gR = gR.contiguous()
            f_in = [m_act, *f_acts]
            for i in range(n_flat - 1, -1, -1):
                o = dict(img=bw[n_x + 1 + i], w_ref=wref(n_x + 1 + i))
                if i == n_flat - 1:
                    o["in_pt"] = gR
                    dz = gR
                    if bf16:
                        dz = pb()
                        o["store_in"] = dz
                else:
                    dz = pb()
                    o.update(mask_bits=f_bits[i], store_in=dz)
                prog.op(**o)
                wjob(1 + n_x + 2 + i, dz, f_in[i], F, F)
            dz_m, dz_hy = pt(), pb()
            prog.op(mask_bits=m_bits, store_in=dz_m, store_in_f32=True, img=bw[n_x], w_ref=wref(n_x))
            prog.op(mask_bits=bits_hy, store_in=dz_hy)
            wjob(1 + n_x + 1, dz_m, hy, F, h, lda=F)
            dWr1 = wjob(1 + n_x, dz_hy, FN._pack(Y4), h, 4, ldz=F)
        if gK is not None or dz_m is not None:
            first = dict(in_pt=gK.contiguous(), pre_add=dz_m) if gK is not None else dict(in_pt=dz_m)
            x_in = [h1, *x_acts]
            for i in range(n_x - 1, -1, -1):
                dz = pb()
                o = dict(store_in=dz, img=bw[i], w_ref=wref(i))
                if i == n_x - 1:
                    o.update(first)
                else:
                    o["mask_bits"] = x_bits[i]
                prog.op(**o)
                wjob(1 + i, dz, x_in[i], F, F)
            dz1 = pb()
            prog.op(mask_bits=bits_h1, store_in=dz1)
            dW1p = wjob(0, dz1, FN._pack(X4), F, 4)
        prog.tag = "context side dgrad (XY-encoder, x-encoder)"
        prog.launch()
        CH.run_wgrad(jobs, B, Cn, dev, tag="context side weight gradients")
        if CH.TRACE is not None:
            CH.TRACE.append(("wgrad", jobs, B, Cn, bf16))
        if gR is not None and dy != 4:
            grads[2 * (1 + n_x)] = dWr1[:, :dy].contiguous()
        if (gK is not None or dz_m is not None) and dx != 4:
            grads[0] = dW1p[:, :dx].contiguous()
        return (None, None, None, *grads)


def context_side_usable(model, C: int) -> bool:
    from .architectures import MLP, MergeFlatInputs

    if not _mode_ok() or C <= 0:
        return False
    WIDTH = _width_of(model)
    if not WIDTH:
        return False
    xe, xy = model.x_encoder, getattr(model, "xy_encoder", None)
    if not (isinstance(xe, MLP) and xe.input_size <= 4 and xe.hidden_size == WIDTH and xe.output_size == WIDTH
            and not xe.is_res and not (xe.dropout_p > 0 and xe.training)):
        return False
    if not (isinstance(xy, MergeFlatInputs) and xy.is_sum_merge and isinstance(xy.flat_module, MLP)):
        return False
    fm, rs = xy.flat_module, xy.resizer
    for m in (fm, rs):
        if m.is_res or (m.dropout_p > 0 and m.training):
            return False
    if not (_square([fm.to_hidden, *fm.linears, fm.out], WIDTH) and len(rs.linears) == 0 and rs.input_size <= 4
            and rs.output_size == WIDTH and rs.hidden_size % 16 == 0 and rs.hidden_size <= WIDTH):
        return False
    n_x, n_flat = len(xe.linears) + 1, len(fm.linears) + 2
    return n_flat + 2 + n_x + 1 <= L.NPF_X6_MAX_OPS


def context_side(model, X_cntxt: torch.Tensor, Y_cntxt: torch.Tensor):
    xe, xy = model.x_encoder, model.xy_encoder
    fm, rs = xy.flat_module, xy.resizer
    lins = [xe.to_hidden, *xe.linears, xe.out, rs.to_hidden, rs.out, fm.to_hidden, *fm.linears, fm.out]
    params = []
    for lin in lins:
        params += [lin.weight, lin.bias]
    Cn = X_cntxt.shape[1]
    if Cn % 32:
        pad = CH.pad32(Cn) - Cn
        X_cntxt = torch.nn.functional.pad(X_cntxt, (0, 0, 0, pad))
        Y_cntxt = torch.nn.functional.pad(Y_cntxt, (0, 0, 0, pad))
    Xc, R = _ContextSideFn.apply(X_cntxt, Y_cntxt, (len(xe.linears) + 1, len(fm.linears) + 2), *params)
    return CH.PTensor(Xc, Cn, model.r_dim), CH.PTensor(R, Cn, model.r_dim)
```

Before: 43.45 million target-points/s.

## Fuse step input padding, packing, bf16 rounding and range check into one kernel

Adds a single HIP kernel that, for the context X/Y and target X tensors, pads rows to four features, optionally rounds to bf16, writes both row-major and packed point-tile layouts, and folds the deferred input-range max into an atomic. The fused target and context paths then reuse these buffers instead of running separate pad, cast, pack and abs-amax torch ops in forward and backward. This removes several small launches and extra passes over the input tensors each step. The cost is a scoped global lookup keyed on tensor identity and extra saved tensors for backward.

```diff
diff --git a/include/npf_hip.h b/include/npf_hip.h
--- a/include/npf_hip.h
+++ b/include/npf_hip.h
@@ -175,6 +175,19 @@
 } npf_wprep_job_t;
 #define NPF_MAX_WPREP_JOBS 32
 int npf_prepare_weights(const npf_wprep_job_t *jobs, int32_t n_jobs, void *stream);
+
+typedef struct npf_step_input {
+  const float *src;
+  float *rows4;
+  float *pt;
+  int32_t pts, pts_pad, d, flags;
+} npf_step_input_t;
+#define NPF_STEP_IN_RANGE 1
+#define NPF_STEP_IN_BF16 2
+#define NPF_MAX_STEP_INPUTS 4
+int npf_step_inputs(const npf_step_input_t *in, int32_t n_in, int32_t n_tasks, float *range_seen, void *stream);
+int64_t npf_range_scalar_bits(float x);
+int npf_struct_layout(int32_t which, int32_t *out, int32_t n_out);
 
 #define NPF_X6_MAX_LAYERS 8
 typedef struct {
diff --git a/npf_gwwaveform_amd/_lib.py b/npf_gwwaveform_amd/_lib.py
--- a/npf_gwwaveform_amd/_lib.py
+++ b/npf_gwwaveform_amd/_lib.py
@@ -56,6 +56,15 @@
 
 
 NPF_MAX_WPREP_JOBS = 32
+
+
+class NpfStepInput(C.Structure):
+    _fields_ = [("src", C.c_void_p), ("rows4", C.c_void_p), ("pt", C.c_void_p), ("pts", C.c_int32), ("pts_pad", C.c_int32),
+                ("d", C.c_int32), ("flags", C.c_int32)]
+
+
+NPF_MAX_STEP_INPUTS = 4
+STEP_IN_RANGE, STEP_IN_BF16 = 1, 2
 NPF_X6_MAX_LAYERS = 8
 
 
@@ -86,7 +95,7 @@
     _fields_ = [("src", C.c_void_p), ("dst", C.c_void_p), ("F", C.c_int32), ("reserved", C.c_int32)]
 
 
-assert C.sizeof(NpfAppendPair) == 24
+assert C.sizeof(NpfAppendPair) == 24 and C.sizeof(NpfStepInput) == 40
 assert C.sizeof(NpfX6Op) == 17 * 8 + 8 * 4
 assert C.sizeof(NpfOp) == 80 and C.sizeof(NpfProgram) == 32 + 80 * NPF_MAX_OPS and C.sizeof(NpfWgradJob) == 72 and C.sizeof(NpfWprepJob) == 32
 
@@ -106,6 +115,9 @@
     "npf_transpose": (C.c_int, [_p, _i32, _i32, _p, _p]),
     "npf_cast_bf16_weights": (C.c_int, [_p, _i32, _i32, _i32, _i32, _p, _p]),
     "npf_prepare_weights": (C.c_int, [C.POINTER(NpfWprepJob), _i32, _p]),
+    "npf_step_inputs": (C.c_int, [C.POINTER(NpfStepInput), _i32, _i32, _p, _p]),
+    "npf_range_scalar_bits": (_i64, [C.c_float]),
+    "npf_struct_layout": (C.c_int, [_i32, C.POINTER(_i32), _i32]),
     "npf_gather_points": (C.c_int, [_p, _p, _p, _i32, _i32, _i32, _i32, _i32, _p, _p, _p]),
     "npf_split_heads": (C.c_int, [_p, _i32, _i32, _i32, _i32, _p, _p]),
     "npf_merge_heads": (C.c_int, [_p, _i32, _i32, _i32, _i32, _p, _p]),
diff --git a/npf_gwwaveform_amd/csrc/layout_kernels.hip b/npf_gwwaveform_amd/csrc/layout_kernels.hip
--- a/npf_gwwaveform_amd/csrc/layout_kernels.hip
+++ b/npf_gwwaveform_amd/csrc/layout_kernels.hip
@@ -1,3 +1,5 @@
+#include <stddef.h>
+
 #include "npf_common.hpp"
 
 namespace npf {
@@ -167,6 +169,56 @@
   }
 }
 
+struct StepInputs {
+  npf_step_input_t in[NPF_MAX_STEP_INPUTS];
+};
+__global__ void step_inputs_kernel(const StepInputs S, int n_tasks, uint32_t* __restrict__ range_seen) {
+  __shared__ uint32_t red[4];
+  const npf_step_input_t& in = S.in[blockIdx.y];
+  const int pts = in.pts, P = in.pts_pad, d = in.d;
+  const bool r16 = (in.flags & NPF_STEP_IN_BF16) != 0;
+  const bool ranged = (in.flags & NPF_STEP_IN_RANGE) != 0 && range_seen != nullptr;
+  const float* __restrict__ src = in.src;
+  const size_t total = (size_t)n_tasks * P;
+  uint32_t worst = 0;
+  for (size_t idx = blockIdx.x * (size_t)blockDim.x + threadIdx.x; idx < total; idx += (size_t)gridDim.x * blockDim.x) {
+    const size_t task = idx / P;
+    const int point = (int)(idx - task * P);
+    f32x4 v = {0.f, 0.f, 0.f, 0.f};
+    if (point < pts) {
+      const float* s = src + (task * pts + point) * (size_t)d;
+#pragma unroll
+      for (int j = 0; j < 4; ++j)
+        if (j < d) {
+          const float x = s[j];
+          const uint32_t e = npf_range_encode(x);
+          worst = e > worst ? e : worst;
+          v[j] = r16 ? npf_round_bf16(x) : x;
+        }
+    }
+    if (in.rows4) *(f32x4*)(in.rows4 + idx * 4) = v;
+    if (in.pt) {
+      float* q = in.pt + ((task * (P >> 5) + (point >> 5)) * 8 * 32 + (point & 31)) * 4;
+      *(f32x4*)q = v;
+      const f32x4 z = {0.f, 0.f, 0.f, 0.f};
+#pragma unroll
+      for (int f4 = 1; f4 < 8; ++f4) *(f32x4*)(q + f4 * 32 * 4) = z;
+    }
+  }
+  if (!ranged) return;
+#pragma unroll
+  for (int off = 32; off >= 1; off >>= 1) {
+    const uint32_t o = (uint32_t)__shfl_xor((int)worst, off);
+    worst = o > worst ? o : worst;
+  }
+  if ((threadIdx.x & 63) == 0) red[threadIdx.x >> 6] = worst;
+  __syncthreads();
+  if (threadIdx.x == 0) {
+    for (int i = 1; i < (int)(blockDim.x >> 6); ++i) worst = red[i] > worst ? red[i] : worst;
+    if (worst) atomicMax(range_seen, worst);
+  }
+}
+
 template <bool MASKED>
 __global__ void mean_fwd_kernel(const float* __restrict__ R, const int32_t* __restrict__ n_valid, int pts, int F,
                                 float* __restrict__ out) {
@@ -444,6 +496,60 @@
   return NPF_OK;
 }
 
+extern "C" int npf_step_inputs(const npf_step_input_t* in, int32_t n_in, int32_t n_tasks, float* range_seen, void* stream) {
+  if (!in || n_in <= 0 || n_in > NPF_MAX_STEP_INPUTS || n_tasks <= 0) return NPF_EINVAL;
+  if (((uintptr_t)range_seen) & 3) return NPF_EINVAL;
+  npf::StepInputs S;
+  size_t most = 0;
+  for (int i = 0; i < n_in; ++i) {
+    const npf_step_input_t& b = in[i];
+    if (!b.src || b.pts <= 0 || b.pts_pad < b.pts || b.d <= 0 || b.d > 4 || (b.flags & ~(NPF_STEP_IN_RANGE | NPF_STEP_IN_BF16)))
+      return NPF_EINVAL;
+    if (b.pt && (b.pts_pad & 31)) return NPF_EINVAL;
+    if ((((uintptr_t)b.rows4) | ((uintptr_t)b.pt)) & 15) return NPF_EINVAL;
+    S.in[i] = b;
+    const size_t total = (size_t)n_tasks * b.pts_pad;
+    most = total > most ? total : most;
+  }
+  for (int i = n_in; i < NPF_MAX_STEP_INPUTS; ++i) S.in[i] = in[0];
+  const size_t blocks = (most + 255) / 256;
+  hipLaunchKernelGGL(npf::step_inputs_kernel, dim3((unsigned)(blocks < 512 ? blocks : 512), n_in), dim3(256), 0,
+                     (hipStream_t)stream, S, n_tasks, (uint32_t*)range_seen);
+  NPF_CHECK_LAUNCH();
+  return NPF_OK;
+}
+
+extern "C" int64_t npf_range_scalar_bits(float x) { return (int64_t)npf::npf_range_encode(x); }
+
+extern "C" int npf_struct_layout(int32_t which, int32_t* out, int32_t n_out) {
+  int32_t v[16];
+  int n = 0;
+#define NPF_MEMBER(T, m) v[n++] = (int32_t)offsetof(T, m)
+  if (which == 0) {
+    v[n++] = (int32_t)sizeof(npf_step_input_t);
+    NPF_MEMBER(npf_step_input_t, src); NPF_MEMBER(npf_step_input_t, rows4); NPF_MEMBER(npf_step_input_t, pt);
+    NPF_MEMBER(npf_step_input_t, pts); NPF_MEMBER(npf_step_input_t, pts_pad); NPF_MEMBER(npf_step_input_t, d);
+    NPF_MEMBER(npf_step_input_t, flags);
+  } else if (which == 1) {
+    v[n++] = (int32_t)sizeof(npf_wgrad_job_t);
+    NPF_MEMBER(npf_wgrad_job_t, dZ); NPF_MEMBER(npf_wgrad_job_t, A); NPF_MEMBER(npf_wgrad_job_t, dW);
+    NPF_MEMBER(npf_wgrad_job_t, db); NPF_MEMBER(npf_wgrad_job_t, ldw); NPF_MEMBER(npf_wgrad_job_t, N);
+    NPF_MEMBER(npf_wgrad_job_t, K); NPF_MEMBER(npf_wgrad_job_t, per_task); NPF_MEMBER(npf_wgrad_job_t, accumulate);
+    NPF_MEMBER(npf_wgrad_job_t, ldz); NPF_MEMBER(npf_wgrad_job_t, lda); NPF_MEMBER(npf_wgrad_job_t, ldo);
+    NPF_MEMBER(npf_wgrad_job_t, reserved);
+  } else if (which == 2) {
+    v[n++] = (int32_t)sizeof(npf_wprep_job_t);
+    NPF_MEMBER(npf_wprep_job_t, src); NPF_MEMBER(npf_wprep_job_t, dst); NPF_MEMBER(npf_wprep_job_t, n_rows);
+    NPF_MEMBER(npf_wprep_job_t, n_cols); NPF_MEMBER(npf_wprep_job_t, ld); NPF_MEMBER(npf_wprep_job_t, kind);
+  } else {
+    return -1;
+  }
+#undef NPF_MEMBER
+  for (int i = 0; i < n && i < n_out; ++i)
+    if (out) out[i] = v[i];
+  return n;
+}
+
 extern "C" int npf_split_heads(const float* src, int32_t n_tasks, int32_t pts, int32_t F, int32_t n_heads, float* dst,
                                void* stream) {
   return heads_launch(true, src, n_tasks, pts, F, n_heads, dst, stream);
diff --git a/npf_gwwaveform_amd/csrc/npf_common.hpp b/npf_gwwaveform_amd/csrc/npf_common.hpp
--- a/npf_gwwaveform_amd/csrc/npf_common.hpp
+++ b/npf_gwwaveform_amd/csrc/npf_common.hpp
@@ -20,7 +20,19 @@
   return v < 0 ? 0 : (v > hi ? hi : v);
 }
 
-#define NPF_CHECK_LAUNCH()                     \
+__host__ __device__ inline uint32_t npf_range_encode(float x) {
+  const uint32_t u = __builtin_bit_cast(uint32_t, x) & 0x7fffffffu;
+  return u > 0x7f800000u ? 0x7fc00000u : u;
+}
+
+__host__ __device__ inline float npf_round_bf16(float x) {
+  uint32_t u = __builtin_bit_cast(uint32_t, x);
+  if ((u & 0x7fffffffu) > 0x7f800000u) return __builtin_bit_cast(float, 0x7fc00000u);
+  u += 0x7fffu + ((u >> 16) & 1u);
+  return __builtin_bit_cast(float, u & 0xffff0000u);
+}
+
+#define NPF_CHECK_LAUNCH()                    \
   do {                                         \
     hipError_t e__ = hipGetLastError();        \
     if (e__ != hipSuccess) return NPF_ELAUNCH; \
diff --git a/npf_gwwaveform_amd/functional.py b/npf_gwwaveform_amd/functional.py
--- a/npf_gwwaveform_amd/functional.py
+++ b/npf_gwwaveform_amd/functional.py
@@ -52,6 +52,45 @@
 
 def unpack_pt(pt: torch.Tensor, pts: int, F: int) -> torch.Tensor:
     return _UnpackFn.apply(pt, pts, F)
+
+
+def step_glue_enabled() -> bool:
+    return os.environ.get("NPF_NO_STEP_GLUE", "0") != "1"
+
+
+class StepInput(NamedTuple):
+    src: torch.Tensor
+    rows4: Optional[torch.Tensor]
+    pt: Optional[torch.Tensor]
+    P: int
+
+
+def step_inputs(srcs, pads, want_rows, want_pt, in_range, range_seen: Optional[torch.Tensor] = None, bf16: bool = False):
+    live = [i for i, s in enumerate(srcs) if s is not None and s.numel()]
+    out = [None] * len(srcs)
+    if not live:
+        return out
+    if len(live) > L.NPF_MAX_STEP_INPUTS:
+        raise ValueError(f"step_inputs takes at most {L.NPF_MAX_STEP_INPUTS} tensors")
+    B, dev = srcs[live[0]].shape[0], srcs[live[0]].device
+    if range_seen is not None and (range_seen.dtype != torch.float32 or range_seen.numel() != 1 or range_seen.device != dev):
+        raise ValueError("range_seen must be one fp32 value on the batch's device")
+    arr = (L.NpfStepInput * len(live))()
+    keep = []
+    for j, i in enumerate(live):
+        s = srcs[i]
+        if s.dim() != 3 or s.shape[0] != B or s.shape[2] > 4 or pads[i] < s.shape[1] or (want_pt[i] and pads[i] % 32):
+            raise ValueError(f"step_inputs: tensor {tuple(s.shape)} for {B} tasks of {pads[i]} padded points")
+        sc = s.detach().contiguous()
+        keep.append(sc)
+        rows4 = torch.empty((B, pads[i], 4), dtype=torch.float32, device=dev) if want_rows[i] else None
+        pt = pt_empty(B, pads[i], 4, dev) if want_pt[i] else None
+        arr[j].src, arr[j].rows4, arr[j].pt = L.ptr(sc), L.ptr(rows4), L.ptr(pt)
+        arr[j].pts, arr[j].pts_pad, arr[j].d = s.shape[1], pads[i], s.shape[2]
+        arr[j].flags = (L.STEP_IN_RANGE if in_range[i] and range_seen is not None else 0) | (L.STEP_IN_BF16 if bf16 else 0)
+        out[i] = StepInput(s, rows4, pt, pads[i])
+    L.check(L.load().npf_step_inputs(arr, len(live), B, L.ptr(range_seen), L.stream_ptr()), "npf_step_inputs")
+    return out
 
 
 def sum_points_pt(pt: torch.Tensor, pts: int, F: int) -> torch.Tensor:
diff --git a/npf_gwwaveform_amd/neuralproc.py b/npf_gwwaveform_amd/neuralproc.py
--- a/npf_gwwaveform_amd/neuralproc.py
+++ b/npf_gwwaveform_amd/neuralproc.py
@@ -665,7 +665,7 @@
             n_trgt = self._check_counts(n_trgt, X_trgt, "n_trgt")
         if w_cntxt is not None:
             w_cntxt = self._check_weights(w_cntxt, X_cntxt)
-        self._validate_inputs(X_cntxt, Y_cntxt, X_trgt, Y_trgt)
+        glue = self._validate_inputs(X_cntxt, Y_cntxt, X_trgt, Y_trgt, n_cntxt is not None or w_cntxt is not None)
         B, C, _ = X_cntxt.shape
         T = X_trgt.shape[1]
         if T == 0:
@@ -674,8 +674,39 @@
             full = n_cntxt if n_cntxt is not None else torch.full((B,), C, dtype=torch.int32, device=X_cntxt.device)
             n_cntxt = TrainKeyWeights(w_cntxt, full)
         fused_t = self._fused_target_side(C, T)
-        Xc_pt, R = self._context_stage(X_cntxt, Y_cntxt, n_cntxt, fused_t)
-        return self._target_stage(Xc_pt, R, X_trgt, Y_trgt, B, C, n_cntxt, n_trgt, fused_t)
+        from . import x6
+
+        with x6.step_inputs_scope(glue):
+            Xc_pt, R = self._context_stage(X_cntxt, Y_cntxt, n_cntxt, fused_t)
+            return self._target_stage(Xc_pt, R, X_trgt, Y_trgt, B, C, n_cntxt, n_trgt, fused_t)
+
+    def _step_inputs(self, X_cntxt, Y_cntxt, X_trgt, padded):
+        from . import chain as _chain
+        from . import x6
+
+        if not (self.training and torch.is_grad_enabled() and FN.step_glue_enabled()):
+            return None, False
+        if any(t.dim() != 3 for t in (X_cntxt, Y_cntxt, X_trgt)):
+            return None, False
+        B, C, dx = X_cntxt.shape
+        T = X_trgt.shape[1]
+        if min(B, C, T, dx, Y_cntxt.shape[2]) <= 0 or max(dx, Y_cntxt.shape[2], X_trgt.shape[2]) > 4:
+            return None, False
+        bf16 = _chain.COMPUTE_DTYPE == "bf16"
+        fused_t = self._fused_target_side(C, T) and not padded
+        fused_c = self._fused_context_side(C) and not (self._attentive and not fused_t and bf16 and not padded)
+        if not (fused_t or fused_c):
+            return None, False
+        defer = self.validate_inputs == "deferred"
+        if defer and (getattr(self, "_range_seen", None) is None or self._range_seen.device != X_trgt.device):
+            self._range_seen = torch.zeros((), device=X_trgt.device)
+        want = (fused_c, fused_c, fused_t)
+        in_range = (defer, False, defer)
+        pack = True
+        srcs = tuple(t if (w or r) else None for t, w, r in zip((X_cntxt, Y_cntxt, X_trgt), want, in_range))
+        glue = FN.step_inputs(srcs, (_chain.pad32(C), _chain.pad32(C), _chain.pad32(T)), want, tuple(w and pack for w in want),
+                              in_range, range_seen=self._range_seen if defer else None, bf16=bf16)
+        return glue, defer
 
     def influence(self, X_cntxt, Y_cntxt, X_trgt, Y_trgt, n_cntxt=None, n_trgt=None) -> torch.Tensor:
         self._refuse_weights()
@@ -915,8 +946,11 @@
             raise ValueError(f"{what} lives on {n.device}, the batch on {X.device}")
         return n
 
-    def _validate_inputs(self, X_cntxt, Y_cntxt, X_trgt, Y_trgt):
+    def _validate_inputs(self, X_cntxt, Y_cntxt, X_trgt, Y_trgt, padded=False):
         self._check_tensors(X_cntxt, Y_cntxt, X_trgt, Y_trgt)
+        glue, ranged = self._step_inputs(X_cntxt, Y_cntxt, X_trgt, padded)
+        if ranged:
+            return glue
         if self.training and self.validate_inputs:
             m = X_trgt.abs().amax() if X_trgt.numel() else X_trgt.new_zeros(())
             if X_cntxt.numel():
@@ -925,11 +959,12 @@
                 if getattr(self, "_range_seen", None) is None or self._range_seen.device != m.device:
                     self._range_seen = torch.zeros((), device=m.device)
                 self._range_seen.copy_(torch.maximum(self._range_seen, m))
-                return
+                return glue
             if not (m.item() <= 1.0):
                 lo = min(X_cntxt.min().item() if X_cntxt.numel() else 0.0, X_trgt.min().item())
                 hi = max(X_cntxt.max().item() if X_cntxt.numel() else 0.0, X_trgt.max().item())
                 raise ValueError(f"Features during training should be in [-1,1]. Got [{lo}, {hi}].")
+        return glue
 
     @staticmethod
     def _check_tensors(*tensors):
diff --git a/npf_gwwaveform_amd/x6.py b/npf_gwwaveform_amd/x6.py
--- a/npf_gwwaveform_amd/x6.py
+++ b/npf_gwwaveform_amd/x6.py
@@ -200,6 +200,43 @@
     return torch.cat((X, _zeros((*X.shape[:-1], 4 - d), X.device)), dim=-1)
 
 
+_STEP_INPUTS = None
+
+
+class step_inputs_scope:
+
+    def __init__(self, entries):
+        self.entries = entries
+
+    def __enter__(self):
+        global _STEP_INPUTS
+        self.before, _STEP_INPUTS = _STEP_INPUTS, self.entries
+        return self
+
+    def __exit__(self, *exc):
+        global _STEP_INPUTS
+        _STEP_INPUTS = self.before
+        return False
+
+
+def _step_input(X: torch.Tensor):
+    for e in _STEP_INPUTS or ():
+        if e is None or e.rows4 is None or e.P != CH.pad32(X.shape[1]):
+            continue
+        s = e.src
+        if s is X or (s.data_ptr() == X.data_ptr() and s.shape == X.shape and s.stride() == X.stride() and s.dtype == X.dtype):
+            return e
+    return None
+
+
+def _rows4_of(X: torch.Tensor, bf16: bool):
+    e = _step_input(X)
+    if e is not None:
+        return e.rows4, e.pt, e.P
+    X4 = _pad_rows4(X.detach())
+    return (_r16(X4) if bf16 else X4), None, X.shape[1]
+
+
 def _first_layer_matrix(W: torch.Tensor, n_out: int) -> torch.Tensor:
     n, d = W.shape
     Wt = W.detach().t()
@@ -268,7 +305,9 @@
     @staticmethod
     def forward(ctx, X, K_pt, V_pt, C, scale, spec, zb, *params):
         n_x, n_mrz, n_res, n_flat = spec
-        B, T, dx = X.shape
+        bf16 = CH.COMPUTE_DTYPE == "bf16"
+        B, dx = X.shape[0], X.shape[2]
+        X4, X4_pt, T = _rows4_of(X, bf16)
         dev = X.device
         tiles = T // 32
         Ws, bs = list(params[0::2]), list(params[1::2])
@@ -280,15 +319,13 @@
         if n_mrz:
             mid_b[n_x] = zb
         train = any(ctx.needs_input_grad)
-        bf16 = CH.COMPUTE_DTYPE == "bf16"
         imgs = _weight_images(mid_W, (1, 2) if train else (1,), F, bf16)
         fw = imgs[0]
         K_row, K_tr = task_images(K_pt, C, row=True, tr=train, width=F, bf16=bf16)
         V_row, V_tr = task_images(V_pt, C, row=train, tr=True, width=F, bf16=bf16)
-        X4 = _pad_rows4(X.detach())
         W1p = _first_layer_matrix(W1, F)
         if bf16:
-            X4, W1p = _r16(X4), _r16(W1p)
+            W1p = _r16(W1p)
         pt = lambda: CH.pt_empty(B, T, F, dev)
         pb = (lambda: CH.pt16_empty(B, T, F, dev)) if bf16 else pt
         prog = Program(B, tiles, per_task=True, width=F, bf16=bf16)
@@ -338,7 +375,7 @@
         ctx.set_materialize_grads(False)
         if train:
             ctx.n_acts, ctx.n_bits = len(saved_acts), len(saved_bits)
-            ctx.save_for_backward(X4, h1, bits_h1, Xt_enc, P, R_trgt, *saved_acts, *saved_bits, *imgs[1], V_row, K_tr, Wo)
+            ctx.save_for_backward(X4, h1, bits_h1, Xt_enc, P, R_trgt, *saved_acts, *saved_bits, *imgs[1], V_row, K_tr, Wo, X4_pt)
         return rows[..., :n_out] if n_out != 4 else rows
 
     @staticmethod
@@ -355,7 +392,7 @@
         acts = sv[6:6 + ctx.n_acts]
         bits = sv[6 + ctx.n_acts:6 + ctx.n_acts + ctx.n_bits]
         rest = sv[6 + ctx.n_acts + ctx.n_bits:]
-        bw, (V_row, K_tr, Wo) = rest[:n_mid], rest[n_mid:]
+        bw, (V_row, K_tr, Wo, X4_pt) = rest[:n_mid], rest[n_mid:]
         dev = g.device
         bf16 = ctx.bf16
         g4 = g.contiguous() if n_out == 4 else torch.nn.functional.pad(g, (0, 4 - n_out)).contiguous()
@@ -394,7 +431,7 @@
         jobs, grads = [], []
         dW1p = torch.empty((F, 4), dtype=torch.float32, device=dev)
         db1 = torch.empty((F,), dtype=torch.float32, device=dev) if ctx.has_b[0] else None
-        jobs.append(dict(dZ=dz1, A=FN._pack(X4), N=F, K=4, dW=dW1p, db=db1))
+        jobs.append(dict(dZ=dz1, A=X4_pt if X4_pt is not None else FN._pack(X4), N=F, K=4, dW=dW1p, db=db1))
         grads += [None, db1]
         ins = [h1, *x_acts, R_trgt, *d_acts[:-1]]
         for j in range(n_mid):
@@ -882,7 +919,7 @@
     scale = 1.0 / math.sqrt(att.kq_size) if att.is_scale else 1.0
     T = X_trgt.shape[1]
     Tp = CH.pad32(T)
-    if Tp != T:
+    if Tp != T and _step_input(X_trgt) is None:
         X_trgt = torch.nn.functional.pad(X_trgt, (0, 0, 0, Tp - T))
     rows = _TargetSideFn.apply(X_trgt, K.t, V.t, K.pts, scale, spec, zb, *params)
     return rows if Tp == T else rows[:, :T].contiguous()
@@ -893,8 +930,12 @@
     @staticmethod
     def forward(ctx, X, Y, spec, *params):
         n_x, n_flat = spec
-        B, Cn, dx = X.shape
-        dy = Y.shape[-1]
+        bf16 = CH.COMPUTE_DTYPE == "bf16"
+        B, dx, dy = X.shape[0], X.shape[2], Y.shape[2]
+        X4, X4_pt, Cn = _rows4_of(X, bf16)
+        Y4, Y4_pt, CnY = _rows4_of(Y, bf16)
+        if CnY != Cn:
+            raise ValueError(f"context side: {Cn} rows of features, {CnY} of values")
         dev = X.device
         tiles = Cn // 32
         Ws, bs = list(params[0::2]), list(params[1::2])
@@ -905,15 +946,13 @@
         h = Wr1.shape[0]
         F = Wr2.shape[0]
         train = any(ctx.needs_input_grad)
-        bf16 = CH.COMPUTE_DTYPE == "bf16"
         Wr2p = torch.zeros((F, F), dtype=torch.float32, device=dev)
         Wr2p[:, :h] = Wr2.detach()
         imgs = _weight_images([*x_W, Wr2p, *f_W], (1, 2) if train else (1,), F, bf16)
         fw = imgs[0]
-        X4, Y4 = _pad_rows4(X.detach()), _pad_rows4(Y.detach())
         W1p, Wr1p = _first_layer_matrix(W1, F), _first_layer_matrix(Wr1, h)
         if bf16:
-            X4, Y4, W1p, Wr1p = _r16(X4), _r16(Y4), _r16(W1p), _r16(Wr1p)
+            W1p, Wr1p = _r16(W1p), _r16(Wr1p)
         pt = lambda: CH.pt_empty(B, Cn, F, dev)
         pb = (lambda: CH.pt16_empty(B, Cn, F, dev)) if bf16 else pt
         prog = Program(B, tiles, per_task=False, width=F, bf16=bf16)
@@ -965,7 +1004,7 @@
         ctx.set_materialize_grads(False)
         if train:
             ctx.n_acts = len(acts)
-            ctx.save_for_backward(X4, Y4, h1, bits_h1, hy, bits_hy, *acts, *bits, *imgs[1])
+            ctx.save_for_backward(X4, Y4, h1, bits_h1, hy, bits_hy, X4_pt, Y4_pt, *acts, *bits, *imgs[1])
         return Xc_enc, R
 
     @staticmethod
@@ -976,9 +1015,9 @@
             return (None,) * (3 + n_par)
         B, Cn, tiles, dx, dy, h, F = ctx.geom
         sv = list(ctx.saved_tensors)
-        X4, Y4, h1, bits_h1, hy, bits_hy = sv[:6]
-        acts, bits = sv[6:6 + ctx.n_acts], sv[6 + ctx.n_acts:6 + 2 * ctx.n_acts]
-        bw = sv[6 + 2 * ctx.n_acts:]
+        X4, Y4, h1, bits_h1, hy, bits_hy, X4_pt, Y4_pt = sv[:8]
+        acts, bits = sv[8:8 + ctx.n_acts], sv[8 + ctx.n_acts:8 + 2 * ctx.n_acts]
+        bw = sv[8 + 2 * ctx.n_acts:]
         dev = X4.device
         bf16 = ctx.bf16
         pt = lambda: CH.pt_empty(B, Cn, F, dev)
@@ -1018,7 +1057,7 @@
             prog.op(mask_bits=m_bits, store_in=dz_m, store_in_f32=True, img=bw[n_x], w_ref=wref(n_x))
             prog.op(mask_bits=bits_hy, store_in=dz_hy)
             wjob(1 + n_x + 1, dz_m, hy, F, h, lda=F)
-            dWr1 = wjob(1 + n_x, dz_hy, FN._pack(Y4), h, 4, ldz=F)
+            dWr1 = wjob(1 + n_x, dz_hy, Y4_pt if Y4_pt is not None else FN._pack(Y4), h, 4, ldz=F)
         if gK is not None or dz_m is not None:
             first = dict(in_pt=gK.contiguous(), pre_add=dz_m) if gK is not None else dict(in_pt=dz_m)
             x_in = [h1, *x_acts]
@@ -1033,7 +1072,7 @@
                 wjob(1 + i, dz, x_in[i], F, F)
             dz1 = pb()
             prog.op(mask_bits=bits_h1, store_in=dz1)
-            dW1p = wjob(0, dz1, FN._pack(X4), F, 4)
+            dW1p = wjob(0, dz1, X4_pt if X4_pt is not None else FN._pack(X4), F, 4)
         prog.tag = "context side dgrad (XY-encoder, x-encoder)"
         prog.launch()
         CH.run_wgrad(jobs, B, Cn, dev, tag="context side weight gradients")
@@ -1081,7 +1120,9 @@
     Cn = X_cntxt.shape[1]
     if Cn % 32:
         pad = CH.pad32(Cn) - Cn
-        X_cntxt = torch.nn.functional.pad(X_cntxt, (0, 0, 0, pad))
-        Y_cntxt = torch.nn.functional.pad(Y_cntxt, (0, 0, 0, pad))
+        if _step_input(X_cntxt) is None:
+            X_cntxt = torch.nn.functional.pad(X_cntxt, (0, 0, 0, pad))
+        if _step_input(Y_cntxt) is None:
+            Y_cntxt = torch.nn.functional.pad(Y_cntxt, (0, 0, 0, pad))
     Xc, R = _ContextSideFn.apply(X_cntxt, Y_cntxt, (len(xe.linears) + 1, len(fm.linears) + 2), *params)
     return CH.PTensor(Xc, Cn, model.r_dim), CH.PTensor(R, Cn, model.r_dim)
```

Result: faster. 43.92 million target-points/s (median of 6 runs) (+1.1%).
